# arkworks-rs/sumcheck

Measured on AMD Instinct MI355X. Metric: MLSumcheck prover field-ops/s (BLS12-381 Fr, nv=24), higher is better.
Workload: dtype u256 (BLS12-381 Fr, Montgomery form; integer arithmetic on 9 x 29-bit limbs); 1 GPU; BASELINE config 3: MLSumcheck prove, ListOfProducts [[0, 1, 2, 3], [4, 5, 6], [7, 8], [9]] over 10 tables, nv=24 (24 per GPU shard), BLS12-381 Fr, tables HBM-resident; nv=24, nv_per_gpu=24, tables=10, degree=4, launcher=single process, ranks_seen=1, communicator=none, round_loop=library, round_loop_reason=single GPU: no exchange

## Files before the change

### sumcheck_amd/build.py

```python
from __future__ import annotations

import os
import subprocess
import sys

HERE = os.path.dirname(os.path.abspath(__file__))
CSRC = os.path.join(HERE, "csrc")
OUT = os.path.join(HERE, "libsumcheck_hip.so")
OUT_EXP = os.path.join(HERE, "libsumcheck_hip_exp.so")
SOURCES = ["kernels_big.hip", "kernels.hip", "kernels_tail.hip", "kernels_batch.hip", "kernels_batch_gkr.hip", "kernels_batch_eval.hip", "kernels_batch_rounds.hip", "kernels_wide.hip", "kernels_wide16.hip", "gkr.hip", "abi.hip", "protocol.hip", "batch.hip", "batch_rounds.hip", "comm.hip", "kernels_selftest.hip"]
HEADERS = ["fr_device.hpp", "fe_device.hpp", "kernel_common.hpp", "finalize_device.hpp", "batch_round.hpp", "wide_cell.hpp", "fe_mad_chain.inc", "fr_mac.inc", "fr_mul_gen.inc", "kernels.h", "host_fr.hpp", "transcript.hpp", "prover_internal.hpp", "load_factor.hpp", "wide_tree.hpp", os.path.join("..", "..", "include", "sumcheck_hip.h")]
EXTRA = os.environ.get("SC_BUILD_EXTRA", "").split()
FLAGS = ["--offload-arch=gfx950", "-O3", "-std=c++17", "-fPIC", "-fvisibility=hidden", "-Wall", "-Wno-unused-function"]


def _stale(out: str) -> bool:
    if not os.path.exists(out):
        return True
    t = os.path.getmtime(out)
    deps = [os.path.join(CSRC, s) for s in SOURCES + HEADERS] + [os.path.abspath(__file__)]
    return any(os.path.getmtime(d) > t for d in deps if os.path.exists(d))


def _obj_stale(obj: str, src: str, cmd: list) -> bool:
    dep = obj + ".d"
    if not (os.path.exists(obj) and os.path.exists(dep)):
        return True
    try:
        if open(obj + ".cmd").read() != " ".join(cmd):
            return True
    except OSError:
        return True
    t = os.path.getmtime(obj)
    try:
        words = open(dep).read().replace("\\\n", " ").split()
    except OSError:
        return True
    files = [w for w in words[1:] if not w.endswith(":")] + [src, os.path.abspath(__file__)]
    return any((not os.path.exists(f)) or os.path.getmtime(f) > t for f in files if not f.startswith("/opt/rocm"))


def _start(experiments: bool, verbose: bool, force: bool = False):
    hipcc = os.environ.get("HIPCC", "/opt/rocm/bin/hipcc")
    bdir = os.path.join(HERE, "build_exp" if experiments else "build")
    os.makedirs(bdir, exist_ok=True)
    procs, objs = [], []
    stale_any = False
    for s in SOURCES:
        o = os.path.join(bdir, s + ".o")
        objs.append(o)
        src = os.path.join(CSRC, s)
        cmd = [hipcc] + FLAGS + (["-DSC_EXPERIMENTS"] if experiments else []) + EXTRA + ["-Rpass-analysis=kernel-resource-usage", "-MD", "-MF", o + ".d", "-c", src, "-o", o]
        if not force and not _obj_stale(o, src, cmd):
            continue
        stale_any = True
        if os.path.exists(o + ".cmd"):
            os.remove(o + ".cmd")
        if verbose:
            print(" ".join(cmd), file=sys.stderr)
        procs.append((cmd, o, subprocess.Popen(cmd, stderr=open(o + ".log", "w"))))
    return hipcc, procs, objs


def _finish(hipcc, procs, objs, out):
    for cmd, o, p in procs:
        if p.wait() != 0:
            try:
                sys.stderr.write("".join(l for l in open(o + ".log") if "remark:" not in l and "-Rpass" not in l)[-8000:])
            except OSError:
                pass
            for f in (o, o + ".d"):
                if os.path.exists(f):
                    os.remove(f)
            raise RuntimeError("hipcc failed: " + " ".join(cmd))
        with open(o + ".cmd", "w") as f:
            f.write(" ".join(cmd))
    subprocess.check_call([hipcc, "--offload-arch=gfx950", "-shared", "-fPIC"] + objs + ["-o", out])
    return out


def _cmd_mismatch(experiments: bool) -> bool:
    hipcc = os.environ.get("HIPCC", "/opt/rocm/bin/hipcc")
    bdir = os.path.join(HERE, "build_exp" if experiments else "build")
    for s in SOURCES:
        o = os.path.join(bdir, s + ".o")
        cmd = [hipcc] + FLAGS + (["-DSC_EXPERIMENTS"] if experiments else []) + EXTRA + ["-Rpass-analysis=kernel-resource-usage", "-MD", "-MF", o + ".d", "-c", os.path.join(CSRC, s), "-o", o]
        try:
            if open(o + ".cmd").read() != " ".join(cmd):
                return True
        except OSError:
            if os.path.exists(o):
                return True
    return False

# ... 21 lines not shown
```

### sumcheck_amd/csrc/abi.hip

```cpp
#include "prover_internal.hpp"

static std::atomic<uint32_t> g_publish_timeout_ms{0};
std::chrono::milliseconds publish_timeout() {
    uint32_t ms = g_publish_timeout_ms.load(std::memory_order_relaxed);
    if (ms == 0) {
        const char *e = std::getenv("SC_PUBLISH_TIMEOUT_MS");
        const long v = e ? std::atol(e) : 0;
        ms = v > 0 ? (uint32_t)std::min<long>(v, 3600 * 1000L) : 20000u;
        g_publish_timeout_ms.store(ms, std::memory_order_relaxed);
    }
    return std::chrono::milliseconds(ms);
}
extern "C" int sc_set_publish_timeout_ms(uint32_t ms) {
    g_publish_timeout_ms.store(ms ? ms : 20000u, std::memory_order_relaxed);
    return SC_OK;
}
static thread_local std::string g_last_error;
static thread_local int g_device = 0;

static std::recursive_mutex g_gate_mutex[64];
thread_local uint16_t g_gate_depth[64];
void gate_lock(int device) {
    g_gate_mutex[(unsigned)device & 63u].lock();
    ++g_gate_depth[(unsigned)device & 63u];
// ... 228 lines not shown
#ifdef SC_EXPERIMENTS
    if (const char *e = std::getenv("SC_FE")) p->use_fe = std::atoi(e) != 0;
    if (const char *e = std::getenv("SC_KERNEL")) p->kernel_variant = std::atoi(e);
    if (!p->use_fe && p->kernel_variant == 3) p->kernel_variant = 0;
#endif
    p->use_f29 = p->kernel_variant == 3;
    p->wide_tree = wide_tree_enabled();
#ifdef SC_EXPERIMENTS
    if (const char *e = std::getenv("SC_F29")) p->use_f29 = p->use_f29 && std::atoi(e) != 0;
#endif
    for (uint32_t k = 0; k < d->n_products; ++k)
        if (d->prod_offsets[k + 1] - d->prod_offsets[k] > (p->wide_tree ? 8u : 4u)) p->use_f29 = false;
    if (d->n_tables > (uint32_t)scd::kMaxSmallTables) p->use_f29 = false;
    p->merge_rounds = p->kernel_variant == 3 && d->n_products > 0 && d->n_products <= (uint32_t)scd::kMaxRoundProds;
    for (uint32_t k = 0; k < d->n_products; ++k)
        if (d->prod_offsets[k + 1] - d->prod_offsets[k] > 4) p->merge_rounds = false;
#ifdef SC_EXPERIMENTS
    if (const char *e = std::getenv("SC_MERGE")) p->merge_rounds = p->merge_rounds && std::atoi(e) != 0;
    if (const char *e = std::getenv("SC_FUSED_FIN")) p->fused_finalize = std::atoi(e) != 0;
#endif
    p->use_tail = scd::policy(scd::kPolTail) != 0;

    uint64_t partial_elems = 0;
    std::vector<uint32_t> slot_table, slot_exp;
    std::vector<FinProd> fin(p->K);
    std::vector<Combo> combos;
    std::vector<sch::Fr> Wall;
    for (uint32_t k = 0; k < p->K; ++k) {
        Product pr;
        std::memcpy(&pr.coeff, d->coeffs + 4 * k, 32);
        if (sch::geq_p(pr.coeff)) return sc_internal_fail(SC_ERR_BAD_ARG, "coefficient %u is not a canonical field element", k);
        for (uint32_t q = d->prod_offsets[k]; q < d->prod_offsets[k + 1]; ++q) {
            const uint32_t t = d->prod_indices[q];
            auto it = std::find(pr.tables.begin(), pr.tables.end(), t);
            if (it == pr.tables.end()) {
                pr.tables.push_back(t);
                pr.exps.push_back(1);
            } else {
                pr.exps[it - pr.tables.begin()]++;
            }
        }
        p->prod_indices.emplace_back(d->prod_indices + d->prod_offsets[k], d->prod_indices + d->prod_offsets[k + 1]);
        pr.M = d->prod_offsets[k + 1] - d->prod_offsets[k];
        pr.fused = pr.M <= (uint32_t)scd::kMaxFusedM;
        if (!pr.fused) p->any_generic = true;
        pr.partial_off = partial_elems;
        partial_elems += (uint64_t)scd::kMaxGrid * (pr.M + 1);
        pr.slot_off = (uint32_t)slot_table.size();
        slot_table.insert(slot_table.end(), pr.tables.begin(), pr.tables.end());
        slot_exp.insert(slot_exp.end(), pr.exps.begin(), pr.exps.end());
        fin[k].M = pr.M;
        fin[k].pad = 0;
        fin[k].partial_off = pr.partial_off;
        {
            sch::Fr sc = pr.coeff;
            for (uint32_t dbl = 0; dbl < 5 * (pr.M - 1); ++dbl) sc = sch::add(sc, sc);
            std::vector<sch::Fr> w;
            fin[k].w_off = Wall.size();
            build_node_matrix(pr.M, p->D, pr.coeff, w);
            Wall.insert(Wall.end(), w.begin(), w.end());
            build_node_matrix(pr.M, p->D, sc, w);
            Wall.insert(Wall.end(), w.begin(), w.end());
        }
        for (uint32_t t = 0; t <= pr.M; ++t) {
            Combo c;
            c.t = t;
            c.M = pr.M;
            c.slot_off = pr.slot_off;
            c.n_slots = (uint32_t)pr.tables.size();
            c.partial_off = pr.partial_off;
            combos.push_back(c);
        }
        p->prods.push_back(std::move(pr));
    }

    const bool on_device = d->flags & SC_TABLES_ON_DEVICE;
    const bool borrow = on_device && (d->flags & SC_TABLES_BORROW);
    const uint64_t n = 1ULL << p->nv;
    const bool streamed = !on_device && (d->flags & SC_TABLES_STREAM) && p->nv >= 11;
    const bool small_foot = borrow || streamed;
    bool staged = false;
    const uint64_t s0 = small_foot ? std::max<uint64_t>(n >> 1, 1) : n;
    const uint64_t s1 = small_foot ? std::max<uint64_t>(n >> 2, 1) : std::max<uint64_t>(n >> 1, 1);
    const uint64_t per_table = (s0 + s1) * 36;
    HIP_TRY(hipMalloc(&p->arena, per_table * p->U));
    p->arena_bytes = per_table * p->U;
    p->tabs.resize(p->U);
    p->borrow = borrow;
    if (on_device && !borrow) HIP_TRY(hipDeviceSynchronize());
    for (uint32_t u = 0; u < p->U; ++u) {
        Table &t = p->tabs[u];
        char *base = static_cast<char *>(p->arena) + per_table * u;
        t.buf[0] = reinterpret_cast<uint4 *>(base);
        t.buf[1] = reinterpret_cast<uint4 *>(base + s0 * 32);
        t.buf_top[0] = reinterpret_cast<int32_t *>(base + (s0 + s1) * 32);
        t.buf_top[1] = t.buf_top[0] + s0;
        if (streamed) {
            t.cur = nullptr;
            t.next = 0;
            p->host_tabs.push_back(d->tables[u]);
        } else if (borrow) {
            t.cur = reinterpret_cast<const uint4 *>(d->tables[u]);
            t.next = 0;
            p->origin.push_back(t.cur);
        } else {
            if (!on_device && (d->flags & SC_TABLES_STREAM)) p->host_tabs.push_back(d->tables[u]);
            if (!(staged = !on_device && staged_init_applies(p)))
                HIP_TRY(hipMemcpyAsync(t.buf[0], d->tables[u], n * 32, on_device ? hipMemcpyDeviceToDevice : hipMemcpyHostToDevice, p->stream));
            t.cur = t.buf[0];
            t.next = 1;
        }
    }

    if (streamed) {
        p->streamed = true;
        uint32_t cl = p->stream_chunk_request ? p->stream_chunk_request : 22u;
        cl = std::max(10u, std::min(cl, p->nv));
        p->chunk_log2 = cl;
        for (int q = 0; q < 2; ++q) {
            HIP_TRY(hipMalloc(&p->ring[q], ((size_t)p->U << cl) * 32));
            HIP_TRY(hipEventCreateWithFlags(&p->ev_copied[q], hipEventDisableTiming));
            HIP_TRY(hipEventCreateWithFlags(&p->ev_consumed[q], hipEventDisableTiming));
        }
        HIP_TRY(hipStreamCreateWithFlags(&p->copy_stream, hipStreamNonBlocking));
        HIP_TRY(hipMalloc(&p->d_chunk_msg, (size_t)2 * p->D * 32));
    }
    HIP_TRY(hipMalloc(&p->d_partials, std::max<uint64_t>(partial_elems, 1) * 32));
    HIP_TRY(hipMalloc(&p->d_partials2, std::max<uint64_t>(partial_elems, 1) * 32));
    HIP_TRY(hipMalloc(&p->d_fin_counters, 4 * (2 + scd::kMaxGrid / 32 + 16)));
    HIP_TRY(hipMemsetAsync(p->d_fin_counters, 0, 4 * (2 + scd::kMaxGrid / 32 + 16), p->stream));
    p->d_fin_mb_counter = p->d_fin_counters + (2 + scd::kMaxGrid / 32 + 8);
    HIP_TRY(hipMalloc(&p->d_finprods, std::max<size_t>(p->K, 1) * sizeof(FinProd)));
    if (p->K) HIP_TRY(hipMemcpyAsync(p->d_finprods, fin.data(), p->K * sizeof(FinProd), hipMemcpyHostToDevice, p->stream));
    p->h_finprods = fin;
    HIP_TRY(hipMalloc(&p->d_W, std::max<size_t>(2 * Wall.size(), 1) * 32));
    p->w_elems = (uint32_t)Wall.size();
    if (!Wall.empty()) {
        HIP_TRY(hipMemcpyAsync(p->d_W, Wall.data(), Wall.size() * 32, hipMemcpyHostToDevice, p->stream));
        HIP_TRY(hipMemcpyAsync(p->d_W + Wall.size(), Wall.data(), Wall.size() * 32, hipMemcpyHostToDevice, p->stream));
    }
    HIP_TRY(hipMalloc(&p->d_scratch, (size_t)(2 + p->D) * std::max<uint32_t>(p->K, 1) * p->D * 32));
    {
        const size_t one = (size_t)std::max<uint32_t>(p->K, 1) * p->D * 32;
        HIP_TRY(hipMalloc(&p->d_sums[0], 2 * one));
        p->d_sums[1] = reinterpret_cast<FrHost *>(reinterpret_cast<char *>(p->d_sums[0]) + one);
    }
    HIP_TRY(hipMalloc(&p->d_out, (size_t)p->D * 32));
    HIP_TRY(hipHostMalloc(reinterpret_cast<void **>(&p->h_out), (size_t)p->D * 32, hipHostMallocMapped | hipHostMallocCoherent));
    HIP_TRY(hipHostMalloc(reinterpret_cast<void **>(&p->h_flag), 64, hipHostMallocMapped | hipHostMallocCoherent));
    *p->h_flag = 0;
    HIP_TRY(hipHostGetDevicePointer(reinterpret_cast<void **>(&p->h_out_dev), p->h_out, 0));
    HIP_TRY(hipHostGetDevicePointer(reinterpret_cast<void **>(&p->h_flag_dev), p->h_flag, 0));
    p->has_meta = combos.size() <= (size_t)scd::kMetaCombos && slot_table.size() <= (size_t)scd::kMetaSlots;
    if (p->has_meta) {
        std::memset(&p->meta, 0, sizeof(p->meta));
        std::copy(combos.begin(), combos.end(), p->meta.combo);
        std::copy(slot_table.begin(), slot_table.end(), p->meta.slot_table);
        std::copy(slot_exp.begin(), slot_exp.end(), p->meta.slot_exp);
    }
    p->n_combos = (int)combos.size();
    HIP_TRY(hipMalloc(&p->d_combos, std::max<size_t>(combos.size(), 1) * sizeof(Combo)));
    if (!combos.empty()) HIP_TRY(hipMemcpyAsync(p->d_combos, combos.data(), combos.size() * sizeof(Combo), hipMemcpyHostToDevice, p->stream));
    HIP_TRY(hipMalloc(&p->d_slot_table, std::max<size_t>(slot_table.size(), 1) * 4));
    HIP_TRY(hipMalloc(&p->d_slot_exp, std::max<size_t>(slot_exp.size(), 1) * 4));
    if (!slot_table.empty()) {
        HIP_TRY(hipMemcpyAsync(p->d_slot_table, slot_table.data(), slot_table.size() * 4, hipMemcpyHostToDevice, p->stream));
        HIP_TRY(hipMemcpyAsync(p->d_slot_exp, slot_exp.data(), slot_exp.size() * 4, hipMemcpyHostToDevice, p->stream));
    }
    if (p->any_generic || p->U > (uint32_t)scd::kMaxSmallTables) {
        HIP_TRY(hipMalloc(&p->d_cur_tables, 2 * p->U * sizeof(void *)));
        HIP_TRY(hipHostMalloc(reinterpret_cast<void **>(&p->h_cur_tables), 2 * p->U * sizeof(void *), hipHostMallocDefault));
    }
    if (staged) {
        int rc_s = staged_copy_and_round1(p, d->tables);
        if (rc_s) return rc_s;
    }
    HIP_TRY(hipStreamSynchronize(p->stream));
    return SC_OK;
}
// ... 22 lines not shown
        kept->pool_key.clear();
        prover_destroy(kept);
    }
    sc_prover *p = new (std::nothrow) sc_prover();
    if (!p) return sc_internal_fail(SC_ERR_OOM, "host allocation failed");
    rc = prover_build(desc, p);
    if (rc) {
        prover_destroy(p);
        return rc;
    }
    p->pool_key = std::move(key);
    *out = p;
    return SC_OK;
}

extern "C" int sc_prover_init_streamed(const sc_poly_desc *desc, uint32_t chunk_log2, sc_prover **out) {
    if (!out) return sc_internal_fail(SC_ERR_BAD_ARG, "null out");
    *out = nullptr;
    int rc = validate_desc(desc);
    if (rc) return rc;
    if (desc->flags & SC_TABLES_ON_DEVICE) return sc_internal_fail(SC_ERR_BAD_ARG, "streamed tables are host tables");
    sc_prover *p = new (std::nothrow) sc_prover();
    if (!p) return sc_internal_fail(SC_ERR_OOM, "host allocation failed");
    p->stream_chunk_request = chunk_log2;
    sc_poly_desc d2 = *desc;
    d2.flags |= SC_TABLES_STREAM;
    rc = prover_build(&d2, p);
    if (rc) {
        prover_destroy(p);
        return rc;
    }
    *out = p;
    return SC_OK;
}

extern "C" int sc_prover_set_stream(sc_prover *p, void *hip_stream, int use_own) {
    if (!p) return sc_internal_fail(SC_ERR_BAD_ARG, "null prover");
    int rc_q = resident_quiesce(p);
    if (rc_q) return rc_q;
    DeviceGate gate_(p->device);
    HIP_TRY(hipSetDevice(p->device));
    HIP_TRY(hipStreamSynchronize(p->stream));
    p->stream = use_own ? p->own_stream : static_cast<hipStream_t>(hip_stream);
    return SC_OK;
}

int collect_timing(sc_prover *p) {
    if (!p->timing || !p->timing_pending) return SC_OK;
    HIP_TRY(hipEventSynchronize(p->ev1));
    float ms = 0.f;
    HIP_TRY(hipEventElapsedTime(&ms, p->ev0, p->ev1));
    p->rounds_ms += ms;
    for (uint32_t k = 0; k < (p->prod_merged ? 1u : p->K) && p->prod_timed; ++k) {
        HIP_TRY(hipEventElapsedTime(&ms, p->prod_ev[2 * k], p->prod_ev[2 * k + 1]));
        p->prod_ms[k] += ms;
        p->prod_launches[k] += 1;
        if (p->timed_round >= 1 && p->timed_round <= p->round_kernel_ms.size()) {
            p->round_kernel_ms[p->timed_round - 1] += ms;
            if (k == 0) p->round_kernel_launches[p->timed_round - 1] += 1;
        }
    }
    p->timing_pending = false;
    return SC_OK;
}

int prover_bind_out(sc_prover *p, const uint64_t *r, uint64_t *d_out) {
    int rc_q = resident_quiesce(p);
    if (rc_q) return rc_q;
    DeviceGate gate_(p->device);
    if (p->exhausted || p->round == 0 || p->round > p->nv) return sc_internal_fail(SC_ERR_NOT_ACTIVE, "bind needs a prover that has run at least one round");
    if (p->streamed && p->round < 2) return sc_internal_fail(SC_ERR_NOT_ACTIVE, "a streamed handle's tables are resident from round 2 on: nothing to bind yet");
    sch::Fr rr;
    std::memcpy(&rr, r, 32);
    if (sch::geq_p(rr)) return sc_internal_fail(SC_ERR_BAD_ARG, "challenge is not a canonical field element");
    HIP_TRY(hipSetDevice(p->device));
    p->randomness.push_back(rr);
    const uint64_t n_out = 1ULL << (p->nv - p->round);
    for (uint32_t u0 = 0; u0 < p->U; u0 += (uint32_t)scd::kMaxSmallTables) {
        const uint32_t cnt = std::min<uint32_t>(p->U - u0, (uint32_t)scd::kMaxSmallTables);
        TablePtrs tp;
        std::memset(&tp, 0, sizeof(tp));
        for (uint32_t j = 0; j < cnt; ++j) {
            tp.src[j] = p->tabs[u0 + j].cur;
            tp.src_top[j] = p->tabs[u0 + j].cur_top;
            tp.dst[j] = reinterpret_cast<uint4 *>(d_out + 4 * n_out * (size_t)(u0 + j));
        }
        HIP_TRY(scd::launch_fix_multi(tp, (int)cnt, to_dev(rr), nullptr, n_out, p->stream));
    }
    p->exhausted = true;
    return SC_OK;
}

extern "C" int sc_prover_bind_final(sc_prover *p, const uint64_t *r, uint64_t *d_out) {
    if (!p || !r || !d_out) return sc_internal_fail(SC_ERR_BAD_ARG, "null argument");
    if (p->exhausted || p->round != p->nv) return sc_internal_fail(SC_ERR_NOT_ACTIVE, "bind_final needs a prover that has finished its last local round");
    return prover_bind_out(p, r, d_out);
}

extern "C" int sc_prover_push_randomness(sc_prover *p, const uint64_t *r) {
    if (!p || !r) return sc_internal_fail(SC_ERR_BAD_ARG, "null argument");
    sch::Fr rr;
    std::memcpy(&rr, r, 32);
    p->randomness.push_back(rr);
    return SC_OK;
}

extern "C" int sc_prover_state(sc_prover *p, uint64_t *randomness, uint32_t *n_randomness, uint64_t *tables_out, uint32_t *round) {
    if (!p) return sc_internal_fail(SC_ERR_BAD_ARG, "null prover");
    if (tables_out) {
        int rc_q = resident_quiesce(p);
        if (rc_q) return rc_q;
    }
    DeviceGate gate_(p->device);
    if (randomness && !p->randomness.empty()) std::memcpy(randomness, p->randomness.data(), p->randomness.size() * 32);
    if (n_randomness) *n_randomness = (uint32_t)p->randomness.size();
    if (round) *round = p->round;
    if (tables_out) {
        if (p->exhausted) return sc_internal_fail(SC_ERR_NOT_ACTIVE, "tables were consumed by sc_prover_bind_final");
        HIP_TRY(hipSetDevice(p->device));
        const uint32_t bound = p->round > 0 ? p->round - 1 : 0;
        const uint64_t n = 1ULL << (p->nv - bound);
        if (p->streamed && p->round < 2) {
            for (uint32_t u = 0; u < p->U; ++u) std::memcpy(tables_out + 4 * n * u, p->host_tabs[u], n * 32);
            return SC_OK;
        }
        void *tmp = nullptr;
        for (uint32_t u = 0; u < p->U; ++u) {
            const void *src = p->tabs[u].cur;
            if (p->tabs[u].cur_top) {
                if (!tmp) HIP_TRY(hipMalloc(&tmp, n * 32));
                HIP_TRY(scd::launch_f29_to_sat(p->tabs[u].cur, p->tabs[u].cur_top, static_cast<uint4 *>(tmp), n, p->stream));
                src = tmp;
            }
            HIP_TRY(hipMemcpyAsync(tables_out + 4 * n * u, src, n * 32, hipMemcpyDeviceToHost, p->stream));
            if (tmp) HIP_TRY(hipStreamSynchronize(p->stream));
        }
        if (tmp) (void)hipFree(tmp);
        HIP_TRY(hipStreamSynchronize(p->stream));
    }
    return SC_OK;
}

extern "C" int sc_prover_last_round_ms(sc_prover *p, float *ms) {
    if (!p || !ms) return sc_internal_fail(SC_ERR_BAD_ARG, "null argument");
    if (!p->timed) return sc_internal_fail(SC_ERR_BAD_ARG, "no timed round: enable sc_prover_set_timing before the round");
    HIP_TRY(hipEventSynchronize(p->ev1));
    HIP_TRY(hipEventElapsedTime(ms, p->ev0, p->ev1));
    return SC_OK;
}

extern "C" int sc_prover_set_timing(sc_prover *p, int on) {
    if (!p) return sc_internal_fail(SC_ERR_BAD_ARG, "null prover");
    int rc_q = resident_quiesce(p);
    if (rc_q) return rc_q;
    DeviceGate gate_(p->device);
    HIP_TRY(hipSetDevice(p->device));
    if (on && p->prod_ev.empty()) {
        p->prod_ev.resize(2 * (size_t)p->K);
        for (auto &e : p->prod_ev) HIP_TRY(hipEventCreate(&e));
    }
    p->timing = on != 0;
    p->timing_pending = false;
    p->prod_ms.assign(p->K, 0.0);
    p->prod_launches.assign(p->K, 0);
    p->rounds_ms = 0.0;
    p->round_kernel_ms.assign(p->nv, 0.0);
    p->round_kernel_launches.assign(p->nv, 0);
    return SC_OK;
}

extern "C" int sc_prover_get_round_timing(sc_prover *p, double *ms_per_round, uint64_t *launches_per_round) {
    if (!p) return sc_internal_fail(SC_ERR_BAD_ARG, "null prover");
    DeviceGate gate_(p->device);
    if (!p->timing) return sc_internal_fail(SC_ERR_BAD_ARG, "timing is not enabled on this handle");
    HIP_TRY(hipSetDevice(p->device));
    int rc = collect_timing(p);
    if (rc) return rc;
    for (uint32_t i = 0; i < p->nv; ++i) {
        if (ms_per_round) ms_per_round[i] = i < p->round_kernel_ms.size() ? p->round_kernel_ms[i] : 0.0;
        if (launches_per_round) launches_per_round[i] = i < p->round_kernel_launches.size() ? p->round_kernel_launches[i] : 0;
    }
    return SC_OK;
}

extern "C" int sc_prover_get_timing(sc_prover *p, double *ms_per_product, uint64_t *launches_per_product, double *rounds_ms) {
    if (!p) return sc_internal_fail(SC_ERR_BAD_ARG, "null prover");
    DeviceGate gate_(p->device);
    if (!p->timing) return sc_internal_fail(SC_ERR_BAD_ARG, "timing is not enabled on this handle");
    HIP_TRY(hipSetDevice(p->device));
    int rc = collect_timing(p);
    if (rc) return rc;
    for (uint32_t k = 0; k < p->K; ++k) {
        if (ms_per_product) ms_per_product[k] = p->prod_ms[k];
        if (launches_per_product) launches_per_product[k] = p->prod_launches[k];
    }
    if (rounds_ms) *rounds_ms = p->rounds_ms;
    return SC_OK;
}

extern "C" int sc_prover_reset(sc_prover *p, const uint64_t *const *tables_or_null, uint32_t flags) {
    if (!p) return sc_internal_fail(SC_ERR_BAD_ARG, "null prover");
    (void)resident_quiesce(p);
    DeviceGate gate_(p->device);
    HIP_TRY(hipSetDevice(p->device));
    abandon_deferred(p);
    if (wait_gave_up(p)) {
        HIP_TRY(hipStreamSynchronize(p->stream));
        __atomic_store_n(p->sig + 1, 0u, __ATOMIC_RELEASE);
    }
    {
        int rc_t = collect_timing(p);
        if (rc_t) return rc_t;
    }
    p->r1_cached = false;
    if (p->w_scaled) {
        HIP_TRY(hipMemcpyAsync(p->d_W, p->d_W + p->w_elems, (size_t)p->w_elems * 32, hipMemcpyDeviceToDevice, p->stream));
        p->w_scaled = false;
    }
    const uint64_t n = 1ULL << p->nv;
    if (p->streamed) {
        if (flags & SC_TABLES_ON_DEVICE) return sc_internal_fail(SC_ERR_BAD_ARG, "streamed tables are host tables");
        HIP_TRY(hipStreamSynchronize(p->stream));
        for (uint32_t u = 0; u < p->U; ++u) {
            if (tables_or_null) {
                if (!tables_or_null[u]) return sc_internal_fail(SC_ERR_BAD_ARG, "table %u is null", u);
                p->host_tabs[u] = tables_or_null[u];
            }
            p->tabs[u].cur = nullptr;
            p->tabs[u].cur_top = nullptr;
            p->tabs[u].next = 0;
        }
    } else if (p->borrow) {
        for (uint32_t u = 0; u < p->U; ++u) {
            if (tables_or_null) {
                if (!tables_or_null[u]) return sc_internal_fail(SC_ERR_BAD_ARG, "table %u is null", u);
                p->origin[u] = reinterpret_cast<const uint4 *>(tables_or_null[u]);
            }
            p->tabs[u].cur = p->origin[u];
            p->tabs[u].cur_top = nullptr;
            p->tabs[u].next = 0;
        }
    } else {
        if (!tables_or_null && p->host_tabs.size() == p->U) tables_or_null = p->host_tabs.data();
        if (!tables_or_null) return sc_internal_fail(SC_ERR_BAD_ARG, "a copying handle needs the tables again to reset");
        const bool on_device = flags & SC_TABLES_ON_DEVICE;
        if (on_device) HIP_TRY(hipDeviceSynchronize());
        const bool staged = !on_device && staged_init_applies(p);
        for (uint32_t u = 0; u < p->U; ++u) {
            if (!tables_or_null[u]) return sc_internal_fail(SC_ERR_BAD_ARG, "table %u is null", u);
            if (!staged)
                HIP_TRY(hipMemcpyAsync(p->tabs[u].buf[0], tables_or_null[u], n * 32, on_device ? hipMemcpyDeviceToDevice : hipMemcpyHostToDevice,
                                       p->stream));
            p->tabs[u].cur = p->tabs[u].buf[0];
            p->tabs[u].cur_top = nullptr;
            p->tabs[u].next = 1;
        }
        if (staged) {
            p->round = 0;
            p->exhausted = false;
            int rc_s = staged_copy_and_round1(p, tables_or_null);
            if (rc_s) return rc_s;
        }
        HIP_TRY(hipStreamSynchronize(p->stream));
    }
    p->round = 0;
    p->sums_round = -1;
    p->exhausted = false;
    p->randomness.clear();
    return SC_OK;
}

hipStream_t sc_internal_prover_stream(sc_prover *p) { return p->stream; }
const void *sc_internal_bound_table(sc_prover *p, uint32_t u) {
    if (!p || u >= p->U || p->round != p->nv || p->exhausted || p->tabs[u].cur_top || p->res.active) return nullptr;
    return p->tabs[u].cur;
}
int sc_internal_scale_by_bound_table(sc_prover *p, const void *table, const sch::Fr &r_last) {
    if (!p || !table || p->round != 0) return sc_internal_fail(SC_ERR_BAD_ARG, "scale_by_bound_table: a freshly reset handle and a bound table");
    DeviceGate gate_(p->device);
    HIP_TRY(hipSetDevice(p->device));
    HIP_TRY(scd::launch_scale_w_by_table_eval(p->d_W, p->d_W + p->w_elems, p->w_elems, table, to_dev(r_last), p->stream));
    p->w_scaled = true;
    return SC_OK;
}

namespace {
struct DevMem {
    void *p = nullptr;
    ~DevMem() {
        if (p) (void)hipFree(p);
    }
};
struct StreamGuard {
    hipStream_t s = nullptr;
    ~StreamGuard() {
        if (s) (void)hipStreamDestroy(s);
    }
};
struct EvalCache {
    std::mutex mu;
    void *buf = nullptr;
    size_t cap = 0;
    int device = -1;
    hipStream_t s = nullptr;
};
EvalCache g_eval_cache;
struct EvalLease {
    bool held = false;
    EvalLease() : held(g_eval_cache.mu.try_lock()) {}
    ~EvalLease() {
        if (held) g_eval_cache.mu.unlock();
    }
    void *get(int device, size_t bytes, hipStream_t *s_out) {
        if (!held || bytes > sc_internal_cache_limit()) return nullptr;
        EvalCache &c = g_eval_cache;
        if (c.device != device) {
            if (c.buf) (void)hipFree(c.buf);
            if (c.s) (void)hipStreamDestroy(c.s);
            c.buf = nullptr;
            c.s = nullptr;
            c.cap = 0;
            c.device = device;
        }
        if (!c.s && hipStreamCreateWithFlags(&c.s, hipStreamNonBlocking) != hipSuccess) {
            (void)hipGetLastError();
            c.s = nullptr;
            return nullptr;
        }
        if (c.cap < bytes) {
            if (c.buf) (void)hipFree(c.buf);
            c.buf = nullptr;
            c.cap = 0;
            if (hipMalloc(&c.buf, bytes) != hipSuccess) {
                (void)hipGetLastError();
                c.buf = nullptr;
                return nullptr;
            }
            c.cap = bytes;
        }
        *s_out = c.s;
        return c.buf;
    }
};
}
void sc_internal_release_eval_cache() {
    std::lock_guard<std::mutex> lk(g_eval_cache.mu);
    if (g_eval_cache.device >= 0) (void)hipSetDevice(g_eval_cache.device);
    if (g_eval_cache.buf) (void)hipFree(g_eval_cache.buf);
    if (g_eval_cache.s) (void)hipStreamDestroy(g_eval_cache.s);
    g_eval_cache.buf = nullptr;
    g_eval_cache.s = nullptr;
    g_eval_cache.cap = 0;
    g_eval_cache.device = -1;
}

extern "C" int sc_fix_variables(const uint64_t *in, uint32_t nv, const uint64_t *point, uint32_t k, uint64_t *out, uint32_t flags) {
    if (!in || !out || (k && !point)) return sc_internal_fail(SC_ERR_BAD_ARG, "null argument");
// ... 538 lines not shown
```

### sumcheck_amd/csrc/fe_device.hpp

```cpp
#pragma once
#include <utility>
#include "fr_device.hpp"
#include "kernels.h"

namespace scd {

struct Fe {
    int32_t l[9];
};
struct FeU {
    int32_t l[9];
};

constexpr int32_t kFeMask = 0x1fffffff;

__device__ __forceinline__ constexpr int32_t fe_p_limb(int i) {
    return i == 0 ? 0x00000001 : i == 1 ? 0x1ffffff8 : i == 2 ? 0x1f96ffbf : i == 3 ? 0x1b4805ff : i == 4 ? 0x1d80553b
         : i == 5 ? 0x0c0404d0 : i == 6 ? 0x1520cce7 : i == 7 ? 0x0a6533af : 0x0073eda7;
}

__device__ __forceinline__ Fe fe_from_fr(const Fr &a) {
    Fe r;
    r.l[0] = (int32_t)(a.v[0] & (uint32_t)kFeMask);
#pragma unroll
    for (int i = 1; i < 8; ++i) r.l[i] = (int32_t)(((a.v[i - 1] >> (32 - 3 * i)) | (a.v[i] << (3 * i))) & (uint32_t)kFeMask);
    r.l[8] = (int32_t)(a.v[7] >> 8);
    return r;
}
__device__ __forceinline__ FeU feu_from_host(const FrHost &h) {
    Fr a;
#pragma unroll
    for (int i = 0; i < 4; ++i) {
        a.v[2 * i] = (uint32_t)h.l[i];
        a.v[2 * i + 1] = (uint32_t)(h.l[i] >> 32);
    }
    const Fe e = fe_from_fr(a);
    FeU u;
#pragma unroll
    for (int i = 0; i < 9; ++i) u.l[i] = e.l[i];
    return u;
}

__device__ __forceinline__ FeU feu_shl5(const uint32_t (&v)[8]) {
    FeU u;
    u.l[0] = (int32_t)((v[0] << 5) & (uint32_t)kFeMask);
#pragma unroll
    for (int i = 1; i < 9; ++i) {
        const int s = 29 * i - 5, w = s >> 5, off = s & 31;
        uint32_t x = v[w] >> off;
        if (off > 3 && w + 1 < 8) x |= v[w + 1] << (32 - off);
        u.l[i] = (int32_t)(x & (uint32_t)kFeMask);
    }
    return u;
}

__device__ __forceinline__ Fe fe_zero() {
    Fe r;
#pragma unroll
    for (int i = 0; i < 9; ++i) r.l[i] = 0;
    return r;
}
__device__ __forceinline__ Fe fe_add(const Fe &a, const Fe &b) {
    Fe r;
#pragma unroll
    for (int i = 0; i < 9; ++i) r.l[i] = a.l[i] + b.l[i];
    return r;
}
__device__ __forceinline__ Fe fe_sub(const Fe &a, const Fe &b) {
    Fe r;
#pragma unroll
    for (int i = 0; i < 9; ++i) r.l[i] = a.l[i] - b.l[i];
    return r;
}
__device__ __forceinline__ Fe fe_normalize(const Fe &a) {
    Fe r;
    int32_t c = 0;
#pragma unroll
    for (int i = 0; i < 8; ++i) {
        const int32_t t = a.l[i] + c;
        r.l[i] = t & kFeMask;
        c = t >> 29;
    }
    r.l[8] = a.l[8] + c;
    return r;
}

__device__ __forceinline__ Fe fe_carry_pass(const Fe &a) {
    Fe r;
    r.l[0] = a.l[0] & kFeMask;
#pragma unroll
    for (int i = 1; i < 8; ++i) r.l[i] = (a.l[i] & kFeMask) + (a.l[i - 1] >> 29);
    r.l[8] = a.l[8] + (a.l[7] >> 29);
    return r;
}

#ifndef SC_NO_NT
typedef uint32_t sc_u32x4 __attribute__((ext_vector_type(4)));
__device__ __forceinline__ uint4 f29_ld(const uint4 *p) {
    const sc_u32x4 v = __builtin_nontemporal_load(reinterpret_cast<const sc_u32x4 *>(p));
    return make_uint4(v.x, v.y, v.z, v.w);
}
__device__ __forceinline__ void f29_st(uint4 *p, const uint32_t a, const uint32_t b, const uint32_t c, const uint32_t d) {
    sc_u32x4 w;
    w.x = a; w.y = b; w.z = c; w.w = d;
    __builtin_nontemporal_store(w, reinterpret_cast<sc_u32x4 *>(p));
}
#else
__device__ __forceinline__ uint4 f29_ld(const uint4 *p) { return *p; }
__device__ __forceinline__ void f29_st(uint4 *p, const uint32_t a, const uint32_t b, const uint32_t c, const uint32_t d) { *p = make_uint4(a, b, c, d); }
#endif
__device__ __forceinline__ uint64_t f29_chunk(uint64_t entry, int half) {
    const uint64_t q = entry >> 1;
    const uint64_t col = ((q & 63) >> 1) | ((q & 1) << 5);
    return (entry >> 7) * 256 + (uint64_t)(2 * (int)(entry & 1) + half) * 64 + col;
}
__device__ __forceinline__ Fe fe_load_f29(const uint4 *main, uint64_t entry, int32_t top) {
    const uint4 a = f29_ld(main + f29_chunk(entry, 0)), b = f29_ld(main + f29_chunk(entry, 1));
    Fe r;
    r.l[0] = (int32_t)a.x; r.l[1] = (int32_t)a.y; r.l[2] = (int32_t)a.z; r.l[3] = (int32_t)a.w;
    r.l[4] = (int32_t)b.x; r.l[5] = (int32_t)b.y; r.l[6] = (int32_t)b.z; r.l[7] = (int32_t)b.w;
    r.l[8] = top;
    return r;
}
__device__ __forceinline__ void fe_store_f29(uint4 *main, uint64_t entry, const Fe &v) {
    f29_st(main + f29_chunk(entry, 0), (uint32_t)v.l[0], (uint32_t)v.l[1], (uint32_t)v.l[2], (uint32_t)v.l[3]);
    f29_st(main + f29_chunk(entry, 1), (uint32_t)v.l[4], (uint32_t)v.l[5], (uint32_t)v.l[6], (uint32_t)v.l[7]);
}
template <bool kChain>
__device__ __forceinline__ void fe_mad(int64_t &acc, const int32_t a, const int32_t b) {
    if constexpr (kChain) asm("v_mad_i64_i32 %0, vcc, %1, %2, %0" : "+v"(acc) : "v"(a), "v"(b) : "vcc");
    else acc += (int64_t)a * (int64_t)b;
}
template <bool kChain>
__device__ __forceinline__ void fe_mad_k(int64_t &acc, const int32_t a, const int32_t k) {
    if constexpr (kChain) asm("v_mad_i64_i32 %0, vcc, %1, %2, %0" : "+v"(acc) : "v"(a), "s"(k) : "vcc");
    else acc += (int64_t)a * (int64_t)k;
}
#include "fe_mad_chain.inc"
#ifdef SC_CHAIN_PER_MAD
constexpr bool kChainColumns = false;
#else
constexpr bool kChainColumns = true;
#endif
#ifdef SC_MAD_CHAIN
constexpr bool kChainDefault = true;
#else
constexpr bool kChainDefault = false;
#endif

__host__ __device__ constexpr int fe_col_n(int k) { return (k < 8 ? k : 8) - (k > 8 ? k - 8 : 0) + 1; }
__host__ __device__ constexpr int fe_col_nr(int k) {
    int c = 0;
    for (int j = 0; j < 9; ++j) c += (j < k && k - j >= 1 && k - j < 9) ? 1 : 0;
    return c;
}
template <int K, typename B>
__device__ __forceinline__ void fe_col_chain(int64_t &acc, const Fe &a, const B &b, const int32_t (&m)[9]) {
    constexpr int n = fe_col_n(K), nr = fe_col_nr(K);
    int32_t xa[9] = {0, 0, 0, 0, 0, 0, 0, 0, 0}, xb[9] = {0, 0, 0, 0, 0, 0, 0, 0, 0}, xm[9] = {0, 0, 0, 0, 0, 0, 0, 0, 0}, xk[9] = {0, 0, 0, 0, 0, 0, 0, 0, 0};
    int q = 0, qr = 0;
#pragma unroll
    for (int i = 0; i < 9; ++i) {
        const int j = K - i;
        if (j >= 0 && j < 9) { xa[q] = a.l[i]; xb[q] = b.l[j]; ++q; }
    }
#pragma unroll
    for (int j = 0; j < 9; ++j) {
        const int l = K - j;
        if (j < K && l >= 1 && l < 9) { xm[qr] = m[j]; xk[qr] = -fe_p_limb(l); ++qr; }
    }
    if constexpr (nr == 0) mad_chain_vv(acc, xa, xb, n);
    else MadMix<n, nr>::run(acc, xa, xb, xm, xk);
}
template <int K>
__device__ __forceinline__ void fe_col2_chain(int64_t &acc, const Fe &a, const Fe &b, const Fe &c, const Fe &d, const int32_t (&m)[9]) {
    constexpr int n = fe_col_n(K), nr = fe_col_nr(K);
    int32_t xa[9] = {0, 0, 0, 0, 0, 0, 0, 0, 0}, xb[9] = {0, 0, 0, 0, 0, 0, 0, 0, 0}, xc[9] = {0, 0, 0, 0, 0, 0, 0, 0, 0}, xd[9] = {0, 0, 0, 0, 0, 0, 0, 0, 0};
    int32_t xm[9] = {0, 0, 0, 0, 0, 0, 0, 0, 0}, xk[9] = {0, 0, 0, 0, 0, 0, 0, 0, 0};
    int q = 0, qr = 0;
#pragma unroll
    for (int i = 0; i < 9; ++i) {
        const int j = K - i;
        if (j >= 0 && j < 9) { xa[q] = a.l[i]; xb[q] = b.l[j]; xc[q] = c.l[i]; xd[q] = d.l[j]; ++q; }
    }
#pragma unroll
    for (int j = 0; j < 9; ++j) {
        const int l = K - j;
        if (j < K && l >= 1 && l < 9) { xm[qr] = m[j]; xk[qr] = -fe_p_limb(l); ++qr; }
    }
    mad_chain_vv(acc, xa, xb, n);
    if constexpr (nr == 0) mad_chain_vv(acc, xc, xd, n);
    else MadMix<n, nr>::run(acc, xc, xd, xm, xk);
}
template <int K>
__device__ __forceinline__ void fe_col_finish(int64_t &acc, int32_t (&m)[9], Fe &r) {
    if constexpr (K < 9) m[K] = (int32_t)((uint32_t)acc & (uint32_t)kFeMask);
    else r.l[K - 9] = (int32_t)((uint32_t)acc & (uint32_t)kFeMask);
    acc >>= 29;
}
template <typename B, int... K>
__device__ __forceinline__ Fe fe_mul_chain_cols(const Fe &a, const B &b, std::integer_sequence<int, K...>) {
    int64_t acc = 0;
    int32_t m[9] = {0, 0, 0, 0, 0, 0, 0, 0, 0};
    Fe r;
    ((fe_col_chain<K, B>(acc, a, b, m), fe_col_finish<K>(acc, m, r)), ...);
    r.l[8] = (int32_t)acc;
    return r;
}
template <int... K>
// ... 171 lines not shown
```

### sumcheck_amd/csrc/kernels.h

```cpp
#pragma once
#include <hip/hip_runtime.h>
#include <stdint.h>

namespace scd {

constexpr int kBlock = 256;
constexpr int kMaxFusedM = 8;
constexpr int kMaxGrid = 1024;
constexpr int kMaxSmallTables = 32;
constexpr uint64_t kSmallRoundPairs = 1u << 14;

struct FrHost {
    uint64_t l[4];
};

constexpr int32_t kNodeInf = 0x7fffffff;
__host__ __device__ constexpr int32_t node_value(int s) {
    return s == 0 ? 0 : s == 1 ? 1 : s == 2 ? kNodeInf : ((s - 3) % 2 == 0 ? -((s - 3) / 2 + 1) : ((s - 3) / 2 + 2));
}

struct BindConst {
    int32_t R[9][9];
};

struct Slot {
    const uint4 *src;
    uint4 *dst;
    uint32_t mode;
    uint32_t exp;
    const int32_t *src_top;
    int32_t *dst_top;
};

struct ProdArgs {
    Slot slot[kMaxFusedM];
    int n_slots;
};
constexpr int kMaxWideM = 12;
struct WideArgs16 {
    Slot slot[kMaxWideM];
    int n_slots;
};

constexpr int kMaxRoundProds = 12;
constexpr int kRoundTreeGrid = 768;
struct TreeProd {
    Slot slot[4];
    uint32_t M;
    uint32_t pad;
    uint64_t partial_off;
};
struct RoundFin {
    int enabled;
    int D;
    uint64_t w_off[kMaxRoundProds];
    const uint4 *Wm;
    uint4 *partials2;
    uint32_t *counters;
    uint4 *out;
    uint64_t *out_wide;
    uint4 *h_out;
    uint32_t *h_flag;
    uint32_t seq;
};
struct RoundArgs {
    TreeProd prod[kMaxRoundProds];
    int n_prod;
    RoundFin fin;
    uint32_t part_stride, part_block0;
};

struct FinProd {
    uint32_t M;
    uint32_t pad;
    uint64_t partial_off;
    uint64_t w_off;
};

struct TablePtrs {
    const uint4 *src[kMaxSmallTables];
    uint4 *dst[kMaxSmallTables];
    const int32_t *src_top[kMaxSmallTables];
};
struct Combo {
    uint32_t t;
    uint32_t M;
    uint32_t slot_off;
    uint32_t n_slots;
    uint64_t partial_off;
};

constexpr int kFoldMaxLevels = 3;
struct FoldArgs {
    const uint4 *src[kMaxSmallTables];
    uint4 *dst[kMaxSmallTables];
    FrHost r32[kFoldMaxLevels];
};
hipError_t launch_fold_multi(const FoldArgs &args, int levels, int n_tables, uint64_t n_out, hipStream_t stream);

constexpr int kMetaProds = 16;
struct FinMeta {
    FinProd prod[kMetaProds];
};
constexpr int kMetaCombos = 24, kMetaSlots = 48;
struct ComboMeta {
    Combo combo[kMetaCombos];
    uint32_t slot_table[kMetaSlots];
    uint32_t slot_exp[kMetaSlots];
};

#ifndef SC_TAIL_MAX_PAIRS
#define SC_TAIL_MAX_PAIRS 2048
#endif
constexpr uint64_t kTailMaxPairs = SC_TAIL_MAX_PAIRS;
static_assert(kTailMaxPairs >= kBlock && (kTailMaxPairs & (kTailMaxPairs - 1)) == 0 && kTailMaxPairs <= kSmallRoundPairs, "a power of two within the small rounds");
constexpr int kTailMaxGrid = 1024;
constexpr int kTailFlatPairs = 16;
__host__ __device__ constexpr uint64_t tail_flat_pairs(int n_combos) {
    uint64_t p = kTailFlatPairs;
    while (p < 64 && 2 * p * (uint64_t)n_combos <= (uint64_t)kBlock) p *= 2;
    return p;
}
struct TailTables {
    const uint4 *cur0[kMaxSmallTables];
    const int32_t *cur0_top[kMaxSmallTables];
    uint4 *b0[kMaxSmallTables];
    uint4 *b1[kMaxSmallTables];
};
struct TailArgs {
    TailTables t;
    int n_tables;
    int n_rounds;
    int first_has_bind;
    uint64_t first_pairs;
    FrHost r0;
    int n_combos, K, D;
    const uint4 *Wm;
    uint4 *partials;
    uint32_t *sync;
    uint4 *sums;
    uint64_t *chal;
    uint4 *h_out;
    uint32_t *h_flag;
    uint32_t seq0;
    uint32_t *sig;
    const uint64_t *mail_host;
    uint32_t sig0;
    uint32_t max_spins;
};
constexpr int kTsBlock = 256, kTsMaxBlocks = 256;
constexpr uint32_t kLazySumMaxP = 282;
__host__ __device__ constexpr bool lazy_sum_needs_reduce(uint64_t terms, uint32_t worst_p) { return terms * (uint64_t)worst_p > (uint64_t)kLazySumMaxP; }
constexpr uint64_t kTsMaxPairs = 1u << 16;
constexpr size_t kTsAccWords = 4 * 8 * (size_t)kMetaCombos * 8;
constexpr size_t kTsXwWords = kTsAccWords + (size_t)kTsMaxBlocks * kMaxSmallTables * 10 + 8;
struct TailSlicesArgs {
    TailArgs base;
    int B;
    uint64_t *xw;
    const uint64_t *mail_vram;
    uint32_t tag0;
    uint32_t fin_bytes;
    uint32_t lds_entries;
    uint32_t stage_off;
    uint32_t worst_p;
};
int tail_slices_blocks(uint64_t first_pairs, int n_tables, int K, int D, int n_combos, int max_multiplicands, int max_blocks, uint32_t worst_p);
constexpr uint32_t tail_worst_p(uint32_t lazy_binds) { return lazy_binds + 2; }
int tail_slices_max_blocks(int device, int max_multiplicands);
hipError_t ensure_dynamic_lds(const void *kernel, int bytes, bool (&done)[64]);
hipError_t launch_tail_slices(TailSlicesArgs args, const ComboMeta &meta, const FinMeta &fin, int max_multiplicands, hipStream_t stream);
struct BatchArgs {
    const uint4 *const *tables;
    const uint4 *Wm;
    uint32_t w_stride;
    uint32_t n, n_tables, nv;
    int n_combos, K, D;
    uint32_t *ticket;
    uint64_t *h_msg;
    const uint64_t *mail;
    uint32_t mail_local;
    uint32_t *h_giveup;
    uint32_t tag0;
    uint32_t max_spins;
    uint32_t fin_bytes;
};
bool batch_shape_fits(uint32_t nv, uint32_t n_tables, int K, int D, uint32_t max_multiplicands);
int batch_blocks_per_cu(int device, uint32_t nv, uint32_t n_tables, int K, int D);
hipError_t launch_batch_proofs(BatchArgs args, const ComboMeta &meta, const FinMeta &fin, int grid, hipStream_t stream);
constexpr int kGkrBatchMaxDim = 9;
constexpr uint64_t kGkrBatchMaxNnzPerCell = 64;
struct GkrBatchInst {
    const uint64_t *idx;
    const uint4 *vals;
    const uint4 *f2, *f3;
    const uint4 *g;
    uint64_t nnz;
};
struct BatchGkrArgs {
    const GkrBatchInst *inst;
    const uint4 *Wm;
    uint32_t n, dim;
    uint32_t *ticket;
    uint64_t *h_msg;
    const uint64_t *mail;
    uint32_t mail_local;
    uint32_t *h_giveup;
    uint32_t tag0;
// ... 93 lines not shown
    kPlanBatchRoundsSerial,
    kPlanFoldMulti,
    kPlanBatchEvalOneBlock,
    kPlanBatchEvalSerial,
    kPlanBatchGkrEvalOneBlock,
    kPlanBatchGkrEvalSerial,
    kPlanBatchOneBlock,
    kPlanBatchSerial,
    kPlanBatchGkrOneBlock,
    kPlanBatchGkrSerial,
    kPlanCount
};
void plan_hit(int plan);
hipError_t launch_scale_w_by_table_eval(FrHost *W, const FrHost *W0, uint32_t n, const void *table, const FrHost &r, hipStream_t stream);
hipError_t launch_zero_words(uint32_t *p, uint32_t n, hipStream_t stream, uint32_t *p2 = nullptr, uint32_t n2 = 0);
hipError_t launch_tail_rounds(const TailArgs &args, const ComboMeta &meta, const FinMeta &fin, int grid, hipStream_t stream);

int grid_for_pairs(uint64_t n_pairs);

#ifdef SC_EXPERIMENTS
hipError_t launch_prod_round(int M, const ProdArgs &args, const FrHost &r, uint64_t n_pairs, FrHost *d_partials, int grid,
                             hipStream_t stream);
#endif
hipError_t launch_prod_round_fe(int M, const ProdArgs &args, const FrHost &r32, uint64_t n_pairs, FrHost *d_partials, int grid,
                                hipStream_t stream);
hipError_t launch_prod_tree(int M, const ProdArgs &args, const BindConst &rc, uint64_t n_pairs, FrHost *d_partials, int grid,
                            hipStream_t stream);
hipError_t launch_prod_tree_wide(int M, const ProdArgs &args, const BindConst &rc, uint64_t n_pairs, FrHost *d_partials, int grid, hipStream_t stream);
hipError_t launch_prod_tree_wide16(int M, const WideArgs16 &args, const FrHost &comp, uint64_t n_pairs, FrHost *d_partials, int grid, hipStream_t stream);
hipError_t launch_round_tree(const RoundArgs &args, const BindConst &rc, uint64_t n_pairs, FrHost *d_partials, int grid, hipStream_t stream, bool split = true,
                             bool skip1 = false);
#ifdef SC_EXPERIMENTS
int grid_for_tiles(uint64_t n_pairs);
hipError_t launch_round_tile(int M, const ProdArgs &args, const FrHost &r32, uint64_t n_pairs, FrHost *d_partials, int grid,
                             hipStream_t stream);
#endif
hipError_t launch_sum_generic(const uint4 *const *d_cur_tables, const uint32_t *d_slot_table, const uint32_t *d_slot_exp,
                              int n_slots, int M, uint64_t n_pairs, FrHost *d_partials, int grid, hipStream_t stream);
hipError_t launch_fix(const uint4 *src, uint4 *dst, const FrHost &r, uint64_t n_out, hipStream_t stream);
hipError_t launch_wait_challenge(uint32_t *flag_dev, uint32_t want, const FrHost *mail_host_dev, FrHost *mail_dev, hipStream_t stream,
                                 uint32_t spins_override = 0);
hipError_t launch_fix_multi(const TablePtrs &tp, int n_tables, const FrHost &r, const FrHost *r_mail, uint64_t n_out, hipStream_t stream);
hipError_t launch_sum_combos(const TablePtrs &tp, const Combo *d_combos, int n_combos, const uint32_t *d_slot_table,
                             const uint32_t *d_slot_exp, uint64_t n_pairs, FrHost *d_partials, int grid, hipStream_t stream);
hipError_t launch_sum_combos_ptrs(const uint4 *const *d_cur_tables, const Combo *d_combos, int n_combos, const uint32_t *d_slot_table,
                                  const uint32_t *d_slot_exp, uint64_t n_pairs, FrHost *d_partials, int grid, hipStream_t stream);
hipError_t launch_sum_combos_meta(const TablePtrs &tp, const ComboMeta &meta, int n_combos, uint64_t n_pairs, FrHost *d_partials, int grid,
                                  hipStream_t stream);
struct ClaimArgs {
    uint32_t skip1;
    uint32_t pad;
    const uint4 *prev;
    FrHost lam[14];
};
__host__ __device__ constexpr int claim_off(int M) { return (M - 1) * (M + 2) / 2; }
constexpr int kWideTagShift = 44;
__host__ __device__ constexpr uint32_t wide_tag_of(uint32_t seq) { return (seq & 0x7fffu) + 1u; }
bool finalize_keeps_sums(int K, int D, int nblocks, bool have_host_prods, bool have_counter);
hipError_t launch_finalize(const FinProd *d_prods, const FinProd *h_prods_or_null, const FrHost *d_W, int K, int D, int nblocks, const FrHost *d_partials, FrHost *d_scratch,
                           FrHost *d_out, uint64_t *d_out_wide, FrHost *h_out_mapped, uint32_t *h_flag_mapped, uint32_t seq,
                           int scaled , uint32_t *d_counter_or_null, hipStream_t stream, const ClaimArgs *claim_or_null = nullptr);
hipError_t launch_synth(uint64_t seed, uint64_t stream_id, uint64_t first, uint64_t n, uint4 *d_out, hipStream_t stream);
hipError_t launch_scale(const uint4 *src, uint4 *dst, const FrHost &s, uint64_t n, hipStream_t stream);
hipError_t launch_tag_words(uint64_t *d_words, int n, uint32_t gen, hipStream_t stream);
hipError_t launch_publish_words(const uint64_t *d_src, uint64_t *h_dst_mapped, int n, uint32_t *h_flag_mapped, uint32_t seq, hipStream_t stream);
constexpr int kP2PMaxRanks = 16, kP2PWords = 64;
constexpr size_t kP2PInboxWords = 2 * (size_t)kP2PMaxRanks * kP2PWords;
constexpr uint32_t kP2PRetryBit = 0x80000000u;
struct P2PArgs {
    uint64_t *inbox[kP2PMaxRanks];
    int nranks, rank, n_words;
    uint32_t gen;
    uint32_t max_spins;
};
struct PeerLanes {
    const uint64_t *p[kP2PMaxRanks];
    int n;
};
hipError_t launch_sum_peer_lanes(const PeerLanes &peers, uint64_t n_words, uint64_t *out, hipStream_t stream);
hipError_t launch_p2p_allreduce(const P2PArgs &args, uint64_t *d_lanes, uint64_t *h_dst_mapped, uint32_t *h_flag_mapped, uint32_t seq, hipStream_t stream);
hipError_t launch_gather_to_tables(const uint4 *recv, uint4 *tabs, uint32_t G, uint32_t U, uint32_t per, hipStream_t stream);
hipError_t launch_msg_accumulate(const FrHost *in, FrHost *acc, int D, bool first, bool last, FrHost *d_out, uint64_t *d_out_wide, FrHost *h_out_mapped,
                                 uint32_t *h_flag_mapped, uint32_t seq, hipStream_t stream);
hipError_t launch_f29_to_sat(const uint4 *src, const int32_t *src_top, uint4 *dst, uint64_t n, hipStream_t stream);
hipError_t launch_fr_elementwise(int op, const uint4 *a, const uint4 *b, const FrHost &u, uint4 *out, uint64_t n, hipStream_t stream);
hipError_t launch_bench_modmul(uint64_t n_threads, uint32_t reps, uint32_t variant, uint64_t *d_sink, hipStream_t stream);

}
```

### sumcheck_amd/csrc/kernels.hip

```cpp
#include "kernel_common.hpp"

#include <algorithm>
#include <cstdlib>
#include <cstring>

namespace scd {
#ifdef SC_FIN_CLOCKS
__device__ uint64_t g_fin_clk[12];
#define FIN_STAMP(i)                                                                                                                      \
    do {                                                                                                                                  \
        if (threadIdx.x == 0) g_fin_clk[i] = wall_clock64();                                                                              \
    } while (0)
#else
#define FIN_STAMP(i)
#endif
}
#include "finalize_device.hpp"
namespace scd {
__global__ __launch_bounds__(kBlock) void k_sum_generic(const uint4 *const *__restrict__ cur_tables,
                                                        const uint32_t *__restrict__ slot_table,
                                                        const uint32_t *__restrict__ slot_exp, const int n_slots, const int M,
                                                        const uint64_t n_pairs, uint4 *__restrict__ partials) {
    __shared__ uint32_t sm[kBlock / 64][8];
    const uint32_t t = blockIdx.y;
// ... 20 lines not shown
}

__global__ __launch_bounds__(kBlock) void k_fix(const uint4 *__restrict__ src, uint4 *__restrict__ dst, const FrHost r_h,
                                                const uint64_t n_out) {
    const FrU r = fru_from_host(r_h);
    const uint64_t stride = (uint64_t)gridDim.x * kBlock;
    for (uint64_t b = (uint64_t)blockIdx.x * kBlock + threadIdx.x; b < n_out; b += stride) {
        const uint4 *p = src + 4 * b;
        const Fr lo = fr_load(p), hi = fr_load(p + 2);
        fr_store(dst + 2 * b, fr_add(lo, fr_mul_u(fr_sub(hi, lo), r)));
    }
}

template <int L>
__global__ __launch_bounds__(kBlock) void k_fold_multi(const FoldArgs A, const uint64_t n_out) {
    const uint4 *__restrict__ src = A.src[blockIdx.y];
    uint4 *__restrict__ dst = A.dst[blockIdx.y];
    FeU r[L];
#pragma unroll
    for (int l = 0; l < L; ++l) r[l] = feu_from_host(A.r32[l]);
    const uint64_t stride = (uint64_t)gridDim.x * kBlock;
    for (uint64_t i = (uint64_t)blockIdx.x * kBlock + threadIdx.x; i < n_out; i += stride) {
        Fe v[1 << L];
        const uint4 *p = src + 2 * (i << L);
#pragma unroll
        for (int j = 0; j < (1 << L); ++j) v[j] = fe_from_fr(fr_load(p + 2 * j));
#pragma unroll
        for (int l = 0; l < L; ++l) {
#pragma unroll
            for (int j = 0; j < (1 << (L - 1 - l)); ++j)
                v[j] = fe_carry_pass(fe_add(v[2 * j], fe_mul_u(fe_sub(v[2 * j + 1], v[2 * j]), r[l])));
        }
        fr_store(dst + 2 * i, fe_to_fr(v[0]));
    }
}

hipError_t launch_fold_multi(const FoldArgs &args, int levels, int n_tables, uint64_t n_out, hipStream_t stream) {
    plan_hit(kPlanFoldMulti);
    const dim3 grid(grid_for_pairs(n_out), n_tables);
    switch (levels) {
    case 1: hipLaunchKernelGGL(k_fold_multi<1>, grid, dim3(kBlock), 0, stream, args, n_out); break;
    case 2: hipLaunchKernelGGL(k_fold_multi<2>, grid, dim3(kBlock), 0, stream, args, n_out); break;
    case 3: hipLaunchKernelGGL(k_fold_multi<3>, grid, dim3(kBlock), 0, stream, args, n_out); break;
    default: return hipErrorInvalidValue;
    }
    return hipGetLastError();
}

__global__ __launch_bounds__(kBlock) void k_scale(const uint4 *__restrict__ src, uint4 *__restrict__ dst, const FrHost s_h,
                                                  const uint64_t n) {
    const FrU s = fru_from_host(s_h);
    const uint64_t stride = (uint64_t)gridDim.x * kBlock;
    for (uint64_t i = (uint64_t)blockIdx.x * kBlock + threadIdx.x; i < n; i += stride)
        fr_store(dst + 2 * i, fr_mul_u(fr_load(src + 2 * i), s));
}

__global__ void k_wait_challenge(uint32_t *__restrict__ flag, const uint32_t want, const uint32_t max_spins,
                                 const uint64_t *__restrict__ mail_host, uint64_t *__restrict__ mail_dev) {
    if (threadIdx.x == 0) {
        bool seen = false;
        for (uint32_t spin = 0; spin < max_spins && !seen; ++spin) {
            seen = __hip_atomic_load(flag, __ATOMIC_ACQUIRE, __HIP_MEMORY_SCOPE_SYSTEM) == want;
            if (!seen) __builtin_amdgcn_s_sleep(8);
        }
        if (!seen) __hip_atomic_store(flag + 1, want, __ATOMIC_RELEASE, __HIP_MEMORY_SCOPE_SYSTEM);
    }
    __syncthreads();
    if (threadIdx.x < 4) mail_dev[threadIdx.x] = __hip_atomic_load(mail_host + threadIdx.x, __ATOMIC_RELAXED, __HIP_MEMORY_SCOPE_SYSTEM);
}
uint32_t wait_spins_default() { return (uint32_t)policy(kPolWaitSpins); }
hipError_t launch_wait_challenge(uint32_t *flag_dev, uint32_t want, const FrHost *mail_host_dev, FrHost *mail_dev, hipStream_t stream,
                                 uint32_t spins_override) {
    const uint32_t max_spins = spins_override ? spins_override : wait_spins_default();
    hipLaunchKernelGGL(k_wait_challenge, dim3(1), dim3(64), 0, stream, flag_dev, want, max_spins, reinterpret_cast<const uint64_t *>(mail_host_dev),
                       reinterpret_cast<uint64_t *>(mail_dev));
    return hipGetLastError();
}

__global__ __launch_bounds__(kBlock) void k_fix_multi(const TablePtrs tp, const FrHost r_h, const FrHost *__restrict__ r_mail, const uint64_t n_out) {
    const FrU r = fru_from_host(r_mail ? *r_mail : r_h);
    const FeU r32 = feu_shl5(r.v);
    const uint4 *__restrict__ src = tp.src[blockIdx.y];
    uint4 *__restrict__ dst = tp.dst[blockIdx.y];
    const int32_t *__restrict__ stop = tp.src_top[blockIdx.y];
    const uint64_t stride = (uint64_t)gridDim.x * kBlock;
    for (uint64_t b = (uint64_t)blockIdx.x * kBlock + threadIdx.x; b < n_out; b += stride) {
        const uint4 *p = src + 4 * b;
        Fe lo, hi;
        if (stop) {
            const int2 t = *reinterpret_cast<const int2 *>(stop + 2 * b);
            lo = fe_load_f29(src, 2 * b, t.x);
            hi = fe_load_f29(src, 2 * b + 1, t.y);
        } else {
            lo = fe_from_fr(fr_load(p));
            hi = fe_from_fr(fr_load(p + 2));
        }
        fr_store(dst + 2 * b, fe_to_fr(fe_add(lo, fe_mul_u<true>(fe_sub(hi, lo), r32))));
    }
}

__global__ __launch_bounds__(kBlock) void k_f29_to_sat(const uint4 *__restrict__ src, const int32_t *__restrict__ stop, uint4 *__restrict__ dst,
                                                       const uint64_t n) {
    const uint64_t stride = (uint64_t)gridDim.x * kBlock;
    for (uint64_t i = (uint64_t)blockIdx.x * kBlock + threadIdx.x; i < n; i += stride)
        fr_store(dst + 2 * i, fe_to_fr(fe_load_f29(src, i, stop[i])));
}

template <typename SlotsT, typename TabFn>
__device__ __forceinline__ Fr combo_product(const TabFn &tab, const Combo &c, const SlotsT slot_table, const SlotsT slot_exp, const uint64_t b,
                                            const int32_t nv, const Fr &tf) {
    Fr prod = fr_zero();
    bool first = true;
    for (uint32_t s0 = 0; s0 < c.n_slots; s0 += 4) {
        const uint32_t ns = c.n_slots - s0 < 4u ? c.n_slots - s0 : 4u;
        Fr lo[4], hi[4];
#pragma unroll
        for (uint32_t q = 0; q < 4; ++q) {
            if (q < ns) {
                const uint4 *p = tab(slot_table[c.slot_off + s0 + q]) + 4 * b;
                if (nv != 1) lo[q] = fr_load(p);
                if (nv != 0) hi[q] = fr_load(p + 2);
            }
        }
#pragma unroll
        for (uint32_t q = 0; q < 4; ++q) {
            if (q < ns) {
                Fr val;
                if (nv == 0) val = lo[q];
                else if (nv == 1) val = hi[q];
                else if (nv == kNodeInf) val = fr_sub(hi[q], lo[q]);
                else if (nv == -1) val = fr_sub(fr_add(lo[q], lo[q]), hi[q]);
                else if (nv == 2) val = fr_sub(fr_add(hi[q], hi[q]), lo[q]);
                else val = fr_add(lo[q], fr_mul(fr_sub(hi[q], lo[q]), tf));
                uint32_t k = 0;
                if (first) { prod = val; k = 1; first = false; }
                for (const uint32_t e = slot_exp[c.slot_off + s0 + q]; k < e; ++k) prod = fr_mul(prod, val);
            }
        }
    }
    return prod;
}

template <typename SlotsT, typename TabFn>
__device__ __forceinline__ Fe combo_product_fe(const TabFn &tab, const Combo &c, const SlotsT slot_table, const SlotsT slot_exp, const uint64_t b,
                                               const int32_t nv) {
    Fe prod = fe_zero();
    bool first = true;
    for (uint32_t s0 = 0; s0 < c.n_slots; s0 += 4) {
        const uint32_t ns = c.n_slots - s0 < 4u ? c.n_slots - s0 : 4u;
        Fr lo[4], hi[4];
#pragma unroll
        for (uint32_t q = 0; q < 4; ++q) {
            if (q < ns) {
                const uint4 *p = tab(slot_table[c.slot_off + s0 + q]) + 4 * b;
                if (nv != 1) lo[q] = fr_load(p);
                if (nv != 0) hi[q] = fr_load(p + 2);
            }
        }
#pragma unroll
        for (uint32_t q = 0; q < 4; ++q) {
            if (q < ns) {
                Fe val;
                if (nv == 0) val = fe_from_fr(lo[q]);
                else if (nv == 1) val = fe_from_fr(hi[q]);
                else val = fe_line(fe_from_fr(lo[q]), fe_from_fr(hi[q]), nv);
                uint32_t k = 0;
                if (first) { prod = val; k = 1; first = false; }
                for (const uint32_t e = slot_exp[c.slot_off + s0 + q]; k < e; ++k) prod = fe_mul<true>(val, prod);
            }
        }
    }
    return prod;
}

template <typename SlotsT, typename TabFn>
__device__ __forceinline__ void sum_combo_body(const TabFn &tab, const Combo c, const SlotsT slot_table, const SlotsT slot_exp,
                                               const uint64_t n_pairs, uint4 *__restrict__ partials, uint32_t (*sm)[8], const uint32_t vbx, const uint32_t vgx) {
    const uint32_t t = c.t;
    const int32_t nv = node_value((int)t);
    const Fr tf = node_constant(nv);
    Fr acc = fr_zero();
    const uint64_t stride = (uint64_t)vgx * kBlock;
    if (c.M <= (uint32_t)kMaxFusedM) {
        Fe a = fe_zero();
        uint32_t iter = 0;
        for (uint64_t b = (uint64_t)vbx * kBlock + threadIdx.x; b < n_pairs; b += stride, ++iter) {
            a = fe_carry_pass(fe_add(a, combo_product_fe(tab, c, slot_table, slot_exp, b, nv)));
            if ((iter & 31u) == 31u) a = fe_from_fr(fe_to_fr(a));
// ... 161 lines not shown
}

#ifdef SC_TAIL_CLOCKS
__device__ uint64_t g_tail_clk[64 * 8];
#define TAIL_STAMP(j, i)                                                                                                                  \
    do {                                                                                                                                  \
        if (blockIdx.x == 0 && threadIdx.x == 0 && (j) < 64) g_tail_clk[8 * (j) + (i)] = wall_clock64();                                  \
    } while (0)
#else
#define TAIL_STAMP(j, i)
#endif
__global__ __launch_bounds__(kBlock) void k_tail_rounds(const TailArgs A, const ComboMeta meta, const FinMeta fin) {
    __shared__ uint32_t sm[kBlock / 64][8];
    __shared__ uint64_t r_sh[4];
    __shared__ uint32_t stop_sh;
    extern __shared__ uint4 fin_lds[];
    const uint32_t G = gridDim.x;
    const uint32_t bar_spins = A.max_spins > (1u << 20) ? A.max_spins : (1u << 20);
    uint32_t gen = 0;
    uint64_t n_pairs = A.first_pairs;
    int binds = 0;
    auto tab = [&](uint32_t u) -> const uint4 * { return binds == 0 ? A.t.cur0[u] : (binds & 1) ? A.t.b0[u] : A.t.b1[u]; };
    auto prod_of = [&](int k) -> FinProd { return fin.prod[k]; };
    __shared__ Combo combo_sh[kMetaCombos];
    __shared__ uint32_t slot_table_sh[kMetaSlots], slot_exp_sh[kMetaSlots];
    __shared__ const uint4 *tab_sh[kMaxSmallTables];
    __shared__ int prod_index_sh[kMetaCombos];
    for (int i = threadIdx.x; i < kMetaCombos; i += kBlock) {
        combo_sh[i] = meta.combo[i];
        int k = 0;
        if (i < A.n_combos)
            while (k < A.K - 1 && fin.prod[k].partial_off != meta.combo[i].partial_off) ++k;
        prod_index_sh[i] = k;
    }
    for (int i = threadIdx.x; i < kMetaSlots; i += kBlock) {
        slot_table_sh[i] = meta.slot_table[i];
        slot_exp_sh[i] = meta.slot_exp[i];
    }
    auto tab_lds = [&](uint32_t u) -> const uint4 * { return tab_sh[u]; };
    if (threadIdx.x == 0) stop_sh = 0;
    const Fr *w_pre = nullptr;
    for (int j = 0; j < A.n_rounds; ++j, n_pairs >>= 1) {
        const uint32_t Gj = tail_active_blocks(n_pairs, A.n_tables, A.n_combos, G);
        if (blockIdx.x >= Gj) return;
        TAIL_STAMP(j, 0);
        const bool solo = Gj == 1;
        if (j > 0 || A.first_has_bind) {
            if (j == 0) {
                if (threadIdx.x < 4) r_sh[threadIdx.x] = A.r0.l[threadIdx.x];
            } else if (blockIdx.x != 0) {
                if (threadIdx.x == 0) {
                    uint32_t spins = 0;
                    bool expired = false;
                    while (__hip_atomic_load(A.sync + 2, __ATOMIC_RELAXED, __HIP_MEMORY_SCOPE_AGENT) < (uint32_t)j) {
                        if (++spins > 16u * (A.max_spins / 4 + 1) + 4096u) { expired = true; break; }
                        __builtin_amdgcn_s_sleep(2);
                    }
                    __builtin_amdgcn_fence(__ATOMIC_ACQUIRE, "agent");
                    stop_sh = __hip_atomic_load(A.sync + 3, __ATOMIC_RELAXED, __HIP_MEMORY_SCOPE_AGENT);
                    if (expired) {
                        __hip_atomic_store(A.sync + 16 + blockIdx.x, kFlagDead, __ATOMIC_RELAXED, __HIP_MEMORY_SCOPE_AGENT);
                        __hip_atomic_store(A.sig + 1, A.sig0 + (uint32_t)j, __ATOMIC_RELEASE, __HIP_MEMORY_SCOPE_SYSTEM);
                        stop_sh = 1;
                    }
                }
                __syncthreads();
                if (threadIdx.x < 4) r_sh[threadIdx.x] = __hip_atomic_load(A.chal + 4 * (j & 1) + threadIdx.x, __ATOMIC_RELAXED, __HIP_MEMORY_SCOPE_AGENT);
            }
            __syncthreads();
            if (stop_sh) return;
            FrHost rh;
#pragma unroll
            for (int i = 0; i < 4; ++i) rh.l[i] = r_sh[i];
            const FeU r32 = feu_shl5(fru_from_host(rh).v);
            const uint64_t n_out = 2 * n_pairs;
            const int sh = 63 - __builtin_clzll(n_out);
            const uint64_t total = n_out * (uint64_t)A.n_tables;
            for (uint64_t i = (uint64_t)blockIdx.x * kBlock + threadIdx.x; i < total; i += (uint64_t)Gj * kBlock) {
                const uint32_t u = (uint32_t)(i >> sh);
                const uint64_t b = i & (n_out - 1);
                const uint4 *src = tab(u);
                uint4 *dst = (binds & 1) ? A.t.b1[u] : A.t.b0[u];
                Fe lo, hi;
                const int32_t *stop = binds == 0 ? A.t.cur0_top[u] : nullptr;
                if (stop) {
                    const int2 t = *reinterpret_cast<const int2 *>(stop + 2 * b);
                    lo = fe_load_f29(src, 2 * b, t.x);
                    hi = fe_load_f29(src, 2 * b + 1, t.y);
                } else {
                    lo = fe_from_fr(fr_load(src + 4 * b));
                    hi = fe_from_fr(fr_load(src + 4 * b + 2));
                }
                fr_store(dst + 2 * b, fe_to_fr(fe_add(lo, fe_mul_u<true>(fe_sub(hi, lo), r32))));
            }
            binds += 1;
            if (solo) {
                __syncthreads();
            } else if (!grid_barrier(A.sync, gen, Gj, bar_spins, A.sig + 1, A.sig0 + (uint32_t)j + 1u, stop_sh)) {
                return;
            }
        }
        if (threadIdx.x < (uint32_t)A.n_tables) tab_sh[threadIdx.x] = tab(threadIdx.x);
        __syncthreads();
        TAIL_STAMP(j, 1);
        if (solo) {
            const int shp = 63 - __builtin_clzll(n_pairs);
            const uint32_t items = (uint32_t)A.n_combos << shp;
            for (uint32_t i0 = 0; i0 < items; i0 += kBlock) {
                const uint32_t i = i0 + threadIdx.x;
                const bool live = i < items;
                const uint32_t ci = live ? (i >> shp) : 0;
                const Combo c = combo_sh[ci];
                const uint64_t b = i & (uint32_t)(n_pairs - 1);
                const int32_t nv = node_value((int)c.t);
                const Fr tf = node_constant(nv);
                Fr prod = fr_zero();
                if (live) {
                    if (c.M <= (uint32_t)kMaxFusedM) prod = fe_to_fr(combo_product_fe(tab_lds, c, slot_table_sh, slot_exp_sh, b, nv));
                    else prod = combo_product(tab_lds, c, slot_table_sh, slot_exp_sh, b, nv, tf);
                }
                for (uint32_t off = (uint32_t)n_pairs >> 1; off >= 1; off >>= 1) prod = fr_add(prod, fr_shfl_down(prod, (int)off));
                if (live && b == 0) fr_store(fin_lds + 2 * (prod_index_sh[ci] * A.D + (int)c.t), prod);
            }
            __syncthreads();
            TAIL_STAMP(j, 2);
            finalize_message<kBlock>(prod_of, A.Wm, A.K, A.D, fin_lds, (uint4 *)nullptr, (uint64_t *)nullptr, A.h_out, A.h_flag, A.seq0 + (uint32_t)j, 1, w_pre);
        } else {
            const uint32_t vgx = (uint32_t)((n_pairs + kBlock - 1) / kBlock);
            const uint32_t n_virtual = vgx * (uint32_t)A.n_combos;
            for (uint32_t v = blockIdx.x; v < n_virtual; v += Gj) {
                const uint32_t cy = v / vgx, vx = v % vgx;
                sum_combo_body(tab_lds, combo_sh[cy], slot_table_sh, slot_exp_sh, n_pairs, A.partials, sm, vx, vgx);
            }
            if (!grid_barrier(A.sync, gen, Gj, bar_spins, A.sig + 1, A.sig0 + (uint32_t)j + 1u, stop_sh)) return;
            TAIL_STAMP(j, 2);
            if (blockIdx.x == 0) {
                finalize_body<kBlock>(prod_of, A.Wm, A.K, A.D, (int)vgx, A.partials, fin_lds, (uint4 *)nullptr, (uint64_t *)nullptr, A.h_out, A.h_flag,
                                      A.seq0 + (uint32_t)j, 1, w_pre);
            }
        }
        TAIL_STAMP(j, 3);
        if (blockIdx.x == 0 && j + 1 < A.n_rounds) {
            const uint32_t want = A.sig0 + (uint32_t)(j + 1);
            if (threadIdx.x < 64) {
                const int lane = threadIdx.x;
                uint64_t w = 0;
                bool seen = false;
                for (uint32_t spin = 0; spin < A.max_spins; ++spin) {
                    if (lane < 8) w = __hip_atomic_load(A.mail_host + 8 * (want & 1u) + lane, __ATOMIC_RELAXED, __HIP_MEMORY_SCOPE_SYSTEM);
                    const bool mine = lane >= 8 || (uint32_t)w == want;
                    if (__all(mine)) { seen = true; break; }
                    if (__any(lane == 0 && (uint32_t)w == (want ^ 0x80000000u))) break;
                    __builtin_amdgcn_s_sleep(1);
                }
                if (!seen && lane == 0) {
                    __hip_atomic_store(A.sig + 1, want, __ATOMIC_RELEASE, __HIP_MEMORY_SCOPE_SYSTEM);
                    __hip_atomic_store(A.sync + 3, 1u, __ATOMIC_RELAXED, __HIP_MEMORY_SCOPE_AGENT);
                    stop_sh = 1;
                }
                const uint32_t lo32 = (uint32_t)(w >> 32);
                const uint32_t hi32 = __shfl_down(lo32, 1, 64);
                if (lane < 8 && (lane & 1) == 0) {
                    const uint64_t limb = (uint64_t)lo32 | ((uint64_t)hi32 << 32);
                    r_sh[lane >> 1] = limb;
                    __hip_atomic_store(A.chal + 4 * ((j + 1) & 1) + (lane >> 1), limb, __ATOMIC_RELAXED, __HIP_MEMORY_SCOPE_AGENT);
                }
                if (lane == 0) {
                    __builtin_amdgcn_fence(__ATOMIC_RELEASE, "agent");
                    __hip_atomic_store(A.sync + 2, (uint32_t)(j + 1), __ATOMIC_RELAXED, __HIP_MEMORY_SCOPE_AGENT);
                }
                TAIL_STAMP(j, 4);
// ... 300 lines not shown
                }
                __builtin_amdgcn_s_sleep(1);
            }
            sum += x & mask;
        }
    }
    __syncthreads();
    if (missing) {
        if (w == 0) __hip_atomic_store(h_flag, seq | kP2PRetryBit, __ATOMIC_RELEASE, __HIP_MEMORY_SCOPE_SYSTEM);
        return;
    }
    if (w < A.n_words) {
        lanes[w] = sum;
        h_dst[w] = sum;
    }
    __threadfence_system();
    __syncthreads();
    if (w == 0) __hip_atomic_store(h_flag, seq, __ATOMIC_RELEASE, __HIP_MEMORY_SCOPE_SYSTEM);
}
hipError_t launch_p2p_allreduce(const P2PArgs &args, uint64_t *d_lanes, uint64_t *h_dst_mapped, uint32_t *h_flag_mapped, uint32_t seq, hipStream_t stream) {
    if (args.n_words > kP2PWords || args.nranks > kP2PMaxRanks) return hipErrorInvalidValue;
    hipLaunchKernelGGL(k_p2p_allreduce, dim3(1), dim3(kP2PWords), 0, stream, args, d_lanes, h_dst_mapped, h_flag_mapped, seq);
    return hipGetLastError();
}

__global__ __launch_bounds__(kBlock) void k_sum_peer_lanes(const PeerLanes P, const uint64_t n_words, uint64_t *__restrict__ out) {
    for (uint64_t i = (uint64_t)blockIdx.x * kBlock + threadIdx.x; i < n_words; i += (uint64_t)gridDim.x * kBlock) {
        uint64_t s = 0;
        for (int q = 0; q < P.n; ++q) s += P.p[q][i];
        out[i] = s;
    }
}
hipError_t launch_sum_peer_lanes(const PeerLanes &peers, uint64_t n_words, uint64_t *out, hipStream_t stream) {
    const int grid = (int)std::min<uint64_t>((n_words + kBlock - 1) / kBlock, 2048);
    hipLaunchKernelGGL(k_sum_peer_lanes, dim3(std::max(grid, 1)), dim3(kBlock), 0, stream, peers, n_words, out);
    return hipGetLastError();
}

__global__ void k_gather_to_tables(const uint4 *__restrict__ recv, uint4 *__restrict__ tabs, const uint32_t G, const uint32_t U, const uint32_t per) {
    const uint64_t n = (uint64_t)G * U * per;
    for (uint64_t i = (uint64_t)blockIdx.x * blockDim.x + threadIdx.x; i < n; i += (uint64_t)gridDim.x * blockDim.x) {
        const uint32_t e = (uint32_t)(i % per);
        const uint64_t ug = i / per;
        const uint32_t g = (uint32_t)(ug % G), u = (uint32_t)(ug / G);
        const uint64_t src = ((uint64_t)g * U + u) * per + e;
        tabs[2 * i] = recv[2 * src];
        tabs[2 * i + 1] = recv[2 * src + 1];
    }
}
hipError_t launch_gather_to_tables(const uint4 *recv, uint4 *tabs, uint32_t G, uint32_t U, uint32_t per, hipStream_t stream) {
    const uint64_t n = (uint64_t)G * U * per;
    hipLaunchKernelGGL(k_gather_to_tables, dim3((unsigned)std::min<uint64_t>((n + 255) / 256, 2048)), dim3(256), 0, stream, recv, tabs, G, U, per);
    return hipGetLastError();
}

__global__ void k_msg_accumulate(const uint4 *__restrict__ in, uint4 *__restrict__ acc, const int D, const int first, const int last,
                                 uint4 *__restrict__ d_out, uint64_t *__restrict__ out_wide, uint4 *__restrict__ h_out, uint32_t *__restrict__ h_flag,
                                 const uint32_t seq) {
    const int t = threadIdx.x;
    if (t < D) {
        Fr a = fr_load(in + 2 * t);
        if (!first) a = fr_add(a, fr_load(acc + 2 * t));
        fr_store(acc + 2 * t, a);
        if (last) {
            if (d_out) fr_store(d_out + 2 * t, a);
            if (h_out) fr_store(h_out + 2 * t, a);
            if (out_wide)
                for (int j = 0; j < 8; ++j) out_wide[8 * t + j] = (uint64_t)a.v[j];
        }
    }
    if (last && h_flag) {
        __threadfence_system();
        __syncthreads();
        if (t == 0) __hip_atomic_store(h_flag, seq, __ATOMIC_RELEASE, __HIP_MEMORY_SCOPE_SYSTEM);
    }
}
hipError_t launch_msg_accumulate(const FrHost *in, FrHost *acc, int D, bool first, bool last, FrHost *d_out, uint64_t *d_out_wide, FrHost *h_out_mapped,
                                 uint32_t *h_flag_mapped, uint32_t seq, hipStream_t stream) {
    hipLaunchKernelGGL(k_msg_accumulate, dim3(1), dim3(64), 0, stream, (const uint4 *)in, (uint4 *)acc, D, first ? 1 : 0, last ? 1 : 0, (uint4 *)d_out,
                       d_out_wide, (uint4 *)h_out_mapped, h_flag_mapped, seq);
    return hipGetLastError();
}

hipError_t launch_f29_to_sat(const uint4 *src, const int32_t *src_top, uint4 *dst, uint64_t n, hipStream_t stream) {
    hipLaunchKernelGGL(k_f29_to_sat, dim3(grid_for_pairs(n)), dim3(kBlock), 0, stream, src, src_top, dst, n);
    return hipGetLastError();
}

hipError_t launch_fr_elementwise(int op, const uint4 *a, const uint4 *b, const FrHost &u, uint4 *out, uint64_t n, hipStream_t stream) {
    hipLaunchKernelGGL(k_fr_elementwise, dim3(grid_for_pairs(n)), dim3(kBlock), 0, stream, op, a, b, u, out, n);
    return hipGetLastError();
}

hipError_t launch_bench_modmul(uint64_t n_threads, uint32_t reps, uint32_t variant, uint64_t *d_sink, hipStream_t stream) {
    hipLaunchKernelGGL(k_bench_modmul, dim3((unsigned)((n_threads + kBlock - 1) / kBlock)), dim3(kBlock), 0, stream, reps, variant, d_sink);
    return hipGetLastError();
}

}

#ifdef SC_TAIL_CLOCKS
extern "C" __attribute__((visibility("default"))) int sc_debug_tail_clocks(uint64_t *out) {
    return (int)hipMemcpyFromSymbol(out, HIP_SYMBOL(scd::g_tail_clk), sizeof(uint64_t) * 64 * 8);
}
#endif
#ifdef SC_FIN_CLOCKS
extern "C" __attribute__((visibility("default"))) int sc_debug_fin_clocks(uint64_t *out) {
    return (int)hipMemcpyFromSymbol(out, HIP_SYMBOL(scd::g_fin_clk), sizeof(uint64_t) * 12);
}
#endif
```

### sumcheck_amd/csrc/kernels_big.hip

```cpp
#include "kernel_common.hpp"
#include "finalize_device.hpp"
#include "load_factor.hpp"

#include <algorithm>
#include <cstdlib>
#include <cstring>

namespace scd {

#ifdef SC_EXPERIMENTS
template <int M>
__global__ __launch_bounds__(kBlock) void k_prod_round(const ProdArgs A, const FrHost r_h, const uint64_t n_pairs,
                                                       uint4 *__restrict__ partials) {
    __shared__ uint32_t sm[kBlock / 64][8];
    const FrU r = fru_from_host(r_h);
    Fr acc[M + 1];
#pragma unroll
    for (int t = 0; t <= M; ++t) acc[t] = fr_zero();

    const uint64_t stride = (uint64_t)gridDim.x * kBlock;
    for (uint64_t b = (uint64_t)blockIdx.x * kBlock + threadIdx.x; b < n_pairs; b += stride) {
        Fr prod[M + 1];
        bool first = true;
        for (int s = 0; s < A.n_slots; ++s) {
// ... 594 lines not shown
#ifdef SC_EXPERIMENTS
__global__ __launch_bounds__(kBlock, 3) void k_round1_tree(const RoundArgs R, const uint64_t n_pairs, uint4 *__restrict__ partials) {
    __shared__ uint32_t sm[kBlock / 64][8];
    __shared__ int32_t rt[kBindLds];
    __shared__ int32_t lacc[9 * 5 * kBlock];
    const int n = R.n_prod;
    int k = (int)((blockIdx.x & 7u) % (uint32_t)n);
    for (int i = 0; i < n; ++i) {
        const TreeProd &T = R.prod[k];
        uint4 *row = partials + 2 * (T.partial_off + (uint64_t)blockIdx.x);
        switch (T.M) {
        case 1: tree_pass<1, true>(T.slot, rt, n_pairs, row, sm, lacc); break;
        case 2: tree_pass<2, true>(T.slot, rt, n_pairs, row, sm, lacc); break;
        case 3: tree_pass<3, true>(T.slot, rt, n_pairs, row, sm, lacc); break;
        default: tree_pass<4, true>(T.slot, rt, n_pairs, row, sm, lacc); break;
        }
        if (++k == n) k = 0;
    }
}
#endif

#ifdef SC_EXPERIMENTS
template <int M>
static hipError_t launch_prod_round_t(const ProdArgs &args, const FrHost &r, uint64_t n_pairs, FrHost *d_partials, int grid,
                                      hipStream_t stream) {
    hipLaunchKernelGGL(k_prod_round<M>, dim3(grid), dim3(kBlock), 0, stream, args, r, n_pairs, (uint4 *)d_partials);
    return hipGetLastError();
}

#endif

template <int M>
static hipError_t launch_prod_round_fe_t(const ProdArgs &args, const FrHost &r32, uint64_t n_pairs, FrHost *d_partials, int grid,
                                         hipStream_t stream) {
    hipLaunchKernelGGL(k_prod_round_fe<M>, dim3(grid), dim3(kBlock), 0, stream, args, r32, n_pairs, (uint4 *)d_partials);
    return hipGetLastError();
}

hipError_t launch_prod_round_fe(int M, const ProdArgs &args, const FrHost &r32, uint64_t n_pairs, FrHost *d_partials, int grid,
                                hipStream_t stream) {
    switch (M) {
    case 1: return launch_prod_round_fe_t<1>(args, r32, n_pairs, d_partials, grid, stream);
    case 2: return launch_prod_round_fe_t<2>(args, r32, n_pairs, d_partials, grid, stream);
    case 3: return launch_prod_round_fe_t<3>(args, r32, n_pairs, d_partials, grid, stream);
    case 4: return launch_prod_round_fe_t<4>(args, r32, n_pairs, d_partials, grid, stream);
    case 5: return launch_prod_round_fe_t<5>(args, r32, n_pairs, d_partials, grid, stream);
    case 6: return launch_prod_round_fe_t<6>(args, r32, n_pairs, d_partials, grid, stream);
    case 7: return launch_prod_round_fe_t<7>(args, r32, n_pairs, d_partials, grid, stream);
    case 8: return launch_prod_round_fe_t<8>(args, r32, n_pairs, d_partials, grid, stream);
    default: return hipErrorInvalidValue;
    }
}

template <int M>
static hipError_t launch_prod_tree_t(const ProdArgs &args, const BindConst &r32, uint64_t n_pairs, FrHost *d_partials, int grid,
                                     hipStream_t stream) {
    hipLaunchKernelGGL(k_prod_tree<M>, dim3(grid), dim3(kBlock), 0, stream, args, r32, n_pairs, (uint4 *)d_partials);
    return hipGetLastError();
}

hipError_t launch_prod_tree(int M, const ProdArgs &args, const BindConst &r32, uint64_t n_pairs, FrHost *d_partials, int grid,
                            hipStream_t stream) {
    switch (M) {
    case 1: return launch_prod_tree_t<1>(args, r32, n_pairs, d_partials, grid, stream);
    case 2: return launch_prod_tree_t<2>(args, r32, n_pairs, d_partials, grid, stream);
    case 3: return launch_prod_tree_t<3>(args, r32, n_pairs, d_partials, grid, stream);
    case 4: return launch_prod_tree_t<4>(args, r32, n_pairs, d_partials, grid, stream);
    default: return launch_prod_tree_wide(M, args, r32, n_pairs, d_partials, grid, stream);
    }
}

hipError_t launch_round_tree(const RoundArgs &args, const BindConst &r32, uint64_t n_pairs, FrHost *d_partials, int grid, hipStream_t stream, bool split,
                             bool skip1) {
    size_t extra_lds = 0;
#ifdef SC_EXPERIMENTS
    static const size_t env_lds = [] {
        const char *e = std::getenv("SC_EXTRA_LDS");
        return e ? (size_t)std::strtoul(e, nullptr, 10) : (size_t)0;
    }();
    extra_lds = env_lds;
#endif
    bool round1 = args.fin.enabled == 0;
    for (int q = 0; q < args.n_prod && round1; ++q)
        for (uint32_t f = 0; f < args.prod[q].M; ++f) round1 = round1 && args.prod[q].slot[f].mode == 0 && args.prod[q].slot[f].src_top == nullptr;
#ifdef SC_EXPERIMENTS
    if (!split) {
        if (skip1) return hipErrorInvalidValue;
        if (round1 && extra_lds == 0) hipLaunchKernelGGL(k_round1_tree, dim3(grid), dim3(kBlock), 0, stream, args, n_pairs, (uint4 *)d_partials);
        else hipLaunchKernelGGL(k_round_tree, dim3(grid), dim3(kBlock), extra_lds, stream, args, r32, n_pairs, (uint4 *)d_partials);
        return hipGetLastError();
    }
#else
    (void)split;
    (void)extra_lds;
#endif
#ifdef SC_NO_CHAIN_R2
    bool canonical_sources = false;
#else
    bool canonical_sources = !round1;
#endif
    for (int q = 0; q < args.n_prod && canonical_sources; ++q)
        for (uint32_t f = 0; f < args.prod[q].M; ++f) canonical_sources = canonical_sources && args.prod[q].slot[f].src_top == nullptr;
    const dim3 g(grid, args.n_prod), b(kBlock);
    uint4 *const part = (uint4 *)d_partials;
    plan_hit(round1 ? kPlanBigMergedRound1 : canonical_sources ? kPlanBigMergedBindChain : kPlanBigMergedBind);
    if (skip1) plan_hit(kPlanBigClaimIdentity);
    if (round1) {
        if (skip1) return hipErrorInvalidValue;
        hipLaunchKernelGGL(k_round1_tree_split, g, b, 0, stream, args, n_pairs, part);
    } else if (canonical_sources) {
        if (skip1) hipLaunchKernelGGL((k_round_tree_split<true, true>), g, b, 0, stream, args, r32, n_pairs, part);
        else hipLaunchKernelGGL((k_round_tree_split<true, false>), g, b, 0, stream, args, r32, n_pairs, part);
    } else {
        if (skip1) hipLaunchKernelGGL((k_round_tree_split<kChainDefault, true>), g, b, 0, stream, args, r32, n_pairs, part);
        else hipLaunchKernelGGL((k_round_tree_split<kChainDefault, false>), g, b, 0, stream, args, r32, n_pairs, part);
    }
    return hipGetLastError();
}

#ifdef SC_EXPERIMENTS
template <int M>
static hipError_t launch_round_tile_t(const ProdArgs &args, const FrHost &r32, uint64_t n_pairs, FrHost *d_partials, int grid,
                                      hipStream_t stream) {
    hipLaunchKernelGGL(k_round_tile<M>, dim3(grid), dim3(64 * (M + 1)), 0, stream, args, r32, n_pairs, (uint4 *)d_partials);
    return hipGetLastError();
}

int grid_for_tiles(uint64_t n_pairs) {
    uint64_t g = (n_pairs + kTilePairs - 1) / kTilePairs;
    if (g < 1) g = 1;
    if (g > (uint64_t)kMaxGrid) g = kMaxGrid;
    return (int)g;
}

hipError_t launch_round_tile(int M, const ProdArgs &args, const FrHost &r32, uint64_t n_pairs, FrHost *d_partials, int grid,
                             hipStream_t stream) {
    switch (M) {
    case 1: return launch_round_tile_t<1>(args, r32, n_pairs, d_partials, grid, stream);
    case 2: return launch_round_tile_t<2>(args, r32, n_pairs, d_partials, grid, stream);
    case 3: return launch_round_tile_t<3>(args, r32, n_pairs, d_partials, grid, stream);
    case 4: return launch_round_tile_t<4>(args, r32, n_pairs, d_partials, grid, stream);
    case 5: return launch_round_tile_t<5>(args, r32, n_pairs, d_partials, grid, stream);
    case 6: return launch_round_tile_t<6>(args, r32, n_pairs, d_partials, grid, stream);
    case 7: return launch_round_tile_t<7>(args, r32, n_pairs, d_partials, grid, stream);
    case 8: return launch_round_tile_t<8>(args, r32, n_pairs, d_partials, grid, stream);
    default: return hipErrorInvalidValue;
    }
}

hipError_t launch_prod_round(int M, const ProdArgs &args, const FrHost &r, uint64_t n_pairs, FrHost *d_partials, int grid,
                             hipStream_t stream) {
    switch (M) {
    case 1: return launch_prod_round_t<1>(args, r, n_pairs, d_partials, grid, stream);
    case 2: return launch_prod_round_t<2>(args, r, n_pairs, d_partials, grid, stream);
    case 3: return launch_prod_round_t<3>(args, r, n_pairs, d_partials, grid, stream);
    case 4: return launch_prod_round_t<4>(args, r, n_pairs, d_partials, grid, stream);
    case 5: return launch_prod_round_t<5>(args, r, n_pairs, d_partials, grid, stream);
    case 6: return launch_prod_round_t<6>(args, r, n_pairs, d_partials, grid, stream);
    case 7: return launch_prod_round_t<7>(args, r, n_pairs, d_partials, grid, stream);
    case 8: return launch_prod_round_t<8>(args, r, n_pairs, d_partials, grid, stream);
    default: return hipErrorInvalidValue;
    }
}

#endif

}
```

### sumcheck_amd/csrc/kernels_selftest.hip

```cpp
#include <hip/hip_runtime.h>
#include "batch_round.hpp"
#include "host_fr.hpp"
#include "wide_cell.hpp"
#include "wide_tree.hpp"

void make_bind_const(const sch::Fr &r, scd::BindConst &rc);

namespace scd {

enum FeOp : int {
    kOpNormalize = 0,
    kOpCarryPass = 1,
    kOpToFr = 2,
    kOpRoundTrip = 3,
    kOpFromFr = 4,
    kOpMul = 5,
    kOpMulChain = 6,
    kOpMulU = 7,
    kOpMulUChain = 8,
    kOpMul2 = 9,
    kOpMul2Chain = 10,
    kOpBind = 11,
    kOpBindChain = 12,
    kOpShl5MulU = 13,
    kOpLine = 14,
    kOpAccum = 15,
    kOpFoldCell = 16,
    kOpWideValue = 17,
    kOpWideExt = 18,
};

__device__ __forceinline__ Fe st_load(const int32_t *p, const uint64_t i) {
    Fe r;
#pragma unroll
    for (int l = 0; l < 9; ++l) r.l[l] = p[9 * i + l];
    return r;
}
__device__ __forceinline__ Fr st_load_fr(const int32_t *p, const uint64_t i) {
    Fr r;
#pragma unroll
    for (int l = 0; l < 8; ++l) r.v[l] = (uint32_t)p[9 * i + l];
    return r;
}
__device__ __forceinline__ void st_store(int32_t *p, const uint64_t i, const Fe &v) {
#pragma unroll
    for (int l = 0; l < 9; ++l) p[9 * i + l] = v.l[l];
}
__device__ __forceinline__ void st_store_fr(int32_t *p, const uint64_t i, const Fr &v) {
#pragma unroll
    for (int l = 0; l < 8; ++l) p[9 * i + l] = (int32_t)v.v[l];
    p[9 * i + 8] = 0;
}
__device__ __forceinline__ FeU st_feu_lane(const Fe &b, const int lane) {
    FeU u;
#pragma unroll
    for (int l = 0; l < 9; ++l) u.l[l] = __builtin_amdgcn_readlane(b.l[l], lane);
    return u;
}

template <int kOp>
__global__ __launch_bounds__(kTsBlock) void k_fe_op(const int32_t *__restrict__ a, const int32_t *__restrict__ b, const int32_t *__restrict__ c,
                                                    const int32_t *__restrict__ d, const uint64_t *__restrict__ aux, const BindConst C, const int64_t p0,
                                                    const int64_t p1, const int64_t p2, int32_t *__restrict__ out, const uint64_t n) {
    __shared__ int32_t rt[kBindLds];
    const uint64_t gid = (uint64_t)blockIdx.x * kTsBlock + threadIdx.x;
    const bool live = gid < n;
    const uint64_t i = live ? gid : n - 1;
    if constexpr (kOp == kOpBind || kOp == kOpBindChain) bind_consts_to_lds(C, rt);
    if constexpr (kOp == kOpNormalize) {
        const Fe r = fe_normalize(st_load(a, i));
        if (live) st_store(out, i, r);
    } else if constexpr (kOp == kOpCarryPass) {
        const Fe r = fe_carry_pass(st_load(a, i));
        if (live) st_store(out, i, r);
    } else if constexpr (kOp == kOpToFr) {
        const Fr r = fe_to_fr(st_load(a, i));
        if (live) st_store_fr(out, i, r);
    } else if constexpr (kOp == kOpRoundTrip) {
        const Fr r = fe_to_fr(fe_from_fr(st_load_fr(a, i)));
        if (live) st_store_fr(out, i, r);
    } else if constexpr (kOp == kOpFromFr) {
        const Fe r = fe_from_fr(st_load_fr(a, i));
        if (live) st_store(out, i, r);
    } else if constexpr (kOp == kOpMul || kOp == kOpMulChain) {
        const Fe r = fe_mul<kOp == kOpMulChain>(st_load(a, i), st_load(b, i));
        if (live) st_store(out, i, r);
    } else if constexpr (kOp == kOpMulU || kOp == kOpMulUChain || kOp == kOpShl5MulU) {
        const Fe x = st_load(a, i);
        Fe y = st_load(b, i), r = fe_zero();
        const int me = threadIdx.x & 63;
#pragma unroll 1
        for (int lane = 0; lane < 64; ++lane) {
            const FeU raw = st_feu_lane(y, lane);
            Fe t;
            if constexpr (kOp == kOpShl5MulU) {
                uint32_t w[8];
#pragma unroll
                for (int l = 0; l < 8; ++l) w[l] = (uint32_t)raw.l[l];
                t = fe_mul_u<true>(x, feu_shl5(w));
            } else {
                t = fe_mul_u<kOp == kOpMulUChain>(x, raw);
            }
            if (lane == me) r = t;
        }
        if (live) st_store(out, i, r);
    } else if constexpr (kOp == kOpMul2 || kOp == kOpMul2Chain) {
        const Fe r = fe_mul2_sum<kOp == kOpMul2Chain>(st_load(a, i), st_load(b, i), st_load(c, i), st_load(d, i));
        if (live) st_store(out, i, r);
    } else if constexpr (kOp == kOpBind || kOp == kOpBindChain) {
        const Fe r = fe_mul_bind<kOp == kOpBindChain>(st_load(a, i), rt);
        if (live) st_store(out, i, r);
    } else if constexpr (kOp == kOpLine) {
        const Fe r = fe_line(st_load(a, i), st_load(b, i), (int32_t)p0);
        if (live) st_store(out, i, r);
    } else if constexpr (kOp == kOpAccum) {
        const uint32_t per_lane = (uint32_t)p0, L = (uint32_t)p1, pairs = per_lane * L;
        const uint64_t group = gid / L;
        const Fe r = bt_combo_sum(true, (uint32_t)(gid % L), (int)L, pairs, lazy_sum_needs_reduce(pairs, (uint32_t)p2),
                                  [&](const uint32_t pr) -> Fe { return st_load(a, group * pairs + pr); });
        st_store(out, gid, r);
    } else if constexpr (kOp == kOpFoldCell) {
        uint64_t lane[8];
#pragma unroll
        for (int l = 0; l < 8; ++l) lane[l] = aux[4 + 8 * i + l];
        const Fr r = wide_fold_cell(lane);
        if (live) st_store_fr(out, i, r);
    }
}

template <int m, int t>
__global__ __launch_bounds__(kTsBlock) void k_wide_value_op(const int32_t *__restrict__ a, int32_t *__restrict__ out, const uint64_t n) {
    const uint64_t i = (uint64_t)blockIdx.x * kTsBlock + threadIdx.x;
    if (i >= n) return;
    Fe v[5];
#pragma unroll
    for (int s = 0; s < 5; ++s) v[s] = st_load(a, 5 * i + s);
    if constexpr (m == 1) st_store(out, i, fe_comb5(v, 1 - node_value(t), node_value(t), 0, 0, 0));
    else st_store(out, i, wide_value<m, t>(v));
}
template <int m, int t>
__global__ __launch_bounds__(kTsBlock) void k_wide_ext_op(const int32_t *__restrict__ a, int32_t *__restrict__ out, const uint64_t n) {
    const uint64_t i = (uint64_t)blockIdx.x * kTsBlock + threadIdx.x;
    if (i >= n) return;
    Fe v[9];
#pragma unroll
    for (int s = 0; s < 9; ++s) v[s] = st_load(a, 9 * i + s);
    st_store(out, i, wide_ext<m, t>(v));
}

}

extern "C" __attribute__((visibility("default"))) int sc_debug_fe_op(int op, const int32_t *a, const int32_t *b, const int32_t *c, const int32_t *d,
                                                                     const uint64_t *aux, int32_t *out, uint64_t n) {
    using namespace scd;
    if (n == 0 || a == nullptr || out == nullptr || aux == nullptr || n > (1ULL << 24)) return -2;
    uint64_t par[4];
    hipError_t e = hipMemcpy(par, aux, sizeof(par), hipMemcpyDeviceToHost);
    if (e != hipSuccess) return (int)e;
    const dim3 grid((unsigned)((n + kTsBlock - 1) / kTsBlock)), block(kTsBlock);
    BindConst C;
    std::memset(&C, 0, sizeof(C));
    if (op == kOpBind || op == kOpBindChain) {
        const sch::Fr r = {{par[0], par[1], par[2], par[3]}};
        if (sch::geq_p(r)) return -2;
        make_bind_const(r, C);
    }
    if (op == kOpAccum) {
        const uint64_t L = par[1];
        if (par[0] == 0 || par[0] > 64 || L == 0 || L > 64 || (L & (L - 1)) != 0 || n % kTsBlock != 0) return -2;
    }
    if ((op >= kOpMul && op <= kOpMul2Chain) || op == kOpShl5MulU || op == kOpLine) {
        if (b == nullptr) return -2;
    }
    if ((op == kOpMul2 || op == kOpMul2Chain) && (c == nullptr || d == nullptr)) return -2;
    const int64_t p0 = (int64_t)par[0], p1 = (int64_t)par[1], p2 = (int64_t)par[2];
#define SC_FE_OP(OP)                                                                                                    \
    case OP:                                                                                                            \
        hipLaunchKernelGGL(k_fe_op<OP>, grid, block, 0, 0, a, b, c, d, aux, C, p0, p1, p2, out, n);                        \
        break;
#define SC_WIDE_OP(KERNEL, M, T)                                                                                        \
    if (p0 == M && p1 == T) {                                                                                           \
        hipLaunchKernelGGL((KERNEL<M, T>), grid, block, 0, 0, a, out, n);                                               \
        found = true;                                                                                                   \
    }
    bool found = false;
    switch (op) {
        SC_FE_OP(kOpNormalize)
        SC_FE_OP(kOpCarryPass)
        SC_FE_OP(kOpToFr)
        SC_FE_OP(kOpRoundTrip)
        SC_FE_OP(kOpFromFr)
        SC_FE_OP(kOpMul)
        SC_FE_OP(kOpMulChain)
        SC_FE_OP(kOpMulU)
        SC_FE_OP(kOpMulUChain)
        SC_FE_OP(kOpMul2)
        SC_FE_OP(kOpMul2Chain)
        SC_FE_OP(kOpBind)
        SC_FE_OP(kOpBindChain)
        SC_FE_OP(kOpShl5MulU)
        SC_FE_OP(kOpLine)
        SC_FE_OP(kOpAccum)
        SC_FE_OP(kOpFoldCell)
    case kOpWideValue:
        SC_WIDE_OP(k_wide_value_op, 4, 5) SC_WIDE_OP(k_wide_value_op, 4, 6) SC_WIDE_OP(k_wide_value_op, 4, 7) SC_WIDE_OP(k_wide_value_op, 4, 8)
        SC_WIDE_OP(k_wide_value_op, 3, 4) SC_WIDE_OP(k_wide_value_op, 3, 5) SC_WIDE_OP(k_wide_value_op, 3, 6) SC_WIDE_OP(k_wide_value_op, 3, 7)
        SC_WIDE_OP(k_wide_value_op, 2, 3) SC_WIDE_OP(k_wide_value_op, 2, 4) SC_WIDE_OP(k_wide_value_op, 2, 5) SC_WIDE_OP(k_wide_value_op, 2, 6)
        SC_WIDE_OP(k_wide_value_op, 1, 3) SC_WIDE_OP(k_wide_value_op, 1, 4) SC_WIDE_OP(k_wide_value_op, 1, 5)
        if (!found) return -1;
        break;
    case kOpWideExt:
        SC_WIDE_OP(k_wide_ext_op, 8, 9) SC_WIDE_OP(k_wide_ext_op, 8, 10) SC_WIDE_OP(k_wide_ext_op, 8, 11) SC_WIDE_OP(k_wide_ext_op, 8, 12)
        SC_WIDE_OP(k_wide_ext_op, 1, 3) SC_WIDE_OP(k_wide_ext_op, 1, 4) SC_WIDE_OP(k_wide_ext_op, 1, 5) SC_WIDE_OP(k_wide_ext_op, 1, 6)
        SC_WIDE_OP(k_wide_ext_op, 1, 7) SC_WIDE_OP(k_wide_ext_op, 1, 8) SC_WIDE_OP(k_wide_ext_op, 1, 9)
        SC_WIDE_OP(k_wide_ext_op, 2, 3) SC_WIDE_OP(k_wide_ext_op, 2, 4) SC_WIDE_OP(k_wide_ext_op, 2, 5) SC_WIDE_OP(k_wide_ext_op, 2, 6)
        SC_WIDE_OP(k_wide_ext_op, 2, 7) SC_WIDE_OP(k_wide_ext_op, 2, 8) SC_WIDE_OP(k_wide_ext_op, 2, 9) SC_WIDE_OP(k_wide_ext_op, 2, 10)
        SC_WIDE_OP(k_wide_ext_op, 3, 4) SC_WIDE_OP(k_wide_ext_op, 3, 5) SC_WIDE_OP(k_wide_ext_op, 3, 6) SC_WIDE_OP(k_wide_ext_op, 3, 7)
        SC_WIDE_OP(k_wide_ext_op, 3, 8) SC_WIDE_OP(k_wide_ext_op, 3, 9) SC_WIDE_OP(k_wide_ext_op, 3, 10) SC_WIDE_OP(k_wide_ext_op, 3, 11)
        SC_WIDE_OP(k_wide_ext_op, 4, 5) SC_WIDE_OP(k_wide_ext_op, 4, 6) SC_WIDE_OP(k_wide_ext_op, 4, 7) SC_WIDE_OP(k_wide_ext_op, 4, 8)
        SC_WIDE_OP(k_wide_ext_op, 4, 9) SC_WIDE_OP(k_wide_ext_op, 4, 10) SC_WIDE_OP(k_wide_ext_op, 4, 11) SC_WIDE_OP(k_wide_ext_op, 4, 12)
        if (!found) return -1;
        break;
    default:
        return -1;
    }
#undef SC_FE_OP
#undef SC_WIDE_OP
    e = hipGetLastError();
    if (e != hipSuccess) return (int)e;
    return (int)hipDeviceSynchronize();
}
```

### sumcheck_amd/csrc/kernels_tail.hip

```cpp
#include "finalize_device.hpp"
#include "kernel_common.hpp"

#include <algorithm>

namespace scd {

constexpr uint32_t kTsStop = 3;

constexpr int kTsEnt = 12;
__device__ __forceinline__ Fe ts_lds_load(const int32_t *t) {
    const int4 a = *reinterpret_cast<const int4 *>(t), b = *reinterpret_cast<const int4 *>(t + 4), c = *reinterpret_cast<const int4 *>(t + 8);
    Fe r;
    r.l[0] = a.x; r.l[1] = a.y; r.l[2] = a.z; r.l[3] = a.w;
    r.l[4] = b.x; r.l[5] = b.y; r.l[6] = b.z; r.l[7] = b.w;
    r.l[8] = c.x;
    return r;
}
__device__ __forceinline__ void ts_lds_store(int32_t *t, const Fe &v) {
    *reinterpret_cast<int4 *>(t) = make_int4(v.l[0], v.l[1], v.l[2], v.l[3]);
    *reinterpret_cast<int4 *>(t + 4) = make_int4(v.l[4], v.l[5], v.l[6], v.l[7]);
    t[8] = v.l[8];
}
__device__ __forceinline__ Fe fe_shfl_down(const Fe &a, const int off) {
    Fe r;
// ... 66 lines not shown
    const Combo my_c = combo_sh[combo_live ? my_combo : 0];
    const int32_t my_nv = node_value((int)my_c.t);
    uint32_t my_base[kSlots], my_exp[kSlots];
#pragma unroll
    for (int sl = 0; sl < kSlots; ++sl) {
        const bool in = (uint32_t)sl < my_c.n_slots;
        my_base[sl] = in ? slot_table_sh[my_c.slot_off + sl] * cap : 0u;
        my_exp[sl] = in ? slot_exp_sh[my_c.slot_off + sl] : 0u;
    }

    uint64_t n_pairs = A.first_pairs;
    uint32_t E = 0;
    int binds = 0;
    for (int j = 0; j < A.n_rounds; ++j, n_pairs >>= 1) {
        const uint32_t tag = S.tag0 + (uint32_t)j;
        const bool has_bind = j > 0 || A.first_has_bind;
        TS_STAMP(j, 0);
        if (has_bind) {
            if (j == 0) {
                if (tid < 4) r_sh[tid] = A.r0.l[tid];
            } else if (tid < 64) {
                const uint32_t want = A.sig0 + (uint32_t)j;
                uint64_t w = 0;
                bool seen = false;
                if (S.mail_vram) {
                    for (uint32_t spin = 0; spin < 8 * A.max_spins; ++spin) {
                        if (tid < 8) w = __hip_atomic_load(S.mail_vram + 8 * (want & 1u) + tid, __ATOMIC_RELAXED, __HIP_MEMORY_SCOPE_SYSTEM);
                        const bool mine = tid >= 8 || (uint32_t)w == want;
                        if (__all(mine)) { seen = true; break; }
                        if ((spin & 255u) == 255u && __hip_atomic_load(stop_word, __ATOMIC_RELAXED, __HIP_MEMORY_SCOPE_AGENT) != 0) break;
                        __builtin_amdgcn_s_sleep(1);
                    }
                } else if (g == 0) {
                    for (uint32_t spin = 0; spin < A.max_spins; ++spin) {
                        if (tid < 8) w = __hip_atomic_load(A.mail_host + 8 * (want & 1u) + tid, __ATOMIC_RELAXED, __HIP_MEMORY_SCOPE_SYSTEM);
                        const bool mine = tid >= 8 || (uint32_t)w == want;
                        if (__all(mine)) { seen = true; break; }
                        if (__any(tid == 0 && (uint32_t)w == (want ^ 0x80000000u))) break;
                        __builtin_amdgcn_s_sleep(1);
                    }
                    if (B > 1) {
                        const uint32_t limb = (uint32_t)(w >> 32);
                        const uint32_t a = __shfl(limb, 2 * (tid & 3), 64), b2 = __shfl(limb, 2 * (tid & 3) + 1, 64);
                        if (seen && tid < 4) ts_store_pair(xrs, (uint32_t)(kTsXwWords - 8) + 2 * (uint32_t)tid, a, b2, tag);
                    }
                } else {
                    const uint64_t *bc = S.xw + kTsXwWords - 8;
                    for (uint32_t spin = 0; spin < wait_spins; ++spin) {
                        if (tid < 8) w = __hip_atomic_load(bc + tid, __ATOMIC_RELAXED, __HIP_MEMORY_SCOPE_AGENT);
                        const bool mine = tid >= 8 || (uint32_t)(w >> 32) == tag;
                        if (__all(mine)) { seen = true; break; }
                        if ((spin & 31u) == 31u && __hip_atomic_load(stop_word, __ATOMIC_RELAXED, __HIP_MEMORY_SCOPE_AGENT) != 0) break;
                        __builtin_amdgcn_s_sleep(1);
                    }
                    w <<= 32;
                }
                if (!seen && tid == 0) {
                    give_up(want);
                    stop_sh = 1;
                }
                const uint32_t lo32 = (uint32_t)(w >> 32);
                const uint32_t hi32 = __shfl_down(lo32, 1, 64);
                if (tid < 8 && (tid & 1) == 0) r_sh[tid >> 1] = (uint64_t)lo32 | ((uint64_t)hi32 << 32);
            }
            __syncthreads();
            if (stop_sh) break;
        }
        TS_STAMP(j, 1);
        FeU r32;
        if (has_bind) {
            FrHost rh;
#pragma unroll
            for (int i = 0; i < 4; ++i) rh.l[i] = r_sh[i];
            r32 = feu_shl5(fru_from_host(rh).v);
        }
        if (j == 0) {
            E = (uint32_t)((2 * n_pairs) / B);
            const uint32_t total = E * (uint32_t)U;
            const int shE = 31 - __builtin_clz(E);
            for (uint32_t i = tid; i < total; i += kTsBlock) {
                const uint32_t u = i >> shE, e = i & (E - 1);
                const uint64_t ge = (uint64_t)g * E + e;
                const uint4 *src = A.t.cur0[u];
                const int32_t *stop = A.t.cur0_top[u];
                Fe v;
                if (has_bind) {
                    Fe lo, hi;
                    if (stop) {
                        const int2 t = *reinterpret_cast<const int2 *>(stop + 2 * ge);
                        lo = fe_load_f29(src, 2 * ge, t.x);
                        hi = fe_load_f29(src, 2 * ge + 1, t.y);
                    } else {
                        lo = fe_from_fr(fr_load(src + 4 * ge));
                        hi = fe_from_fr(fr_load(src + 4 * ge + 2));
                    }
                    v = fe_carry_pass(fe_add(lo, fe_mul_u<true>(fe_sub(hi, lo), r32)));
                } else {
                    v = stop ? fe_load_f29(src, ge, stop[ge]) : fe_from_fr(fr_load(src + 2 * ge));
                }
                ts_lds_store(tab_at((int)u, e), v);
            }
            if (has_bind) binds += 1;
            __syncthreads();
        } else {
            const uint32_t half = E / 2, total = half * (uint32_t)U;
            const int shH = 31 - __builtin_clz(half);
            for (uint32_t i0 = 0; i0 < total; i0 += kTsBlock) {
                const uint32_t i = i0 + tid;
                const bool live = i < total;
                const uint32_t u = live ? i >> shH : 0, e = live ? i & (half - 1) : 0;
                Fe v = fe_zero();
                if (live) {
                    const Fe lo = ts_lds_load(tab_at((int)u, 2 * e)), hi = ts_lds_load(tab_at((int)u, 2 * e + 1));
                    v = fe_carry_pass(fe_add(lo, fe_mul_u<true>(fe_sub(hi, lo), r32)));
                }
                __syncthreads();
                if (live) ts_lds_store(tab_at((int)u, e), v);
            }
            E = half;
            binds += 1;
            __syncthreads();
        }
        if (B > 1 && E == 1) {
            const uint32_t R = B < 16u ? B : 16u;
            const int shR = 31 - __builtin_clz(R);
            for (int i = tid; i < U * 5; i += kTsBlock) {
                const int u = i / 5, pr = i % 5;
                const int32_t *e0 = tab_at(u, 0);
                ts_store_pair(xrs, (uint32_t)kTsAccWords + ((uint32_t)u * B + g) * 10 + 2 * (uint32_t)pr, (uint32_t)e0[2 * pr], pr < 4 ? (uint32_t)e0[2 * pr + 1] : 0u, tag);
            }
            if ((g & (R - 1)) != 0) return;
            __syncthreads();
            bool ok = true;
            constexpr int kXferBatch = 12;
            const uint32_t per_table = R * 5, total_p = (uint32_t)U * per_table;
            for (uint32_t c0 = 0; c0 < total_p && ok; c0 += kXferBatch * kTsBlock) {
                ts_v4 w[kXferBatch];
                bool got = false;
                for (uint32_t spins = 0; spins <= wait_spins && !got; ++spins) {
                    got = true;
#pragma unroll
                    for (int k = 0; k < kXferBatch; ++k) {
                        if (c0 + (uint32_t)k * kTsBlock < total_p) {
                            const uint32_t i = min(c0 + (uint32_t)k * kTsBlock + (uint32_t)tid, total_p - 1);
                            const uint32_t ent = i / 5, pr = i - 5 * ent;
                            w[k] = ts_load_pair(xrs, (uint32_t)kTsAccWords + ((ent >> shR) * B + g + (ent & (R - 1))) * 10 + 2 * pr);
                        }
                    }
#pragma unroll
                    for (int k = 0; k < kXferBatch; ++k)
                        if (c0 + (uint32_t)k * kTsBlock < total_p) got = got && w[k].y == tag && w[k].w == tag;
                    if (!got) {
                        if ((spins & 63u) == 63u && __hip_atomic_load(stop_word, __ATOMIC_RELAXED, __HIP_MEMORY_SCOPE_AGENT) != 0) break;
                        __builtin_amdgcn_s_sleep(1);
                    }
                }
                ok = got;
#pragma unroll
                for (int k = 0; k < kXferBatch; ++k) {
                    if (c0 + (uint32_t)k * kTsBlock < total_p) {
                        const uint32_t i = min(c0 + (uint32_t)k * kTsBlock + (uint32_t)tid, total_p - 1);
                        const uint32_t ent = i / 5, pr = i - 5 * ent;
                        int32_t *dst = tab_at((int)(ent >> shR), ent & (R - 1));
                        dst[2 * pr] = (int32_t)w[k].x;
                        if (pr < 4) dst[2 * pr + 1] = (int32_t)w[k].z;
                    }
                }
            }
            if (!ok) stop_sh = 1;
            __syncthreads();
            if (stop_sh) {
                if (tid == 0) give_up(A.sig0 + (uint32_t)j + 1u);
                return;
            }
            E = R;
            g >>= shR;
            B >>= shR;
        }
        TS_STAMP(j, 2);
        const uint32_t pairs_here = E / 2;
        Fe acc = fe_zero();
// ... 211 lines not shown
```

### sumcheck_amd/csrc/load_factor.hpp

```cpp
#pragma once
#include "kernel_common.hpp"

namespace scd {

template <int F, bool kR1 = false, bool kChain = kChainDefault>
struct LoadFactor {
    static __device__ __forceinline__ void run(const Slot *S, const uint64_t b, const int32_t (&r)[kBindLds], Fe &lo_out, Fe &hi_out) {
        const Slot &sl = S[F];
        if constexpr (kR1) {
            const uint4 *p = sl.src + 4 * b;
            lo_out = fe_from_fr(fr_load(p));
            hi_out = fe_from_fr(fr_load(p + 2));
            return;
        }
        const uint32_t mode = sl.mode;
        const int32_t *stop = sl.src_top;
        if (mode == 0) {
            const uint4 *p = sl.src + 4 * b;
            if (stop) {
                const int2 t = *reinterpret_cast<const int2 *>(stop + 2 * b);
                lo_out = fe_load_f29(sl.src, 2 * b, t.x);
                hi_out = fe_load_f29(sl.src, 2 * b + 1, t.y);
            } else {
                lo_out = fe_from_fr(fr_load(p));
                hi_out = fe_from_fr(fr_load(p + 2));
            }
        } else {
            const uint4 *p = sl.src + 8 * b;
            Fe e0, e1, e2, e3;
            if (stop) {
                const int4 t = *reinterpret_cast<const int4 *>(stop + 4 * b);
                const uint4 *m = sl.src;
                e0 = fe_load_f29(m, 4 * b, t.x); e1 = fe_load_f29(m, 4 * b + 1, t.y);
                e2 = fe_load_f29(m, 4 * b + 2, t.z); e3 = fe_load_f29(m, 4 * b + 3, t.w);
            } else {
                e0 = fe_from_fr(fr_load(p)); e1 = fe_from_fr(fr_load(p + 2)); e2 = fe_from_fr(fr_load(p + 4)); e3 = fe_from_fr(fr_load(p + 6));
            }
            const Fe l0 = fe_add(e0, fe_mul_bind<kChain>(fe_sub(e1, e0), r));
            asm volatile("" : "+v"(e3.l[8]) : "v"(l0.l[8]));
            const Fe h0 = fe_add(e2, fe_mul_bind<kChain>(fe_sub(e3, e2), r));
            if (sl.dst_top || (mode == 3 && stop)) {
                lo_out = fe_carry_pass(l0);
                hi_out = fe_carry_pass(h0);
                if (mode == 1) {
                    fe_store_f29(sl.dst, 2 * b, lo_out);
                    fe_store_f29(sl.dst, 2 * b + 1, hi_out);
                    *reinterpret_cast<int2 *>(sl.dst_top + 2 * b) = make_int2(lo_out.l[8], hi_out.l[8]);
                }
            } else {
                const Fr lc = fe_to_fr(l0), hc = fe_to_fr(h0);
                if (mode == 1) {
                    uint4 *q = sl.dst + 4 * b;
                    fr_store(q, lc);
                    fr_store(q + 2, hc);
                }
                lo_out = fe_from_fr(lc);
                hi_out = fe_from_fr(hc);
            }
        }
    }
};


}
```

### sumcheck_amd/csrc/protocol.hip

```cpp
#include "prover_internal.hpp"

uint64_t small_pairs_limit() {
#ifdef SC_EXPERIMENTS
    static const uint64_t v = [] {
        const char *e = std::getenv("SC_SMALL_LOG2");
        return e ? (1ULL << std::atoi(e)) : scd::kSmallRoundPairs;
    }();
    return v;
#else
    return scd::kSmallRoundPairs;
#endif
}

bool launches_are_async(sc_prover *p) {
    static const bool ok = [p] {
        uint32_t *h = nullptr, *d = nullptr;
        FrHost *dm = nullptr;
        if (hipHostMalloc(reinterpret_cast<void **>(&h), 256, hipHostMallocMapped | hipHostMallocCoherent) != hipSuccess) return false;
        bool good = hipHostGetDevicePointer(reinterpret_cast<void **>(&d), h, 0) == hipSuccess &&
                    hipMalloc(reinterpret_cast<void **>(&dm), sizeof(FrHost)) == hipSuccess;
        if (good) {
            std::memset(h, 0, 256);
            good = scd::launch_wait_challenge(d, 0xffffffffu, reinterpret_cast<const FrHost *>(d + 16), dm, p->stream, 1) == hipSuccess &&
                   hipStreamSynchronize(p->stream) == hipSuccess;
// ... 84 lines not shown
    if (p->deferred_pending) {
        __atomic_store_n(p->sig, p->sig_seq, __ATOMIC_RELEASE);
        p->deferred_pending = false;
        (void)hipStreamSynchronize(p->stream);
        p->exhausted = true;
    }
}

void make_bind_const(const sch::Fr &r, scd::BindConst &rc) {
    static const std::array<sch::Fr, 9> pow2 = [] {
        std::array<sch::Fr, 9> t;
        sch::Fr c = sch::kOne;
        for (int d = 0; d < 58; ++d) c = sch::add(c, c);
        for (int i = 0; i < 9; ++i) {
            t[i] = c;
            for (int d = 0; d < 29; ++d) c = sch::add(c, c);
        }
        return t;
    }();
    for (int i = 0; i < 9; ++i) {
        const sch::Fr x = sch::to_canonical(sch::mul(r, pow2[i]));
        for (int k = 0; k < 9; ++k) {
            const int bit = 29 * k, w = bit >> 6, sh = bit & 63;
            uint64_t v = x.l[w] >> sh;
            if (sh > 35 && w < 3) v |= x.l[w + 1] << (64 - sh);
            rc.R[i][k] = (int32_t)(v & 0x1fffffffULL);
        }
    }
}

int launch_round_streamed(sc_prover *p, const uint64_t *r_or_null, uint64_t *d_wide, bool publish_to_host) {
    scd::plan_hit(scd::kPlanBigStreamed);
    if (p->exhausted) return sc_internal_fail(SC_ERR_NOT_ACTIVE, "Prover is not active");
    if (r_or_null && p->round == 0) return sc_internal_fail(SC_ERR_FIRST_ROUND_HAS_MSG, "first round should be prover first.");
    if (!r_or_null && p->round > 0) return sc_internal_fail(SC_ERR_MISSING_MSG, "verifier message is empty");
    sch::Fr r = sch::zero();
    if (r_or_null) {
        std::memcpy(&r, r_or_null, 32);
        if (sch::geq_p(r)) return sc_internal_fail(SC_ERR_BAD_ARG, "challenge is not a canonical field element");
    }
    HIP_TRY(hipSetDevice(p->device));
    int rc_t = collect_timing(p);
    if (rc_t) return rc_t;
    const bool bind = r_or_null != nullptr;
    if (bind) p->randomness.push_back(r);
    p->round += 1;
    scd::BindConst rc;
    std::memset(&rc, 0, sizeof(rc));
    if (bind) make_bind_const(r, rc);
    const uint64_t C = 1ULL << p->chunk_log2, n = 1ULL << p->nv, n_chunks = n / C;
    const uint64_t pairs_per_chunk = bind ? C / 4 : C / 2;
    const bool merged = p->merge_rounds && !p->any_generic;
    const int grid = merged ? std::min(scd::grid_for_pairs(pairs_per_chunk), scd::kRoundTreeGrid) : scd::grid_for_pairs(pairs_per_chunk);
    sch::Fr r32v = sch::zero();
    const FrHost r32 = to_dev(r32v);
    p->seq += 1;
    for (uint64_t c = 0; c < n_chunks; ++c) {
        const int q = (int)(c & 1);
        if (c >= 2) HIP_TRY(hipStreamWaitEvent(p->copy_stream, p->ev_consumed[q], 0));
        for (uint32_t u = 0; u < p->U; ++u)
            HIP_TRY(hipMemcpyAsync(static_cast<char *>(p->ring[q]) + (((size_t)u << p->chunk_log2) * 32), p->host_tabs[u] + 4 * c * C, C * 32, hipMemcpyHostToDevice,
                                   p->copy_stream));
        HIP_TRY(hipEventRecord(p->ev_copied[q], p->copy_stream));
        HIP_TRY(hipStreamWaitEvent(p->stream, p->ev_copied[q], 0));
        auto ring_tab = [&](uint32_t u) { return reinterpret_cast<const uint4 *>(static_cast<char *>(p->ring[q]) + (((size_t)u << p->chunk_log2) * 32)); };
        if (merged) {
            scd::RoundArgs ra;
            std::memset(&ra, 0, sizeof(ra));
            ra.n_prod = (int)p->K;
            std::vector<uint8_t> bound(p->U, 0);
            for (uint32_t k = 0; k < p->K; ++k) {
                const Product &pr = p->prods[k];
                scd::TreeProd &tp = ra.prod[k];
                tp.M = pr.M;
                tp.partial_off = pr.partial_off;
                int f = 0;
                for (size_t s = 0; s < pr.tables.size(); ++s) {
                    const uint32_t u = pr.tables[s];
                    Table &t = p->tabs[u];
                    for (uint32_t rep = 0; rep < pr.exps[s]; ++rep, ++f) {
                        scd::Slot &sl = tp.slot[f];
                        sl.exp = 1;
                        sl.src = ring_tab(u);
                        sl.src_top = nullptr;
                        if (!bind) {
                            sl.mode = 0;
                        } else if (!bound[u]) {
                            sl.mode = 1;
                            sl.dst = t.buf[0] + 2 * (c * (C / 2));
                            sl.dst_top = p->use_f29 ? t.buf_top[0] + c * (C / 2) : nullptr;
                            bound[u] = 1;
                        } else {
                            sl.mode = 3;
                            sl.dst_top = p->use_f29 ? t.buf_top[0] : nullptr;
                        }
                    }
                }
            }
            HIP_TRY(scd::launch_round_tree(ra, rc, pairs_per_chunk, p->d_partials, grid, p->stream, true));
            if (bind) {
                for (uint32_t u = 0; u < p->U; ++u)
                    if (!bound[u]) HIP_TRY(scd::launch_fix(ring_tab(u), p->tabs[u].buf[0] + 2 * (c * (C / 2)), to_dev(r), C / 2, p->stream));
            }
        } else {
            std::vector<const uint4 *> src(p->U);
            for (uint32_t u = 0; u < p->U; ++u) {
                if (bind) {
                    uint4 *dst = p->tabs[u].buf[0] + 2 * (c * (C / 2));
                    HIP_TRY(scd::launch_fix(ring_tab(u), dst, to_dev(r), C / 2, p->stream));
                    src[u] = dst;
                } else {
                    src[u] = ring_tab(u);
                }
            }
            bool ptrs_uploaded = false;
            for (uint32_t k = 0; k < p->K; ++k) {
                const Product &pr = p->prods[k];
                FrHost *partials = p->d_partials + pr.partial_off;
                ProdArgs a;
                std::memset(&a, 0, sizeof(a));
                if (pr.fused && p->kernel_variant == 3 && pr.M <= 4) {
                    a.n_slots = (int)pr.M;
                    int f = 0;
                    for (size_t s2 = 0; s2 < pr.tables.size(); ++s2)
                        for (uint32_t rep = 0; rep < pr.exps[s2]; ++rep, ++f) {
                            a.slot[f].exp = 1;
                            a.slot[f].mode = 0;
                            a.slot[f].src = src[pr.tables[s2]];
                        }
                    HIP_TRY(scd::launch_prod_tree((int)pr.M, a, rc, pairs_per_chunk, partials, grid, p->stream));
                } else if (pr.fused) {
                    a.n_slots = (int)pr.tables.size();
                    for (size_t s2 = 0; s2 < pr.tables.size(); ++s2) {
                        a.slot[s2].exp = pr.exps[s2];
                        a.slot[s2].mode = 0;
                        a.slot[s2].src = src[pr.tables[s2]];
                    }
                    HIP_TRY(scd::launch_prod_round_fe((int)pr.M, a, r32, pairs_per_chunk, partials, grid, p->stream));
                } else {
                    if (!ptrs_uploaded) {
                        const uint4 **h = p->h_cur_tables + (size_t)q * p->U;
                        if (c >= 2) HIP_TRY(hipEventSynchronize(p->ev_consumed[q]));
                        for (uint32_t u = 0; u < p->U; ++u) h[u] = src[u];
                        HIP_TRY(hipMemcpyAsync(p->d_cur_tables + (size_t)q * p->U, h, p->U * sizeof(void *), hipMemcpyHostToDevice, p->stream));
                        ptrs_uploaded = true;
                    }
                    HIP_TRY(scd::launch_sum_generic(p->d_cur_tables + (size_t)q * p->U, p->d_slot_table + pr.slot_off, p->d_slot_exp + pr.slot_off, (int)pr.tables.size(),
                                                    (int)pr.M, pairs_per_chunk, partials, grid, p->stream));
                }
            }
        }
        HIP_TRY(scd::launch_finalize(p->d_finprods, p->h_finprods.empty() ? nullptr : p->h_finprods.data(), p->d_W, (int)p->K, (int)p->D, grid, p->d_partials,
                                     p->d_scratch, p->d_chunk_msg, nullptr, nullptr, nullptr, 0, 1, p->d_fin_mb_counter, p->stream));
        const bool last = c + 1 == n_chunks;
        HIP_TRY(scd::launch_msg_accumulate(p->d_chunk_msg, p->d_chunk_msg + p->D, (int)p->D, c == 0, last, p->d_out, last ? d_wide : nullptr,
                                           (last && publish_to_host) ? p->h_out_dev : nullptr, (last && publish_to_host) ? p->h_flag_dev : nullptr, p->seq, p->stream));
        HIP_TRY(hipEventRecord(p->ev_consumed[q], p->stream));
    }
    if (bind) {
        for (uint32_t u = 0; u < p->U; ++u) {
            Table &t = p->tabs[u];
            bool referenced = false;
            for (const Product &pr : p->prods)
                for (uint32_t tt : pr.tables) referenced |= tt == u;
            t.cur = t.buf[0];
            t.cur_top = (merged && p->use_f29 && referenced) ? t.buf_top[0] : nullptr;
            t.next = 1;
        }
    }
    p->timed = false;
    p->timing_pending = false;
    return SC_OK;
}

struct SlowCallProbe {
    const char *what;
    std::chrono::steady_clock::time_point t0;
    bool on;
    explicit SlowCallProbe(const char *w) : what(w), on(std::getenv("SC_HOST_TRACE") != nullptr) {
        if (on) t0 = std::chrono::steady_clock::now();
    }
    ~SlowCallProbe() {
        if (!on) return;
        const double ms = std::chrono::duration<double, std::milli>(std::chrono::steady_clock::now() - t0).count();
        if (ms > 1.0) std::fprintf(stderr, "[sc] slow host call: %s took %.1f ms\n", what, ms);
    }
};
bool fin_mb_enabled();
bool staged_init_applies(const sc_prover *p) {
    return scd::policy(scd::kPolStagedInit) != 0 && p->merge_rounds && !p->any_generic && !p->streamed && !p->borrow && !p->fused_finalize && p->kernel_variant == 3 &&
           p->nv >= 18 && p->K > 0 && p->K <= (uint32_t)scd::kMetaProds;
}
int staged_copy_and_round1(sc_prover *p, const uint64_t *const *host_tables) {
    HIP_TRY(hipSetDevice(p->device));
    if (!p->copy_stream) HIP_TRY(hipStreamCreateWithFlags(&p->copy_stream, hipStreamNonBlocking));
    if (!p->copy_stream2) HIP_TRY(hipStreamCreateWithFlags(&p->copy_stream2, hipStreamNonBlocking));
    for (int q = 0; q < 2; ++q) {
        if (!p->ev_copied[q]) HIP_TRY(hipEventCreateWithFlags(&p->ev_copied[q], hipEventDisableTiming));
        if (!p->ev_copied2[q]) HIP_TRY(hipEventCreateWithFlags(&p->ev_copied2[q], hipEventDisableTiming));
    }
    const uint64_t n = 1ULL << p->nv, n_pairs = n >> 1;
    int G = n_pairs >= (1ULL << 21) ? 1024 : n_pairs >= (1ULL << 20) ? 768 : n_pairs >= (1ULL << 18) ? 384 : n_pairs >= (1ULL << 17) ? 256 : 192;
    if (p->K == 1) G = std::min(G, scd::kRoundTreeGrid);
    G = std::min(G, scd::grid_for_pairs(n_pairs));
    int levels = p->nv >= 21 ? 5 : 2;
    int sec[6], n_chunks = levels + 1;
    if (levels == 5 && G % 8 == 0) {
        sec[0] = G / 4, sec[1] = G / 8, sec[2] = G / 8;
        sec[3] = G / 8, sec[4] = G / 8, sec[5] = G / 4;
    } else {
        levels = 2;
        while (levels > 0 && (G % (1 << levels)) != 0) --levels;
        n_chunks = levels + 1;
        for (int c = 0; c < n_chunks; ++c) sec[c] = G >> (c < levels ? c + 1 : levels);
    }
    for (uint32_t u = 0; u < p->U; ++u)
        if (!host_tables[u]) return sc_internal_fail(SC_ERR_BAD_ARG, "table %u is null", u);
    scd::BindConst rc;
    std::memset(&rc, 0, sizeof(rc));
    HIP_TRY(hipEventRecord(p->ev_copied[1], p->stream));
    HIP_TRY(hipStreamWaitEvent(p->copy_stream, p->ev_copied[1], 0));
    HIP_TRY(hipStreamWaitEvent(p->copy_stream2, p->ev_copied[1], 0));
    int block0 = 0;
    for (int c = 0; c < n_chunks; ++c) {
        const int sh = c < levels ? c + 1 : levels;
        const uint64_t chunk = n >> sh, first = n - (n >> c);
        const int gc = sec[c];
        for (uint32_t u = 0; u < p->U; ++u) {
            HIP_TRY(hipMemcpyAsync(reinterpret_cast<char *>(p->tabs[u].buf[0]) + (size_t)first * 32, reinterpret_cast<const char *>(host_tables[u]) + (size_t)first * 32,
                                   (size_t)chunk * 32, hipMemcpyHostToDevice, (u & 1) ? p->copy_stream2 : p->copy_stream));
        }
        HIP_TRY(hipEventRecord(p->ev_copied[c & 1], p->copy_stream));
        HIP_TRY(hipStreamWaitEvent(p->stream, p->ev_copied[c & 1], 0));
        if (p->U > 1) {
            HIP_TRY(hipEventRecord(p->ev_copied2[c & 1], p->copy_stream2));
            HIP_TRY(hipStreamWaitEvent(p->stream, p->ev_copied2[c & 1], 0));
        }
        scd::RoundArgs ra;
        std::memset(&ra, 0, sizeof(ra));
        ra.n_prod = (int)p->K;
        for (uint32_t k = 0; k < p->K; ++k) {
            const Product &pr = p->prods[k];
            scd::TreeProd &tp = ra.prod[k];
            tp.M = pr.M;
            tp.partial_off = pr.partial_off;
            int f = 0;
            for (size_t s2 = 0; s2 < pr.tables.size(); ++s2)
                for (uint32_t rep = 0; rep < pr.exps[s2]; ++rep, ++f) {
                    tp.slot[f].exp = 1;
// ... 33 lines not shown
    if (p->round + 1 > p->nv) return sc_internal_fail(SC_ERR_NOT_ACTIVE, "Prover is not active");
    sch::Fr r = sch::zero();
    if (r_or_null) {
        std::memcpy(&r, r_or_null, 32);
        if (sch::geq_p(r)) return sc_internal_fail(SC_ERR_BAD_ARG, "challenge is not a canonical field element");
    }
    if (deferred) {
        const uint64_t np = 1ULL << (p->nv - (p->round + 1));
        if (!(np <= small_pairs_limit() && p->U <= (uint32_t)scd::kMaxSmallTables && p->K > 0)) return sc_internal_fail(SC_ERR_BAD_ARG, "only late rounds are pipelined");
    }
    HIP_TRY(hipSetDevice(p->device));
    if (!deferred) {
        int rc_t = collect_timing(p);
        if (rc_t) return rc_t;
    }
    if (p->r1_cached) {
        p->r1_cached = false;
        if (p->round == 0 && !r_or_null && !deferred && !d_wide && publish_to_host) {
            p->round = 1;
            p->seq += 1;
            p->sums_round = p->r1_keeps ? 1 : -1;
            p->timed = false;
            p->timing_pending = false;
            p->prod_timed = false;
            return SC_OK;
        }
    }
    bool bind = r_or_null != nullptr || deferred;
    if (r_or_null) p->randomness.push_back(r);
    p->round += 1;
    const uint64_t n_pairs = 1ULL << (p->nv - p->round);
    const FrHost rdev = to_dev(r);
    sch::Fr r32v = r;
    for (int d = 0; d < 5; ++d) r32v = sch::add(r32v, r32v);
    const FrHost r32 = to_dev(r32v);
    int scaled = 0;
    const uint64_t small_pairs = small_pairs_limit();
    const bool small_round = n_pairs <= small_pairs && p->K > 0 && (p->U <= (uint32_t)scd::kMaxSmallTables || p->d_cur_tables != nullptr);
#ifdef SC_EXPERIMENTS
    const bool tiled = !small_round && !p->any_generic && p->kernel_variant == 2;
#else
    const bool tiled = false;
    (void)tiled;
#endif
    scd::BindConst rc;
    std::memset(&rc, 0, sizeof(rc));
    if (bind && !small_round && p->kernel_variant == 3) make_bind_const(r, rc);
    int grid = scd::grid_for_pairs(n_pairs);
#ifdef SC_EXPERIMENTS
    if (tiled) grid = scd::grid_for_tiles(n_pairs);
#endif
    const bool timed = p->timing && !deferred;
    if (timed) HIP_TRY(hipEventRecord(p->ev0, p->stream));
    const FrHost *r_mail = nullptr;
    if (deferred) {
        p->sig_seq += 1;
        {
            SlowCallProbe pr("launch k_wait_challenge");
            HIP_TRY(scd::launch_wait_challenge(p->sig_dev, p->sig_seq, p->h_mail_dev + (p->sig_seq & 1u), p->d_mail + (p->sig_seq & 1u), p->stream));
        }
        r_mail = p->d_mail + (p->sig_seq & 1u);
        p->deferred_pending = true;
    }

    auto bind_table = [&](uint32_t u) -> hipError_t {
        Table &t = p->tabs[u];
        uint4 *dst = t.buf[t.next];
        hipError_t e = scd::launch_fix(t.cur, dst, rdev, 2 * n_pairs, p->stream);
        t.cur = dst;
        t.next ^= 1;
        return e;
    };

    const bool small = small_round;
    if (small) {
        TablePtrs tp;
        if (bind) {
            for (uint32_t u0 = 0; u0 < p->U; u0 += (uint32_t)scd::kMaxSmallTables) {
                const uint32_t cnt = std::min<uint32_t>(p->U - u0, (uint32_t)scd::kMaxSmallTables);
                std::memset(&tp, 0, sizeof(tp));
                for (uint32_t j = 0; j < cnt; ++j) {
                    Table &t = p->tabs[u0 + j];
                    tp.src[j] = t.cur;
                    tp.src_top[j] = t.cur_top;
                    tp.dst[j] = t.buf[t.next];
                }
                {
                    SlowCallProbe pr("launch k_fix_multi");
                    HIP_TRY(scd::launch_fix_multi(tp, (int)cnt, rdev, r_mail, 2 * n_pairs, p->stream));
                }
                for (uint32_t j = 0; j < cnt; ++j) {
                    Table &t = p->tabs[u0 + j];
                    t.cur = t.buf[t.next];
                    t.cur_top = nullptr;
                    t.next ^= 1;
                }
            }
        }
        SlowCallProbe pr_sum("launch k_sum_combos");
        scd::plan_hit(deferred ? scd::kPlanSmallPipelined : p->U > (uint32_t)scd::kMaxSmallTables ? scd::kPlanSmallPtrs : p->has_meta ? scd::kPlanSmallLaunched : scd::kPlanSmallCombosTable);
        if (p->U <= (uint32_t)scd::kMaxSmallTables) {
            std::memset(&tp, 0, sizeof(tp));
            for (uint32_t u = 0; u < p->U; ++u) tp.src[u] = p->tabs[u].cur;
            if (p->has_meta) HIP_TRY(scd::launch_sum_combos_meta(tp, p->meta, p->n_combos, n_pairs, p->d_partials, grid, p->stream));
            else HIP_TRY(scd::launch_sum_combos(tp, p->d_combos, p->n_combos, p->d_slot_table, p->d_slot_exp, n_pairs, p->d_partials, grid, p->stream));
        } else {
            for (uint32_t u = 0; u < p->U; ++u) p->h_cur_tables[u] = p->tabs[u].cur;
            HIP_TRY(hipMemcpyAsync(p->d_cur_tables, p->h_cur_tables, p->U * sizeof(void *), hipMemcpyHostToDevice, p->stream));
            HIP_TRY(scd::launch_sum_combos_ptrs(p->d_cur_tables, p->d_combos, p->n_combos, p->d_slot_table, p->d_slot_exp, n_pairs, p->d_partials, grid, p->stream));
        }
        scaled = 1;
        bind = false;
    }
    if (bind && p->any_generic) {
        scd::plan_hit(scd::kPlanBigBindPass);
        for (uint32_t u0 = 0; u0 < p->U; u0 += (uint32_t)scd::kMaxSmallTables) {
            const uint32_t cnt = std::min<uint32_t>(p->U - u0, (uint32_t)scd::kMaxSmallTables);
            TablePtrs tp;
            std::memset(&tp, 0, sizeof(tp));
            for (uint32_t j = 0; j < cnt; ++j) {
                Table &t = p->tabs[u0 + j];
                tp.src[j] = t.cur;
                tp.src_top[j] = t.cur_top;
                tp.dst[j] = t.buf[t.next];
            }
            HIP_TRY(scd::launch_fix_multi(tp, (int)cnt, rdev, nullptr, 2 * n_pairs, p->stream));
            for (uint32_t j = 0; j < cnt; ++j) {
                Table &t = p->tabs[u0 + j];
                t.cur = t.buf[t.next];
                t.cur_top = nullptr;
                t.next ^= 1;
            }
        }
        bind = false;
    }
    std::vector<uint8_t> bound(p->U, 0);
    bool ptrs_uploaded = false;
    bool finalized = false;
    bool skip1 = false;
    const bool merged = !small && p->merge_rounds && !p->any_generic;
    if (merged) {
        grid = std::min(grid, scd::kRoundTreeGrid);
        bool split = !p->fused_finalize;
        int split_grid = n_pairs >= (1ULL << 21) ? 1024 : n_pairs >= (1ULL << 20) ? 768 : n_pairs >= (1ULL << 18) ? 384 : n_pairs >= (1ULL << 17) ? 256 : 192;
#ifdef SC_EXPERIMENTS
        static const bool split_off = std::getenv("SC_SPLIT") && std::atoi(std::getenv("SC_SPLIT")) == 0;
        static const int split_cap = std::getenv("SC_SPLIT_GRID") ? std::atoi(std::getenv("SC_SPLIT_GRID")) : 0;
        if (split_off) split = false;
        if (split_cap > 0) split_grid = split_cap;
#endif
#ifndef SC_NO_KGRID
        if (p->K < 4 && n_pairs < (1ULL << 21)) split_grid = std::min(scd::kMaxGrid, split_grid * 4 / (int)p->K);
        else if (p->K == 1) split_grid = std::min(split_grid, scd::kRoundTreeGrid);
#else
        if (p->K == 1) split_grid = std::min(split_grid, scd::kRoundTreeGrid);
#endif
        if (split) grid = std::min(scd::grid_for_pairs(n_pairs), split_grid);
        skip1 = bind && split && p->sums_round == (int64_t)p->round - 1 && skip1_enabled() &&
                scd::finalize_keeps_sums((int)p->K, (int)p->D, grid, !p->h_finprods.empty(), fin_mb_enabled());
        scd::RoundArgs ra;
        std::memset(&ra, 0, sizeof(ra));
        ra.n_prod = (int)p->K;
        std::vector<const uint4 *> old_src(p->U);
        std::vector<const int32_t *> old_top(p->U);
        for (uint32_t u = 0; u < p->U; ++u) {
            old_src[u] = p->tabs[u].cur;
            old_top[u] = p->tabs[u].cur_top;
        }
        for (uint32_t k = 0; k < p->K; ++k) {
            const Product &pr = p->prods[k];
            scd::TreeProd &tp = ra.prod[k];
            tp.M = pr.M;
            tp.partial_off = pr.partial_off;
            int f = 0;
            for (size_t s = 0; s < pr.tables.size(); ++s) {
                const uint32_t u = pr.tables[s];
                Table &t = p->tabs[u];
                for (uint32_t rep = 0; rep < pr.exps[s]; ++rep, ++f) {
                    scd::Slot &sl = tp.slot[f];
                    sl.exp = 1;
                    sl.src = old_src[u];
                    sl.src_top = old_top[u];
                    if (!bind) {
                        sl.mode = 0;
                    } else if (!bound[u]) {
                        sl.mode = 1;
                        sl.dst = t.buf[t.next];
                        sl.dst_top = p->use_f29 ? t.buf_top[t.next] : nullptr;
                        t.cur = t.buf[t.next];
                        t.cur_top = sl.dst_top;
                        t.next ^= 1;
                        bound[u] = 1;
                    } else {
                        sl.mode = 3;
                        sl.dst_top = p->use_f29 ? t.buf_top[0] : nullptr;
                    }
                }
            }
        }
        p->seq += 1;
        ra.fin.enabled = p->fused_finalize ? 1 : 0;
        ra.fin.D = (int)p->D;
        for (uint32_t k = 0; k < p->K; ++k) ra.fin.w_off[k] = p->h_finprods[k].w_off;
        ra.fin.Wm = reinterpret_cast<const uint4 *>(p->d_W);
        ra.fin.partials2 = reinterpret_cast<uint4 *>(p->d_partials2);
        ra.fin.counters = p->d_fin_counters;
        ra.fin.out = reinterpret_cast<uint4 *>(p->d_out);
        ra.fin.out_wide = d_wide;
        ra.fin.h_out = publish_to_host ? reinterpret_cast<uint4 *>(p->h_out_dev) : nullptr;
        ra.fin.h_flag = publish_to_host ? p->h_flag_dev : nullptr;
        ra.fin.seq = p->seq;
        if (p->timing) HIP_TRY(hipEventRecord(p->prod_ev[0], p->stream));
        if (bind) scd::plan_hit(p->use_f29 ? scd::kPlanBigF29Store : scd::kPlanBigCanonicalStore);
        HIP_TRY(scd::launch_round_tree(ra, rc, n_pairs, p->d_partials, grid, p->stream, split, skip1));
        if (p->timing) HIP_TRY(hipEventRecord(p->prod_ev[1], p->stream));
        scaled = 1;
        if (p->fused_finalize) finalized = true;
        else p->seq -= 1;
    }
    for (uint32_t k = 0; k < p->K && !small && !merged; ++k) {
        const Product &pr = p->prods[k];
        FrHost *partials = p->d_partials + pr.partial_off;
        if (p->timing) HIP_TRY(hipEventRecord(p->prod_ev[2 * k], p->stream));
        if (pr.fused && p->kernel_variant == 3 && (pr.M <= 4 || p->wide_tree)) {
            ProdArgs a;
            std::memset(&a, 0, sizeof(a));
            a.n_slots = (int)pr.M;
            int f = 0;
            for (size_t s = 0; s < pr.tables.size(); ++s) {
                Table &t = p->tabs[pr.tables[s]];
                const uint4 *old_src = t.cur;
                const int32_t *old_top = t.cur_top;
                bool stored_here = false;
                for (uint32_t rep = 0; rep < pr.exps[s]; ++rep, ++f) {
                    a.slot[f].exp = 1;
                    if (bind && !bound[pr.tables[s]]) {
                        a.slot[f].mode = 1;
                        a.slot[f].src = old_src;
                        a.slot[f].src_top = old_top;
                        a.slot[f].dst = t.buf[t.next];
                        a.slot[f].dst_top = p->use_f29 ? t.buf_top[t.next] : nullptr;
                        t.cur = t.buf[t.next];
                        t.cur_top = a.slot[f].dst_top;
                        t.next ^= 1;
                        bound[pr.tables[s]] = 1;
                        stored_here = true;
                    } else if (stored_here) {
                        a.slot[f].mode = 3;
                        a.slot[f].src = old_src;
                        a.slot[f].src_top = old_top;
                        a.slot[f].dst = nullptr;
                        a.slot[f].dst_top = p->use_f29 ? t.buf_top[0] : nullptr;
                    } else {
                        a.slot[f].mode = 0;
                        a.slot[f].src = t.cur;
                        a.slot[f].src_top = t.cur_top;
                        a.slot[f].dst = nullptr;
                    }
                }
            }
            scd::plan_hit(pr.M <= 4 ? scd::kPlanBigPerProductTree : scd::kPlanBigWide);
            if (bind) scd::plan_hit(p->use_f29 ? scd::kPlanBigF29Store : scd::kPlanBigCanonicalStore);
            HIP_TRY(scd::launch_prod_tree((int)pr.M, a, rc, n_pairs, partials, grid, p->stream));
            scaled = 1;
        } else if (pr.fused) {
            ProdArgs a;
            std::memset(&a, 0, sizeof(a));
            a.n_slots = (int)pr.tables.size();
            for (size_t s = 0; s < pr.tables.size(); ++s) {
                Table &t = p->tabs[pr.tables[s]];
                a.slot[s].exp = pr.exps[s];
                if (bind && !bound[pr.tables[s]]) {
                    a.slot[s].mode = 1;
                    a.slot[s].src = t.cur;
                    a.slot[s].dst = t.buf[t.next];
                    t.cur = t.buf[t.next];
                    t.next ^= 1;
                    bound[pr.tables[s]] = 1;
                } else {
                    a.slot[s].mode = 0;
                    a.slot[s].src = t.cur;
                    a.slot[s].dst = nullptr;
                }
            }
#ifdef SC_EXPERIMENTS
            if (tiled) {
                HIP_TRY(scd::launch_round_tile((int)pr.M, a, r32, n_pairs, partials, grid, p->stream));
                scaled = 1;
            } else if (!p->use_fe) {
                HIP_TRY(scd::launch_prod_round((int)pr.M, a, rdev, n_pairs, partials, grid, p->stream));
            } else
#endif
            {
                scd::plan_hit(scd::kPlanBigNodeByNode);
                HIP_TRY(scd::launch_prod_round_fe((int)pr.M, a, r32, n_pairs, partials, grid, p->stream));
                scaled = 1;
            }
        } else if (pr.M <= (uint32_t)scd::kMaxWideM && p->wide_tree && p->kernel_variant == 3) {
            scd::WideArgs16 a;
            std::memset(&a, 0, sizeof(a));
            const std::vector<uint32_t> &factors = p->prod_indices[k];
            a.n_slots = (int)factors.size();
            for (size_t f = 0; f < factors.size(); ++f) {
                const Table &t = p->tabs[factors[f]];
                a.slot[f].mode = 0;
                a.slot[f].exp = 1;
                a.slot[f].src = t.cur;
                a.slot[f].src_top = t.cur_top;
            }
            sch::Fr comp = sch::kOne;
            for (uint32_t dbl = 0; dbl < 5 * (pr.M - 1); ++dbl) comp = sch::add(comp, comp);
            scd::plan_hit(scd::kPlanBigWide16);
            HIP_TRY(scd::launch_prod_tree_wide16((int)pr.M, a, to_dev(comp), n_pairs, partials, grid, p->stream));
        } else {
            if (!ptrs_uploaded) {
                for (uint32_t u = 0; u < p->U; ++u) p->h_cur_tables[u] = p->tabs[u].cur;
                HIP_TRY(hipMemcpyAsync(p->d_cur_tables, p->h_cur_tables, p->U * sizeof(void *), hipMemcpyHostToDevice, p->stream));
                ptrs_uploaded = true;
            }
            scd::plan_hit(scd::kPlanBigGeneric);
            HIP_TRY(scd::launch_sum_generic(p->d_cur_tables, p->d_slot_table + pr.slot_off, p->d_slot_exp + pr.slot_off,
                                            (int)pr.tables.size(), (int)pr.M, n_pairs, partials, grid, p->stream));
        }
        if (p->timing) HIP_TRY(hipEventRecord(p->prod_ev[2 * k + 1], p->stream));
    }
    if (bind) {
        for (uint32_t u = 0; u < p->U; ++u)
            if (!bound[u]) HIP_TRY(bind_table(u));
    }
    if (!finalized) {
    p->seq += 1;
    const bool keeps = scd::finalize_keeps_sums((int)p->K, (int)p->D, grid, !p->h_finprods.empty(), fin_mb_enabled());
    scd::ClaimArgs ca;
    std::memset(&ca, 0, sizeof(ca));
    if (skip1) {
        ca.skip1 = 1;
        ca.prev = reinterpret_cast<const uint4 *>(p->d_sums[(p->round - 1) & 1]);
        bool done[5] = {false, false, false, false, false};
        for (uint32_t k = 0; k < p->K; ++k) {
            const uint32_t M = p->prods[k].M;
            if (done[M]) continue;
            done[M] = true;
            sch::Fr lam[5];
            claim_weights(M, r, lam);
            for (uint32_t s2 = 0; s2 <= M; ++s2) ca.lam[scd::claim_off((int)M) + (int)s2] = to_dev(lam[s2]);
        }
    }
    SlowCallProbe pr_fin("launch k_finalize");
    HIP_TRY(scd::launch_finalize(p->d_finprods, p->h_finprods.empty() ? nullptr : p->h_finprods.data(), p->d_W, (int)p->K, (int)p->D, grid, p->d_partials,
                                 keeps ? p->d_sums[p->round & 1] : p->d_scratch, p->d_out, d_wide,
                                 publish_to_host ? p->h_out_dev : nullptr, publish_to_host ? p->h_flag_dev : nullptr,
                                 (p->wide_tagged && d_wide) ? p->wide_gen : p->seq,
                                 scaled | ((p->wide_tagged && d_wide) ? 2 : 0), fin_mb_enabled() ? p->d_fin_mb_counter : nullptr, p->stream, skip1 ? &ca : nullptr));
    p->sums_round = keeps && merged ? (int64_t)p->round : -1;
    }
    if (timed) HIP_TRY(hipEventRecord(p->ev1, p->stream));
    if (!deferred) {
        p->timed = timed;
        p->timing_pending = timed;
        p->prod_timed = timed && !small;
        p->prod_merged = merged;
        p->timed_round = p->round;
    }
    return SC_OK;
}

int await_round(sc_prover *p, uint64_t *out_evals, uint32_t want);

int resident_start(sc_prover *p, const uint64_t *r_or_null, uint64_t *out_evals);
int resident_round(sc_prover *p, const uint64_t *r_or_null, uint64_t *out_evals);
extern "C" int sc_prove_round(sc_prover *p, const uint64_t *r_or_null, uint64_t *out_evals) {
    if (!p || !out_evals) return sc_internal_fail(SC_ERR_BAD_ARG, "null argument");
    int rc = p->res.active ? resident_round(p, r_or_null, out_evals) : resident_start(p, r_or_null, out_evals);
    if (rc != kResidentGone) return rc;
    rc = launch_round(p, r_or_null, nullptr, true);
    if (rc) return rc;
    return await_round(p, out_evals, p->seq);
}

int await_round(sc_prover *p, uint64_t *out_evals, const uint32_t want) {
    uint64_t spins = 0;
    bool seen = false;
    const auto t_start = std::chrono::steady_clock::now();
    while (!(seen = (__atomic_load_n(p->h_flag, __ATOMIC_ACQUIRE) == want))) {
        if ((++spins & 0xfff) == 0) {
            if (std::chrono::steady_clock::now() - t_start > std::chrono::seconds(2)) break;
        }
    }
    if (!seen) {
        if (p->deferred_pending) {
            abandon_deferred(p);
// ... 4 lines not shown
            HIP_TRY(hipStreamSynchronize(p->stream));
        }
        if (__atomic_load_n(p->h_flag, __ATOMIC_ACQUIRE) != want) return sc_internal_fail(SC_ERR_HIP, "round finished without publishing its message");
    }
    if (wait_gave_up(p)) {
        if (std::getenv("SC_HOST_TRACE"))
            std::fprintf(stderr, "[sc] give-up seen in await_round: marker %u, sig word %u, sig_seq %u, awaited seq %u, h_flag %u, round %u, deferred_pending %d, waited %.3f s\n",
                         __atomic_load_n(p->sig + 1, __ATOMIC_ACQUIRE), __atomic_load_n(p->sig, __ATOMIC_ACQUIRE), p->sig_seq, want,
                         __atomic_load_n(p->h_flag, __ATOMIC_ACQUIRE), p->round, (int)p->deferred_pending,
                         std::chrono::duration<double>(std::chrono::steady_clock::now() - t_start).count());
        abandon_deferred(p);
        p->exhausted = true;
        return sc_internal_fail(SC_ERR_HIP, "the host took longer than the wait kernel's bound to deliver a challenge; the proof is void");
    }
    std::memcpy(out_evals, p->h_out, (size_t)p->D * 32);
    return SC_OK;
}

constexpr size_t kTailSyncBytes = 4 * (16 + (size_t)scd::kTailMaxGrid);
std::atomic<uint64_t> g_stat[8];
struct TailOwner {
    std::mutex mu;
    sc_prover *owner = nullptr;
    bool resident = false;
    const uint32_t *marker = nullptr;
};
static TailOwner g_tail_owner[64];
bool tail_slot_acquire(sc_prover *p, bool resident) {
    TailOwner &t = g_tail_owner[(unsigned)p->device & 63u];
    std::lock_guard<std::mutex> lk(t.mu);
    if (t.owner && t.owner != p) {
        if (!(t.resident && t.marker && __atomic_load_n(t.marker, __ATOMIC_ACQUIRE) != 0)) {
            g_stat[kStatTailSlotBusy].fetch_add(1, std::memory_order_relaxed);
            return false;
        }
        g_stat[kStatTailSlotReclaims].fetch_add(1, std::memory_order_relaxed);
    }
    t.owner = p;
    t.resident = resident;
    t.marker = p->sig ? p->sig + 1 : nullptr;
    return true;
}
void tail_slot_release(sc_prover *p) {
    TailOwner &t = g_tail_owner[(unsigned)p->device & 63u];
    std::lock_guard<std::mutex> lk(t.mu);
    if (t.owner == p) {
        t.owner = nullptr;
        t.marker = nullptr;
    }
}
struct TailSlot {
    sc_prover *const p;
    bool held;
    explicit TailSlot(sc_prover *p_) : p(p_), held(tail_slot_acquire(p_, false)) {}
    ~TailSlot() {
        if (held) tail_slot_release(p);
    }
    TailSlot(const TailSlot &) = delete;
    TailSlot &operator=(const TailSlot &) = delete;
};
bool tail_shape_ok(const sc_prover *p) {
    return p->use_tail && p->K > 0 && p->U <= (uint32_t)scd::kMaxSmallTables && p->has_meta && p->K <= (uint32_t)scd::kMetaProds &&
           (size_t)p->K * p->D * (p->D + 2) * 32 <= 48 * 1024;
}
int tail_slices_blocks_for(sc_prover *p);
bool tail_possible(sc_prover *p, bool slices = false) {
    if (!tail_shape_ok(p) || p->exhausted || p->round >= p->nv || p->deferred_pending) return false;
    if (p->streamed && p->round < 2) return false;
    const uint64_t next_pairs = 1ULL << (p->nv - (p->round + 1));
    if (next_pairs > scd::kTailMaxPairs && !(slices && next_pairs <= scd::kTsMaxPairs && tail_slices_blocks_for(p) > 0)) return false;
    if (!ensure_mailbox(p)) return false;
    if (!p->d_tail_sync) {
        if (hipMalloc(reinterpret_cast<void **>(&p->d_tail_sync), kTailSyncBytes + 64 + (size_t)p->K * p->D * 32) != hipSuccess) {
            (void)hipGetLastError();
            return false;
        }
        p->tail_max_blocks = scd::tail_max_resident_blocks(p->device);
    }
    return p->tail_max_blocks > 0;
}

static uint32_t tail_tables_worst_p(sc_prover *p) {
    bool f29 = false;
    for (uint32_t u = 0; u < p->U; ++u) f29 = f29 || p->tabs[u].cur_top != nullptr;
    return scd::tail_worst_p(f29 ? p->round : 0);
}
int tail_slices_blocks_for(sc_prover *p) {
    if (scd::policy(scd::kPolTailSlices) == 0 || p->max_mult > (uint32_t)(p->wide_tree ? scd::kMaxWideM : scd::kMaxFusedM) || p->round >= p->nv) return 0;
    const int B = scd::tail_slices_blocks(1ULL << (p->nv - (p->round + 1)), (int)p->U, (int)p->K, (int)p->D, p->n_combos, (int)p->max_mult,
                                          scd::tail_slices_max_blocks(p->device, (int)p->max_mult), tail_tables_worst_p(p));
    if (B <= 0) return 0;
    if (!p->d_tail_xw) {
        if (hipMalloc(reinterpret_cast<void **>(&p->d_tail_xw), scd::kTsXwWords * 8) != hipSuccess ||
            hipMemsetAsync(p->d_tail_xw, 0, scd::kTsXwWords * 8, p->stream) != hipSuccess) {
            (void)hipGetLastError();
            if (p->d_tail_xw) (void)hipFree(p->d_tail_xw);
            p->d_tail_xw = nullptr;
            return 0;
        }
        p->ts_tag = 1;
        int large_bar = 0;
        if (scd::policy(scd::kPolVramMailbox) != 0 && hipDeviceGetAttribute(&large_bar, hipDeviceAttributeIsLargeBar, p->device) == hipSuccess && large_bar) {
            void *m = nullptr;
            if (hipExtMallocWithFlags(&m, 256, hipDeviceMallocFinegrained) == hipSuccess && hipMemsetAsync(m, 0, 256, p->stream) == hipSuccess &&
                hipStreamSynchronize(p->stream) == hipSuccess)
                p->d_vram_mail = static_cast<uint64_t *>(m);
            else if (m)
                (void)hipFree(m);
        }
        (void)hipGetLastError();
    }
    return B;
}
int tail_launch(sc_prover *p, uint32_t n_rounds, const sch::Fr *r_or_null, uint32_t max_spins, scd::TailArgs &A, int &grid, int slices_B = 0, bool host_mailbox_only = false) {
    const uint32_t D = p->D;
    std::memset(&A, 0, sizeof(A));
    for (uint32_t u = 0; u < p->U; ++u) {
        Table &t = p->tabs[u];
        A.t.cur0[u] = t.cur;
        A.t.cur0_top[u] = t.cur_top;
        A.t.b0[u] = t.buf[t.next];
        A.t.b1[u] = t.buf[t.next ^ 1];
    }
    A.n_tables = (int)p->U;
    A.n_rounds = (int)n_rounds;
    A.first_has_bind = r_or_null ? 1 : 0;
    A.first_pairs = 1ULL << (p->nv - (p->round + 1));
    if (r_or_null) A.r0 = to_dev(*r_or_null);
    A.n_combos = p->n_combos;
    A.K = (int)p->K;
    A.D = (int)D;
    A.Wm = reinterpret_cast<const uint4 *>(p->d_W);
    A.partials = reinterpret_cast<uint4 *>(p->d_partials);
    A.sync = p->d_tail_sync;
    A.chal = reinterpret_cast<uint64_t *>(reinterpret_cast<char *>(p->d_tail_sync) + kTailSyncBytes);
    A.sums = reinterpret_cast<uint4 *>(reinterpret_cast<char *>(p->d_tail_sync) + kTailSyncBytes + 64);
    A.h_out = reinterpret_cast<uint4 *>(p->h_out_dev);
    A.h_flag = p->h_flag_dev;
    A.seq0 = p->seq + 1;
    A.sig = p->sig_dev;
    A.mail_host = reinterpret_cast<const uint64_t *>(p->h_mail_dev) + 16;
    A.sig0 = p->sig_seq;
    A.max_spins = max_spins;
    scd::FinMeta fm;
    std::memset(&fm, 0, sizeof(fm));
    std::memcpy(fm.prod, p->h_finprods.data(), (size_t)p->K * sizeof(FinProd));
    grid = 1;
    if (A.first_pairs > scd::tail_flat_pairs(p->n_combos)) {
        const uint64_t bind_blocks = (2 * A.first_pairs * p->U + scd::kBlock - 1) / scd::kBlock;
        const uint64_t sum_blocks = ((A.first_pairs + scd::kBlock - 1) / scd::kBlock) * (uint64_t)p->n_combos;
        grid = (int)std::min<uint64_t>((uint64_t)p->tail_max_blocks, std::max(bind_blocks, sum_blocks));
    }
    if (slices_B > 0) {
        HIP_TRY(scd::launch_zero_words(p->d_tail_sync, (uint32_t)((kTailSyncBytes + 64) / 4), p->stream, reinterpret_cast<uint32_t *>(p->d_tail_xw),
                                       (uint32_t)(scd::kTsAccWords * 2)));
        scd::TailSlicesArgs S;
        std::memset(&S, 0, sizeof(S));
        S.base = A;
        S.B = slices_B;
        S.xw = p->d_tail_xw;
        S.tag0 = p->ts_tag;
        S.mail_vram = host_mailbox_only ? nullptr : p->d_vram_mail;
        S.worst_p = tail_tables_worst_p(p);
        p->ts_tag += n_rounds;
        grid = slices_B;
        HIP_TRY(scd::launch_tail_slices(S, p->meta, fm, (int)p->max_mult, p->stream));
        return SC_OK;
    }
    HIP_TRY(scd::launch_zero_words(p->d_tail_sync, (uint32_t)((kTailSyncBytes + 64) / 4), p->stream));
    HIP_TRY(scd::launch_tail_rounds(A, p->meta, fm, grid, p->stream));
    return SC_OK;
}
void tail_epilogue_tables(sc_prover *p, uint32_t nb) {
    if (nb == 0) return;
    for (uint32_t u = 0; u < p->U; ++u) {
        Table &t = p->tabs[u];
        uint4 *b0 = t.buf[t.next], *b1 = t.buf[t.next ^ 1];
        t.cur = (nb & 1) ? b0 : b1;
        t.cur_top = nullptr;
        if (nb & 1) t.next ^= 1;
    }
}
void tail_post_challenge(sc_prover *p, uint32_t sv, const sch::Fr &vm, bool vram = false) {
    uint64_t *slot = reinterpret_cast<uint64_t *>(p->h_mail) + 16 + 8 * (sv & 1u);
    if (vram) {
        volatile uint64_t *vslot = p->d_vram_mail + 8 * (sv & 1u);
        for (int i = 0; i < 8; ++i) vslot[i] = ((uint64_t)(uint32_t)(vm.l[i >> 1] >> (32 * (i & 1))) << 32) | sv;
        __atomic_thread_fence(__ATOMIC_SEQ_CST);
        return;
    }
    for (int i = 0; i < 8; ++i) {
        const uint32_t limb = (uint32_t)(vm.l[i >> 1] >> (32 * (i & 1)));
        __atomic_store_n(slot + i, ((uint64_t)limb << 32) | sv, __ATOMIC_RELEASE);
    }
}

int run_tail(sc_prover *p, sch::Blake2b512Rng &rng, uint32_t n_rounds, const sch::Fr *r_or_null, uint64_t *out_msgs, sch::Fr *out_challenges) {
    gate_lock(p->device);
    struct Unlock {
        const int device;
        bool held = true;
        void release() {
            if (held) gate_unlock(device);
            held = false;
        }
        ~Unlock() { release(); }
    } gate{p->device};
    HIP_TRY(hipSetDevice(p->device));
    int rc_t = collect_timing(p);
    if (rc_t) return rc_t;
    const uint32_t D = p->D;
    scd::TailArgs A;
    int grid = 1;
    const int slices_B = tail_slices_blocks_for(p);
    int rc_l = tail_launch(p, n_rounds, r_or_null, scd::wait_spins_default(), A, grid, slices_B);
    if (rc_l) return rc_l;
    g_stat[kStatTailLaunches].fetch_add(1, std::memory_order_relaxed);
    if (slices_B > 0) g_stat[kStatTailSlices].fetch_add(1, std::memory_order_relaxed);
    scd::plan_hit(slices_B > 0 ? (p->max_mult > (uint32_t)scd::kMaxFusedM ? scd::kPlanTailSlices12 : scd::kPlanTailSlices8) : scd::kPlanTailRounds);
    gate.release();
    p->seq += n_rounds;
    p->sig_seq += n_rounds - 1;
    if (r_or_null) p->randomness.push_back(*r_or_null);
    static const bool trace = std::getenv("SC_HOST_TRACE") != nullptr;
    auto t_prev = std::chrono::steady_clock::now();
    int rc = SC_OK;
    for (uint32_t j = 0; j < n_rounds; ++j) {
        uint64_t *pm = out_msgs + (size_t)j * D * 4;
        if (rc == SC_OK) {
            uint64_t spins = 0;
            bool seen = false;
            const auto t_start = std::chrono::steady_clock::now();
            while (!(seen = (__atomic_load_n(p->h_flag, __ATOMIC_ACQUIRE) == A.seq0 + j))) {
                if ((++spins & 0xfff) == 0) {
                    if (wait_gave_up(p)) break;
                    if (std::chrono::steady_clock::now() - t_start > publish_timeout()) break;
                }
            }
            if (!seen || wait_gave_up(p)) {
                if (std::getenv("SC_HOST_TRACE")) {
                    const uint64_t *tg = reinterpret_cast<const uint64_t *>(p->h_mail) + 16;
                    std::fprintf(stderr, "[sc] tail failure: waiting for message %u of %u (seq %u), h_flag %u, give-up marker %u, sig0 %u, grid %d, first_pairs %llu, tags %u %u\n", j,
                                 n_rounds, A.seq0 + j, __atomic_load_n(p->h_flag, __ATOMIC_ACQUIRE), __atomic_load_n(p->sig + 1, __ATOMIC_ACQUIRE), A.sig0, grid,
                                 (unsigned long long)A.first_pairs, (uint32_t)tg[0], (uint32_t)tg[8]);
                }
                rc = sc_internal_fail(SC_ERR_HIP, wait_gave_up(p) ? "the host took longer than the wait kernel's bound to deliver a challenge; the proof is void"
                                                      : "a tail round did not publish its message within 20 s");
            }
        }
        if (trace) {
            const auto now = std::chrono::steady_clock::now();
            std::fprintf(stderr, "[sc] tail round %u (%llu pairs): message after %.1f us\n", p->round + j + 1,
                         (unsigned long long)(A.first_pairs >> j), std::chrono::duration<double, std::micro>(now - t_prev).count());
            t_prev = now;
        }
        sch::Fr vm = sch::zero();
        if (rc == SC_OK) {
            std::memcpy(pm, p->h_out, (size_t)D * 32);
            rng.feed_prover_msg(reinterpret_cast<const sch::Fr *>(pm), D);
            vm = rng.sample_fr();
            if (out_challenges) out_challenges[j] = vm;
        }
// ... 557 lines not shown
```

### sumcheck_amd/csrc/prover_internal.hpp

```cpp
#pragma once
#include <hip/hip_runtime.h>

#include <dlfcn.h>
#include <rccl/rccl.h>

#include <algorithm>
#include <array>
#include <atomic>
#include <chrono>
#include <condition_variable>
#include <map>
#include <memory>
#include <mutex>
#include <cstdarg>
#include <cstdio>
#include <cstdlib>
#include <cstring>
#include <new>
#include <string>
#include <thread>
#include <vector>

#include "../../include/sumcheck_hip.h"
#include "host_fr.hpp"
#include "kernels.h"
#include "transcript.hpp"

using scd::FinProd;
using scd::FrHost;
using scd::ProdArgs;
using scd::Combo;
using scd::TablePtrs;

std::chrono::milliseconds publish_timeout();
extern thread_local uint16_t g_gate_depth[64];
void gate_lock(int device);
void gate_unlock(int device);
struct DeviceGate {
    const int device;
    explicit DeviceGate(int d) : device(d) { gate_lock(device); }
    ~DeviceGate() { gate_unlock(device); }
    DeviceGate(const DeviceGate &) = delete;
    DeviceGate &operator=(const DeviceGate &) = delete;
};
struct GateYield {
    const int device;
    uint16_t depth;
    GateYield(int d, bool enable) : device(d), depth(enable ? g_gate_depth[(unsigned)d & 63u] : 0) {
        for (uint16_t i = 0; i < depth; ++i) gate_unlock(device);
    }
    ~GateYield() {
        for (uint16_t i = 0; i < depth; ++i) gate_lock(device);
    }
    GateYield(const GateYield &) = delete;
    GateYield &operator=(const GateYield &) = delete;
};
int sc_internal_fail(int code, const char *fmt, ...);
int &sc_internal_device_ref();
#define HIP_TRY(expr)                                                                                                   \
    do {                                                                                                                \
        hipError_t e_ = (expr);                                                                                         \
        if (e_ != hipSuccess) {                                                                                         \
            (void)hipGetLastError();                                                                                    \
            return sc_internal_fail(e_ == hipErrorOutOfMemory ? SC_ERR_OOM : SC_ERR_HIP, "%s failed: %s (%s:%d)", #expr,            \
                        hipGetErrorString(e_), __FILE__, __LINE__);                                                     \
        }                                                                                                               \
    } while (0)

static inline FrHost to_dev(const sch::Fr &a) {
    FrHost h;
    std::memcpy(&h, &a, sizeof(h));
    return h;
}

struct sc_rng {
    sch::Blake2b512Rng rng;
};

struct Product {
    sch::Fr coeff;
    std::vector<uint32_t> tables;
    std::vector<uint32_t> exps;
    uint32_t M = 0;
    bool fused = false;
    uint64_t partial_off = 0;
    uint32_t slot_off = 0;
};

struct Table {
    const uint4 *cur = nullptr;
    const int32_t *cur_top = nullptr;
    uint4 *buf[2] = {nullptr, nullptr};
    int32_t *buf_top[2] = {nullptr, nullptr};
    int next = 0;
};

constexpr uint32_t kResidentSpinsDefault = 256;
struct sc_prover {
    int device = 0;
    hipStream_t stream = nullptr;
    hipStream_t own_stream = nullptr;
    uint32_t nv = 0, max_mult = 0, D = 0, K = 0, U = 0, round = 0;
    bool exhausted = false;
    std::vector<sch::Fr> randomness;
    std::vector<Product> prods;
    std::vector<Table> tabs;
    void *arena = nullptr;
    FrHost *d_partials = nullptr;
    FrHost *d_partials2 = nullptr;
    uint32_t *d_fin_mb_counter = nullptr;
    uint32_t *d_fin_counters = nullptr;
    FinProd *d_finprods = nullptr;
    FrHost *d_W = nullptr;
    uint32_t w_elems = 0;
    bool w_scaled = false;
    FrHost *d_scratch = nullptr;
    FrHost *d_sums[2] = {nullptr, nullptr};
    int64_t sums_round = -1;
    FrHost *d_out = nullptr;
    FrHost *h_out = nullptr;
    uint32_t *h_flag = nullptr;
    FrHost *h_out_dev = nullptr;
    uint32_t *h_flag_dev = nullptr;
    uint32_t seq = 0;
    uint64_t *d_wide = nullptr;
    uint32_t wide_gen = 0;
    bool wide_tagged = false;
    uint64_t *h_wide = nullptr;
    uint64_t *h_wide_dev = nullptr;
    void *d_tail_send = nullptr, *d_tail_recv = nullptr, *d_tail_tabs = nullptr;
    sc_prover *tail = nullptr;
    uint32_t tail_ranks = 0;
    size_t tail_buf_bytes = 0;
    std::vector<std::vector<uint32_t>> prod_indices;
    Combo *d_combos = nullptr;
    std::vector<FinProd> h_finprods;
    scd::ComboMeta meta;
    bool has_meta = false;
    int n_combos = 0;
    bool any_generic = false;
    const uint4 **d_cur_tables = nullptr;
    const uint4 **h_cur_tables = nullptr;
    uint32_t *d_slot_table = nullptr, *d_slot_exp = nullptr;
    hipEvent_t ev0 = nullptr, ev1 = nullptr;
    bool timed = false;
    uint32_t *sig = nullptr;
    uint32_t *sig_dev = nullptr;
    uint32_t sig_seq = 0;
    FrHost *h_mail = nullptr;
    FrHost *h_mail_dev = nullptr;
    FrHost *d_mail = nullptr;
    uint32_t *d_tail_sync = nullptr;
    uint64_t *d_tail_xw = nullptr;
    uint32_t ts_tag = 1;
    uint64_t *d_vram_mail = nullptr;
    int tail_max_blocks = 0;
    uint64_t arena_bytes = 0;
    std::vector<uint8_t> pool_key;
    uint32_t n_retries = 0;
    bool pipeline_ok = true;
    bool polling_off_by_caller = false;
    struct Resident {
        bool active = false;
        bool first_has_bind = false;
        uint32_t seq0 = 0, sig0 = 0, n_rounds = 0, done = 0;
    } res;
    uint32_t resident_spins = kResidentSpinsDefault;
    bool deferred_pending = false;
    bool fused_finalize = false;
    bool use_tail = true;
    bool merge_rounds = false;
    bool wide_tree = true;
    bool use_f29 = false;
    bool use_fe = true;
    int kernel_variant = 3;
    bool streamed = false;
// ... 133 lines not shown
```

Measured before the change: 535.4 billion field-ops/s.

## Pack 9x29-bit f29 limbs into 32 bytes and drop separate top-limb array

Intermediate f29 tables used to be stored as 8 raw limbs in the main buffer plus a separate int32 array holding the top limb. They are now bit-packed into 256 bits, after a settle step that keeps the signed top limb in range. This removes the extra top-limb array and its loads and stores, cutting per-table memory from 36 to 32 bytes per entry and the memory traffic of the bind rounds. In exchange, every load now does shift/mask unpacking and every store does a conditional add of p plus packing, which adds ALU work.

```diff
diff --git a/sumcheck_amd/build.py b/sumcheck_amd/build.py
--- a/sumcheck_amd/build.py
+++ b/sumcheck_amd/build.py
@@ -9,7 +9,7 @@
 OUT = os.path.join(HERE, "libsumcheck_hip.so")
 OUT_EXP = os.path.join(HERE, "libsumcheck_hip_exp.so")
 SOURCES = ["kernels_big.hip", "kernels.hip", "kernels_tail.hip", "kernels_batch.hip", "kernels_batch_gkr.hip", "kernels_batch_eval.hip", "kernels_batch_rounds.hip", "kernels_wide.hip", "kernels_wide16.hip", "gkr.hip", "abi.hip", "protocol.hip", "batch.hip", "batch_rounds.hip", "comm.hip", "kernels_selftest.hip"]
-HEADERS = ["fr_device.hpp", "fe_device.hpp", "kernel_common.hpp", "finalize_device.hpp", "batch_round.hpp", "wide_cell.hpp", "fe_mad_chain.inc", "fr_mac.inc", "fr_mul_gen.inc", "kernels.h", "host_fr.hpp", "transcript.hpp", "prover_internal.hpp", "load_factor.hpp", "wide_tree.hpp", os.path.join("..", "..", "include", "sumcheck_hip.h")]
+HEADERS = ["fr_device.hpp", "fe_device.hpp", "f29_pack.hpp","kernel_common.hpp", "finalize_device.hpp", "batch_round.hpp", "wide_cell.hpp", "fe_mad_chain.inc", "fr_mac.inc", "fr_mul_gen.inc", "kernels.h", "host_fr.hpp", "transcript.hpp", "prover_internal.hpp", "load_factor.hpp", "wide_tree.hpp", os.path.join("..", "..", "include", "sumcheck_hip.h")]
 EXTRA = os.environ.get("SC_BUILD_EXTRA", "").split()
 FLAGS = ["--offload-arch=gfx950", "-O3", "-std=c++17", "-fPIC", "-fvisibility=hidden", "-Wall", "-Wno-unused-function"]
 
diff --git a/sumcheck_amd/csrc/abi.hip b/sumcheck_amd/csrc/abi.hip
--- a/sumcheck_amd/csrc/abi.hip
+++ b/sumcheck_amd/csrc/abi.hip
@@ -334,7 +334,7 @@
     bool staged = false;
     const uint64_t s0 = small_foot ? std::max<uint64_t>(n >> 1, 1) : n;
     const uint64_t s1 = small_foot ? std::max<uint64_t>(n >> 2, 1) : std::max<uint64_t>(n >> 1, 1);
-    const uint64_t per_table = (s0 + s1) * 36;
+    const uint64_t per_table = (s0 + s1) * 32;
     HIP_TRY(hipMalloc(&p->arena, per_table * p->U));
     p->arena_bytes = per_table * p->U;
     p->tabs.resize(p->U);
@@ -345,8 +345,6 @@
         char *base = static_cast<char *>(p->arena) + per_table * u;
         t.buf[0] = reinterpret_cast<uint4 *>(base);
         t.buf[1] = reinterpret_cast<uint4 *>(base + s0 * 32);
-        t.buf_top[0] = reinterpret_cast<int32_t *>(base + (s0 + s1) * 32);
-        t.buf_top[1] = t.buf_top[0] + s0;
         if (streamed) {
             t.cur = nullptr;
             t.next = 0;
@@ -535,7 +533,7 @@
         std::memset(&tp, 0, sizeof(tp));
         for (uint32_t j = 0; j < cnt; ++j) {
             tp.src[j] = p->tabs[u0 + j].cur;
-            tp.src_top[j] = p->tabs[u0 + j].cur_top;
+            tp.src_f29[j] = p->tabs[u0 + j].cur_f29 ? 1 : 0;
             tp.dst[j] = reinterpret_cast<uint4 *>(d_out + 4 * n_out * (size_t)(u0 + j));
         }
         HIP_TRY(scd::launch_fix_multi(tp, (int)cnt, to_dev(rr), nullptr, n_out, p->stream));
@@ -580,9 +578,9 @@
         void *tmp = nullptr;
         for (uint32_t u = 0; u < p->U; ++u) {
             const void *src = p->tabs[u].cur;
-            if (p->tabs[u].cur_top) {
+            if (p->tabs[u].cur_f29) {
                 if (!tmp) HIP_TRY(hipMalloc(&tmp, n * 32));
-                HIP_TRY(scd::launch_f29_to_sat(p->tabs[u].cur, p->tabs[u].cur_top, static_cast<uint4 *>(tmp), n, p->stream));
+                HIP_TRY(scd::launch_f29_to_sat(p->tabs[u].cur, static_cast<uint4 *>(tmp), n, p->stream));
                 src = tmp;
             }
             HIP_TRY(hipMemcpyAsync(tables_out + 4 * n * u, src, n * 32, hipMemcpyDeviceToHost, p->stream));
@@ -680,7 +678,7 @@
                 p->host_tabs[u] = tables_or_null[u];
             }
             p->tabs[u].cur = nullptr;
-            p->tabs[u].cur_top = nullptr;
+            p->tabs[u].cur_f29 = false;
             p->tabs[u].next = 0;
         }
     } else if (p->borrow) {
@@ -690,7 +688,7 @@
                 p->origin[u] = reinterpret_cast<const uint4 *>(tables_or_null[u]);
             }
             p->tabs[u].cur = p->origin[u];
-            p->tabs[u].cur_top = nullptr;
+            p->tabs[u].cur_f29 = false;
             p->tabs[u].next = 0;
         }
     } else {
@@ -705,7 +703,7 @@
                 HIP_TRY(hipMemcpyAsync(p->tabs[u].buf[0], tables_or_null[u], n * 32, on_device ? hipMemcpyDeviceToDevice : hipMemcpyHostToDevice,
                                        p->stream));
             p->tabs[u].cur = p->tabs[u].buf[0];
-            p->tabs[u].cur_top = nullptr;
+            p->tabs[u].cur_f29 = false;
             p->tabs[u].next = 1;
         }
         if (staged) {
@@ -725,7 +723,7 @@
 
 hipStream_t sc_internal_prover_stream(sc_prover *p) { return p->stream; }
 const void *sc_internal_bound_table(sc_prover *p, uint32_t u) {
-    if (!p || u >= p->U || p->round != p->nv || p->exhausted || p->tabs[u].cur_top || p->res.active) return nullptr;
+    if (!p || u >= p->U || p->round != p->nv || p->exhausted || p->tabs[u].cur_f29 || p->res.active) return nullptr;
     return p->tabs[u].cur;
 }
 int sc_internal_scale_by_bound_table(sc_prover *p, const void *table, const sch::Fr &r_last) {
diff --git a/sumcheck_amd/csrc/f29_pack.hpp b/sumcheck_amd/csrc/f29_pack.hpp
--- /dev/null
+++ b/sumcheck_amd/csrc/f29_pack.hpp
@@ -0,0 +1,44 @@
+#pragma once
+#include <cstdint>
+
+#if defined(__HIPCC__)
+#define SC_F29_FN __host__ __device__ __forceinline__
+#else
+#define SC_F29_FN inline
+#endif
+
+namespace scd {
+
+constexpr int32_t kF29Mask = 0x1fffffff;
+constexpr int32_t kF29RuleTop = (0x0073eda7 >> 1) + 1;
+
+SC_F29_FN constexpr int32_t f29_p_limb(int i) {
+    return i == 0 ? 0x00000001 : i == 1 ? 0x1ffffff8 : i == 2 ? 0x1f96ffbf : i == 3 ? 0x1b4805ff : i == 4 ? 0x1d80553b
+         : i == 5 ? 0x0c0404d0 : i == 6 ? 0x1520cce7 : i == 7 ? 0x0a6533af : 0x0073eda7;
+}
+
+SC_F29_FN void f29_unpack(const uint32_t (&w)[8], int32_t (&l)[9]) {
+    l[0] = (int32_t)(w[0] & (uint32_t)kF29Mask);
+#pragma unroll
+    for (int i = 1; i < 8; ++i) l[i] = (int32_t)(((w[i - 1] >> (32 - 3 * i)) | (w[i] << (3 * i))) & (uint32_t)kF29Mask);
+    l[8] = (int32_t)w[7] >> 8;
+}
+
+SC_F29_FN void f29_pack(const int32_t (&l)[9], uint32_t (&w)[8]) {
+#pragma unroll
+    for (int k = 0; k < 8; ++k) w[k] = ((uint32_t)l[k] >> (3 * k)) | ((uint32_t)l[k + 1] << (29 - 3 * k));
+}
+
+SC_F29_FN void f29_settle(int32_t (&l)[9]) {
+    const int32_t add = l[8] < -kF29RuleTop ? -1 : 0;
+    int32_t c = 0;
+#pragma unroll
+    for (int i = 0; i < 8; ++i) {
+        const int32_t t = l[i] + (f29_p_limb(i) & add) + c;
+        l[i] = t & kF29Mask;
+        c = t >> 29;
+    }
+    l[8] = l[8] + (f29_p_limb(8) & add) + c;
+}
+
+}
diff --git a/sumcheck_amd/csrc/fe_device.hpp b/sumcheck_amd/csrc/fe_device.hpp
--- a/sumcheck_amd/csrc/fe_device.hpp
+++ b/sumcheck_amd/csrc/fe_device.hpp
@@ -2,6 +2,7 @@
 #include <utility>
 #include "fr_device.hpp"
 #include "kernels.h"
+#include "f29_pack.hpp"
 
 namespace scd {
 
@@ -15,8 +16,7 @@
 constexpr int32_t kFeMask = 0x1fffffff;
 
 __device__ __forceinline__ constexpr int32_t fe_p_limb(int i) {
-    return i == 0 ? 0x00000001 : i == 1 ? 0x1ffffff8 : i == 2 ? 0x1f96ffbf : i == 3 ? 0x1b4805ff : i == 4 ? 0x1d80553b
-         : i == 5 ? 0x0c0404d0 : i == 6 ? 0x1520cce7 : i == 7 ? 0x0a6533af : 0x0073eda7;
+    return f29_p_limb(i);
 }
 
 __device__ __forceinline__ Fe fe_from_fr(const Fr &a) {
@@ -114,17 +114,23 @@
     const uint64_t col = ((q & 63) >> 1) | ((q & 1) << 5);
     return (entry >> 7) * 256 + (uint64_t)(2 * (int)(entry & 1) + half) * 64 + col;
 }
-__device__ __forceinline__ Fe fe_load_f29(const uint4 *main, uint64_t entry, int32_t top) {
+__device__ __forceinline__ Fe fe_load_f29(const uint4 *main, uint64_t entry) {
     const uint4 a = f29_ld(main + f29_chunk(entry, 0)), b = f29_ld(main + f29_chunk(entry, 1));
-    Fe r;
-    r.l[0] = (int32_t)a.x; r.l[1] = (int32_t)a.y; r.l[2] = (int32_t)a.z; r.l[3] = (int32_t)a.w;
-    r.l[4] = (int32_t)b.x; r.l[5] = (int32_t)b.y; r.l[6] = (int32_t)b.z; r.l[7] = (int32_t)b.w;
-    r.l[8] = top;
+    const uint32_t w[8] = {a.x, a.y, a.z, a.w, b.x, b.y, b.z, b.w};
+    Fe r;
+    f29_unpack(w, r.l);
     return r;
 }
 __device__ __forceinline__ void fe_store_f29(uint4 *main, uint64_t entry, const Fe &v) {
-    f29_st(main + f29_chunk(entry, 0), (uint32_t)v.l[0], (uint32_t)v.l[1], (uint32_t)v.l[2], (uint32_t)v.l[3]);
-    f29_st(main + f29_chunk(entry, 1), (uint32_t)v.l[4], (uint32_t)v.l[5], (uint32_t)v.l[6], (uint32_t)v.l[7]);
+    uint32_t w[8];
+    f29_pack(v.l, w);
+    f29_st(main + f29_chunk(entry, 0), w[0], w[1], w[2], w[3]);
+    f29_st(main + f29_chunk(entry, 1), w[4], w[5], w[6], w[7]);
+}
+__device__ __forceinline__ Fe fe_settle_f29(const Fe &a) {
+    Fe r = a;
+    f29_settle(r.l);
+    return r;
 }
 template <bool kChain>
 __device__ __forceinline__ void fe_mad(int64_t &acc, const int32_t a, const int32_t b) {
diff --git a/sumcheck_amd/csrc/kernels.h b/sumcheck_amd/csrc/kernels.h
--- a/sumcheck_amd/csrc/kernels.h
+++ b/sumcheck_amd/csrc/kernels.h
@@ -28,8 +28,8 @@
     uint4 *dst;
     uint32_t mode;
     uint32_t exp;
-    const int32_t *src_top;
-    int32_t *dst_top;
+    uint32_t src_f29;
+    uint32_t dst_f29;
 };
 
 struct ProdArgs {
@@ -80,7 +80,7 @@
 struct TablePtrs {
     const uint4 *src[kMaxSmallTables];
     uint4 *dst[kMaxSmallTables];
-    const int32_t *src_top[kMaxSmallTables];
+    uint8_t src_f29[kMaxSmallTables];
 };
 struct Combo {
     uint32_t t;
@@ -123,7 +123,7 @@
 }
 struct TailTables {
     const uint4 *cur0[kMaxSmallTables];
-    const int32_t *cur0_top[kMaxSmallTables];
+    uint8_t cur0_f29[kMaxSmallTables];
     uint4 *b0[kMaxSmallTables];
     uint4 *b1[kMaxSmallTables];
 };
@@ -383,7 +383,7 @@
 hipError_t launch_gather_to_tables(const uint4 *recv, uint4 *tabs, uint32_t G, uint32_t U, uint32_t per, hipStream_t stream);
 hipError_t launch_msg_accumulate(const FrHost *in, FrHost *acc, int D, bool first, bool last, FrHost *d_out, uint64_t *d_out_wide, FrHost *h_out_mapped,
                                  uint32_t *h_flag_mapped, uint32_t seq, hipStream_t stream);
-hipError_t launch_f29_to_sat(const uint4 *src, const int32_t *src_top, uint4 *dst, uint64_t n, hipStream_t stream);
+hipError_t launch_f29_to_sat(const uint4 *src, uint4 *dst, uint64_t n, hipStream_t stream);
 hipError_t launch_fr_elementwise(int op, const uint4 *a, const uint4 *b, const FrHost &u, uint4 *out, uint64_t n, hipStream_t stream);
 hipError_t launch_bench_modmul(uint64_t n_threads, uint32_t reps, uint32_t variant, uint64_t *d_sink, hipStream_t stream);
 
diff --git a/sumcheck_amd/csrc/kernels.hip b/sumcheck_amd/csrc/kernels.hip
--- a/sumcheck_amd/csrc/kernels.hip
+++ b/sumcheck_amd/csrc/kernels.hip
@@ -126,15 +126,14 @@
     const FeU r32 = feu_shl5(r.v);
     const uint4 *__restrict__ src = tp.src[blockIdx.y];
     uint4 *__restrict__ dst = tp.dst[blockIdx.y];
-    const int32_t *__restrict__ stop = tp.src_top[blockIdx.y];
+    const bool sf29 = tp.src_f29[blockIdx.y] != 0;
     const uint64_t stride = (uint64_t)gridDim.x * kBlock;
     for (uint64_t b = (uint64_t)blockIdx.x * kBlock + threadIdx.x; b < n_out; b += stride) {
         const uint4 *p = src + 4 * b;
         Fe lo, hi;
-        if (stop) {
-            const int2 t = *reinterpret_cast<const int2 *>(stop + 2 * b);
-            lo = fe_load_f29(src, 2 * b, t.x);
-            hi = fe_load_f29(src, 2 * b + 1, t.y);
+        if (sf29) {
+            lo = fe_load_f29(src, 2 * b);
+            hi = fe_load_f29(src, 2 * b + 1);
         } else {
             lo = fe_from_fr(fr_load(p));
             hi = fe_from_fr(fr_load(p + 2));
@@ -143,11 +142,10 @@
     }
 }
 
-__global__ __launch_bounds__(kBlock) void k_f29_to_sat(const uint4 *__restrict__ src, const int32_t *__restrict__ stop, uint4 *__restrict__ dst,
-                                                       const uint64_t n) {
+__global__ __launch_bounds__(kBlock) void k_f29_to_sat(const uint4 *__restrict__ src, uint4 *__restrict__ dst, const uint64_t n) {
     const uint64_t stride = (uint64_t)gridDim.x * kBlock;
     for (uint64_t i = (uint64_t)blockIdx.x * kBlock + threadIdx.x; i < n; i += stride)
-        fr_store(dst + 2 * i, fe_to_fr(fe_load_f29(src, i, stop[i])));
+        fr_store(dst + 2 * i, fe_to_fr(fe_load_f29(src, i)));
 }
 
 template <typename SlotsT, typename TabFn>
@@ -475,11 +473,10 @@
                 const uint4 *src = tab(u);
                 uint4 *dst = (binds & 1) ? A.t.b1[u] : A.t.b0[u];
                 Fe lo, hi;
-                const int32_t *stop = binds == 0 ? A.t.cur0_top[u] : nullptr;
-                if (stop) {
-                    const int2 t = *reinterpret_cast<const int2 *>(stop + 2 * b);
-                    lo = fe_load_f29(src, 2 * b, t.x);
-                    hi = fe_load_f29(src, 2 * b + 1, t.y);
+                const bool sf29 = binds == 0 && A.t.cur0_f29[u] != 0;
+                if (sf29) {
+                    lo = fe_load_f29(src, 2 * b);
+                    hi = fe_load_f29(src, 2 * b + 1);
                 } else {
                     lo = fe_from_fr(fr_load(src + 4 * b));
                     hi = fe_from_fr(fr_load(src + 4 * b + 2));
@@ -946,8 +943,8 @@
     return hipGetLastError();
 }
 
-hipError_t launch_f29_to_sat(const uint4 *src, const int32_t *src_top, uint4 *dst, uint64_t n, hipStream_t stream) {
-    hipLaunchKernelGGL(k_f29_to_sat, dim3(grid_for_pairs(n)), dim3(kBlock), 0, stream, src, src_top, dst, n);
+hipError_t launch_f29_to_sat(const uint4 *src, uint4 *dst, uint64_t n, hipStream_t stream) {
+    hipLaunchKernelGGL(k_f29_to_sat, dim3(grid_for_pairs(n)), dim3(kBlock), 0, stream, src, dst, n);
     return hipGetLastError();
 }
 
diff --git a/sumcheck_amd/csrc/kernels_big.hip b/sumcheck_amd/csrc/kernels_big.hip
--- a/sumcheck_amd/csrc/kernels_big.hip
+++ b/sumcheck_amd/csrc/kernels_big.hip
@@ -700,7 +700,7 @@
 #endif
     bool round1 = args.fin.enabled == 0;
     for (int q = 0; q < args.n_prod && round1; ++q)
-        for (uint32_t f = 0; f < args.prod[q].M; ++f) round1 = round1 && args.prod[q].slot[f].mode == 0 && args.prod[q].slot[f].src_top == nullptr;
+        for (uint32_t f = 0; f < args.prod[q].M; ++f) round1 = round1 && args.prod[q].slot[f].mode == 0 && args.prod[q].slot[f].src_f29 == 0;
 #ifdef SC_EXPERIMENTS
     if (!split) {
         if (skip1) return hipErrorInvalidValue;
@@ -718,7 +718,7 @@
     bool canonical_sources = !round1;
 #endif
     for (int q = 0; q < args.n_prod && canonical_sources; ++q)
-        for (uint32_t f = 0; f < args.prod[q].M; ++f) canonical_sources = canonical_sources && args.prod[q].slot[f].src_top == nullptr;
+        for (uint32_t f = 0; f < args.prod[q].M; ++f) canonical_sources = canonical_sources && args.prod[q].slot[f].src_f29 == 0;
     const dim3 g(grid, args.n_prod), b(kBlock);
     uint4 *const part = (uint4 *)d_partials;
     plan_hit(round1 ? kPlanBigMergedRound1 : canonical_sources ? kPlanBigMergedBindChain : kPlanBigMergedBind);
diff --git a/sumcheck_amd/csrc/kernels_selftest.hip b/sumcheck_amd/csrc/kernels_selftest.hip
--- a/sumcheck_amd/csrc/kernels_selftest.hip
+++ b/sumcheck_amd/csrc/kernels_selftest.hip
@@ -28,6 +28,8 @@
     kOpFoldCell = 16,
     kOpWideValue = 17,
     kOpWideExt = 18,
+    kOpF29RoundTrip = 19,
+    kOpF29Settle = 20,
 };
 
 __device__ __forceinline__ Fe st_load(const int32_t *p, const uint64_t i) {
@@ -119,6 +121,9 @@
         const Fe r = bt_combo_sum(true, (uint32_t)(gid % L), (int)L, pairs, lazy_sum_needs_reduce(pairs, (uint32_t)p2),
                                   [&](const uint32_t pr) -> Fe { return st_load(a, group * pairs + pr); });
         st_store(out, gid, r);
+    } else if constexpr (kOp == kOpF29Settle) {
+        const Fe r = fe_settle_f29(st_load(a, i));
+        if (live) st_store(out, i, r);
     } else if constexpr (kOp == kOpFoldCell) {
         uint64_t lane[8];
 #pragma unroll
@@ -126,6 +131,15 @@
         const Fr r = wide_fold_cell(lane);
         if (live) st_store_fr(out, i, r);
     }
+}
+
+__global__ __launch_bounds__(kTsBlock) void k_f29_store_op(const int32_t *__restrict__ a, uint4 *__restrict__ table, const uint64_t n) {
+    const uint64_t i = (uint64_t)blockIdx.x * kTsBlock + threadIdx.x;
+    if (i < n) fe_store_f29(table, i, st_load(a, i));
+}
+__global__ __launch_bounds__(kTsBlock) void k_f29_load_op(const uint4 *__restrict__ table, int32_t *__restrict__ out, const uint64_t n) {
+    const uint64_t i = (uint64_t)blockIdx.x * kTsBlock + threadIdx.x;
+    if (i < n) st_store(out, i, fe_load_f29(table, i));
 }
 
 template <int m, int t>
@@ -169,9 +183,10 @@
         const uint64_t L = par[1];
         if (par[0] == 0 || par[0] > 64 || L == 0 || L > 64 || (L & (L - 1)) != 0 || n % kTsBlock != 0) return -2;
     }
-    if ((op >= kOpMul && op <= kOpMul2Chain) || op == kOpShl5MulU || op == kOpLine) {
+    if ((op >= kOpMul && op <= kOpMul2Chain) || op == kOpShl5MulU || op == kOpLine || op == kOpF29RoundTrip) {
         if (b == nullptr) return -2;
     }
+    if (op == kOpF29RoundTrip && n % 128 != 0) return -2;
     if ((op == kOpMul2 || op == kOpMul2Chain) && (c == nullptr || d == nullptr)) return -2;
     const int64_t p0 = (int64_t)par[0], p1 = (int64_t)par[1], p2 = (int64_t)par[2];
 #define SC_FE_OP(OP)                                                                                                    \
@@ -202,6 +217,13 @@
         SC_FE_OP(kOpLine)
         SC_FE_OP(kOpAccum)
         SC_FE_OP(kOpFoldCell)
+        SC_FE_OP(kOpF29Settle)
+    case kOpF29RoundTrip: {
+        uint4 *table = reinterpret_cast<uint4 *>(const_cast<int32_t *>(b));
+        hipLaunchKernelGGL(k_f29_store_op, grid, block, 0, 0, a, table, n);
+        hipLaunchKernelGGL(k_f29_load_op, grid, block, 0, 0, table, out, n);
+        break;
+    }
     case kOpWideValue:
         SC_WIDE_OP(k_wide_value_op, 4, 5) SC_WIDE_OP(k_wide_value_op, 4, 6) SC_WIDE_OP(k_wide_value_op, 4, 7) SC_WIDE_OP(k_wide_value_op, 4, 8)
         SC_WIDE_OP(k_wide_value_op, 3, 4) SC_WIDE_OP(k_wide_value_op, 3, 5) SC_WIDE_OP(k_wide_value_op, 3, 6) SC_WIDE_OP(k_wide_value_op, 3, 7)
diff --git a/sumcheck_amd/csrc/kernels_tail.hip b/sumcheck_amd/csrc/kernels_tail.hip
--- a/sumcheck_amd/csrc/kernels_tail.hip
+++ b/sumcheck_amd/csrc/kernels_tail.hip
@@ -172,21 +172,20 @@
                 const uint32_t u = i >> shE, e = i & (E - 1);
                 const uint64_t ge = (uint64_t)g * E + e;
                 const uint4 *src = A.t.cur0[u];
-                const int32_t *stop = A.t.cur0_top[u];
+                const bool sf29 = A.t.cur0_f29[u] != 0;
                 Fe v;
                 if (has_bind) {
                     Fe lo, hi;
-                    if (stop) {
-                        const int2 t = *reinterpret_cast<const int2 *>(stop + 2 * ge);
-                        lo = fe_load_f29(src, 2 * ge, t.x);
-                        hi = fe_load_f29(src, 2 * ge + 1, t.y);
+                    if (sf29) {
+                        lo = fe_load_f29(src, 2 * ge);
+                        hi = fe_load_f29(src, 2 * ge + 1);
                     } else {
                         lo = fe_from_fr(fr_load(src + 4 * ge));
                         hi = fe_from_fr(fr_load(src + 4 * ge + 2));
                     }
                     v = fe_carry_pass(fe_add(lo, fe_mul_u<true>(fe_sub(hi, lo), r32)));
                 } else {
-                    v = stop ? fe_load_f29(src, ge, stop[ge]) : fe_from_fr(fr_load(src + 2 * ge));
+                    v = sf29 ? fe_load_f29(src, ge) : fe_from_fr(fr_load(src + 2 * ge));
                 }
                 ts_lds_store(tab_at((int)u, e), v);
             }
diff --git a/sumcheck_amd/csrc/load_factor.hpp b/sumcheck_amd/csrc/load_factor.hpp
--- a/sumcheck_amd/csrc/load_factor.hpp
+++ b/sumcheck_amd/csrc/load_factor.hpp
@@ -14,13 +14,12 @@
             return;
         }
         const uint32_t mode = sl.mode;
-        const int32_t *stop = sl.src_top;
+        const bool sf29 = sl.src_f29 != 0;
         if (mode == 0) {
             const uint4 *p = sl.src + 4 * b;
-            if (stop) {
-                const int2 t = *reinterpret_cast<const int2 *>(stop + 2 * b);
-                lo_out = fe_load_f29(sl.src, 2 * b, t.x);
-                hi_out = fe_load_f29(sl.src, 2 * b + 1, t.y);
+            if (sf29) {
+                lo_out = fe_load_f29(sl.src, 2 * b);
+                hi_out = fe_load_f29(sl.src, 2 * b + 1);
             } else {
                 lo_out = fe_from_fr(fr_load(p));
                 hi_out = fe_from_fr(fr_load(p + 2));
@@ -28,24 +27,22 @@
         } else {
             const uint4 *p = sl.src + 8 * b;
             Fe e0, e1, e2, e3;
-            if (stop) {
-                const int4 t = *reinterpret_cast<const int4 *>(stop + 4 * b);
+            if (sf29) {
                 const uint4 *m = sl.src;
-                e0 = fe_load_f29(m, 4 * b, t.x); e1 = fe_load_f29(m, 4 * b + 1, t.y);
-                e2 = fe_load_f29(m, 4 * b + 2, t.z); e3 = fe_load_f29(m, 4 * b + 3, t.w);
+                e0 = fe_load_f29(m, 4 * b); e1 = fe_load_f29(m, 4 * b + 1);
+                e2 = fe_load_f29(m, 4 * b + 2); e3 = fe_load_f29(m, 4 * b + 3);
             } else {
                 e0 = fe_from_fr(fr_load(p)); e1 = fe_from_fr(fr_load(p + 2)); e2 = fe_from_fr(fr_load(p + 4)); e3 = fe_from_fr(fr_load(p + 6));
             }
             const Fe l0 = fe_add(e0, fe_mul_bind<kChain>(fe_sub(e1, e0), r));
             asm volatile("" : "+v"(e3.l[8]) : "v"(l0.l[8]));
             const Fe h0 = fe_add(e2, fe_mul_bind<kChain>(fe_sub(e3, e2), r));
-            if (sl.dst_top || (mode == 3 && stop)) {
-                lo_out = fe_carry_pass(l0);
-                hi_out = fe_carry_pass(h0);
+            if (sl.dst_f29 || (mode == 3 && sf29)) {
+                lo_out = fe_settle_f29(l0);
+                hi_out = fe_settle_f29(h0);
                 if (mode == 1) {
                     fe_store_f29(sl.dst, 2 * b, lo_out);
                     fe_store_f29(sl.dst, 2 * b + 1, hi_out);
-                    *reinterpret_cast<int2 *>(sl.dst_top + 2 * b) = make_int2(lo_out.l[8], hi_out.l[8]);
                 }
             } else {
                 const Fr lc = fe_to_fr(l0), hc = fe_to_fr(h0);
diff --git a/sumcheck_amd/csrc/protocol.hip b/sumcheck_amd/csrc/protocol.hip
--- a/sumcheck_amd/csrc/protocol.hip
+++ b/sumcheck_amd/csrc/protocol.hip
@@ -190,17 +190,17 @@
                         scd::Slot &sl = tp.slot[f];
                         sl.exp = 1;
                         sl.src = ring_tab(u);
-                        sl.src_top = nullptr;
+                        sl.src_f29 = 0;
                         if (!bind) {
                             sl.mode = 0;
                         } else if (!bound[u]) {
                             sl.mode = 1;
                             sl.dst = t.buf[0] + 2 * (c * (C / 2));
-                            sl.dst_top = p->use_f29 ? t.buf_top[0] + c * (C / 2) : nullptr;
+                            sl.dst_f29 = p->use_f29 ? 1 : 0;
                             bound[u] = 1;
                         } else {
                             sl.mode = 3;
-                            sl.dst_top = p->use_f29 ? t.buf_top[0] : nullptr;
+                            sl.dst_f29 = p->use_f29 ? 1 : 0;
                         }
                     }
                 }
@@ -272,7 +272,7 @@
             for (const Product &pr : p->prods)
                 for (uint32_t tt : pr.tables) referenced |= tt == u;
             t.cur = t.buf[0];
-            t.cur_top = (merged && p->use_f29 && referenced) ? t.buf_top[0] : nullptr;
+            t.cur_f29 = merged && p->use_f29 && referenced;
             t.next = 1;
         }
     }
@@ -472,7 +472,7 @@
                 for (uint32_t j = 0; j < cnt; ++j) {
                     Table &t = p->tabs[u0 + j];
                     tp.src[j] = t.cur;
-                    tp.src_top[j] = t.cur_top;
+                    tp.src_f29[j] = t.cur_f29 ? 1 : 0;
                     tp.dst[j] = t.buf[t.next];
                 }
                 {
@@ -482,7 +482,7 @@
                 for (uint32_t j = 0; j < cnt; ++j) {
                     Table &t = p->tabs[u0 + j];
                     t.cur = t.buf[t.next];
-                    t.cur_top = nullptr;
+                    t.cur_f29 = false;
                     t.next ^= 1;
                 }
             }
@@ -511,14 +511,14 @@
             for (uint32_t j = 0; j < cnt; ++j) {
                 Table &t = p->tabs[u0 + j];
                 tp.src[j] = t.cur;
-                tp.src_top[j] = t.cur_top;
+                tp.src_f29[j] = t.cur_f29 ? 1 : 0;
                 tp.dst[j] = t.buf[t.next];
             }
             HIP_TRY(scd::launch_fix_multi(tp, (int)cnt, rdev, nullptr, 2 * n_pairs, p->stream));
             for (uint32_t j = 0; j < cnt; ++j) {
                 Table &t = p->tabs[u0 + j];
                 t.cur = t.buf[t.next];
-                t.cur_top = nullptr;
+                t.cur_f29 = false;
                 t.next ^= 1;
             }
         }
@@ -552,10 +552,10 @@
         std::memset(&ra, 0, sizeof(ra));
         ra.n_prod = (int)p->K;
         std::vector<const uint4 *> old_src(p->U);
-        std::vector<const int32_t *> old_top(p->U);
+        std::vector<uint8_t> old_f29(p->U);
         for (uint32_t u = 0; u < p->U; ++u) {
             old_src[u] = p->tabs[u].cur;
-            old_top[u] = p->tabs[u].cur_top;
+            old_f29[u] = p->tabs[u].cur_f29 ? 1 : 0;
         }
         for (uint32_t k = 0; k < p->K; ++k) {
             const Product &pr = p->prods[k];
@@ -570,20 +570,20 @@
                     scd::Slot &sl = tp.slot[f];
                     sl.exp = 1;
                     sl.src = old_src[u];
-                    sl.src_top = old_top[u];
+                    sl.src_f29 = old_f29[u];
                     if (!bind) {
                         sl.mode = 0;
                     } else if (!bound[u]) {
                         sl.mode = 1;
                         sl.dst = t.buf[t.next];
-                        sl.dst_top = p->use_f29 ? t.buf_top[t.next] : nullptr;
+                        sl.dst_f29 = p->use_f29 ? 1 : 0;
                         t.cur = t.buf[t.next];
-                        t.cur_top = sl.dst_top;
+                        t.cur_f29 = p->use_f29;
                         t.next ^= 1;
                         bound[u] = 1;
                     } else {
                         sl.mode = 3;
-                        sl.dst_top = p->use_f29 ? t.buf_top[0] : nullptr;
+                        sl.dst_f29 = p->use_f29 ? 1 : 0;
                     }
                 }
             }
@@ -620,31 +620,31 @@
             for (size_t s = 0; s < pr.tables.size(); ++s) {
                 Table &t = p->tabs[pr.tables[s]];
                 const uint4 *old_src = t.cur;
-                const int32_t *old_top = t.cur_top;
+                const uint32_t old_f29 = t.cur_f29 ? 1 : 0;
                 bool stored_here = false;
                 for (uint32_t rep = 0; rep < pr.exps[s]; ++rep, ++f) {
                     a.slot[f].exp = 1;
                     if (bind && !bound[pr.tables[s]]) {
                         a.slot[f].mode = 1;
                         a.slot[f].src = old_src;
-                        a.slot[f].src_top = old_top;
+                        a.slot[f].src_f29 = old_f29;
                         a.slot[f].dst = t.buf[t.next];
-                        a.slot[f].dst_top = p->use_f29 ? t.buf_top[t.next] : nullptr;
+                        a.slot[f].dst_f29 = p->use_f29 ? 1 : 0;
                         t.cur = t.buf[t.next];
-                        t.cur_top = a.slot[f].dst_top;
+                        t.cur_f29 = p->use_f29;
                         t.next ^= 1;
                         bound[pr.tables[s]] = 1;
                         stored_here = true;
                     } else if (stored_here) {
                         a.slot[f].mode = 3;
                         a.slot[f].src = old_src;
-                        a.slot[f].src_top = old_top;
+                        a.slot[f].src_f29 = old_f29;
                         a.slot[f].dst = nullptr;
-                        a.slot[f].dst_top = p->use_f29 ? t.buf_top[0] : nullptr;
+                        a.slot[f].dst_f29 = p->use_f29 ? 1 : 0;
                     } else {
                         a.slot[f].mode = 0;
                         a.slot[f].src = t.cur;
-                        a.slot[f].src_top = t.cur_top;
+                        a.slot[f].src_f29 = t.cur_f29 ? 1 : 0;
                         a.slot[f].dst = nullptr;
                     }
                 }
@@ -696,7 +696,7 @@
                 a.slot[f].mode = 0;
                 a.slot[f].exp = 1;
                 a.slot[f].src = t.cur;
-                a.slot[f].src_top = t.cur_top;
+                a.slot[f].src_f29 = t.cur_f29 ? 1 : 0;
             }
             sch::Fr comp = sch::kOne;
             for (uint32_t dbl = 0; dbl < 5 * (pr.M - 1); ++dbl) comp = sch::add(comp, comp);
@@ -867,7 +867,7 @@
 
 static uint32_t tail_tables_worst_p(sc_prover *p) {
     bool f29 = false;
-    for (uint32_t u = 0; u < p->U; ++u) f29 = f29 || p->tabs[u].cur_top != nullptr;
+    for (uint32_t u = 0; u < p->U; ++u) f29 = f29 || p->tabs[u].cur_f29;
     return scd::tail_worst_p(f29 ? p->round : 0);
 }
 int tail_slices_blocks_for(sc_prover *p) {
@@ -903,7 +903,7 @@
     for (uint32_t u = 0; u < p->U; ++u) {
         Table &t = p->tabs[u];
         A.t.cur0[u] = t.cur;
-        A.t.cur0_top[u] = t.cur_top;
+        A.t.cur0_f29[u] = t.cur_f29 ? 1 : 0;
         A.t.b0[u] = t.buf[t.next];
         A.t.b1[u] = t.buf[t.next ^ 1];
     }
@@ -962,7 +962,7 @@
         Table &t = p->tabs[u];
         uint4 *b0 = t.buf[t.next], *b1 = t.buf[t.next ^ 1];
         t.cur = (nb & 1) ? b0 : b1;
-        t.cur_top = nullptr;
+        t.cur_f29 = false;
         if (nb & 1) t.next ^= 1;
     }
 }
diff --git a/sumcheck_amd/csrc/prover_internal.hpp b/sumcheck_amd/csrc/prover_internal.hpp
--- a/sumcheck_amd/csrc/prover_internal.hpp
+++ b/sumcheck_amd/csrc/prover_internal.hpp
@@ -89,9 +89,8 @@
 
 struct Table {
     const uint4 *cur = nullptr;
-    const int32_t *cur_top = nullptr;
+    bool cur_f29 = false;
     uint4 *buf[2] = {nullptr, nullptr};
-    int32_t *buf_top[2] = {nullptr, nullptr};
     int next = 0;
 };
 
```

Result: faster. 551.9 billion field-ops/s, median of 6 (+3.1%).
